# smacke/ffsubsync

Measured on NVIDIA H100. Metric: alignments/sec (2h@100Hz signals), higher is better.
Workload: dtype int64 VAD; f32 FFT nomination + f64 exact re-score

## Files before the change

__graft_entry__.py:

```python
import os
import subprocess
import sys

ROOT = os.path.dirname(os.path.abspath(__file__))
CSRC = os.path.join(ROOT, "ffsubsync_b200", "csrc")
LIB_DIR = os.path.join(ROOT, "ffsubsync_b200", "_lib")
LIB = os.path.join(LIB_DIR, "libffsubsync_b200.so")
EMUL = os.path.join(ROOT, "tests", "host_emul", "corr_emul")
EMUL_BIG = os.path.join(ROOT, "tests", "host_emul", "bigfft_emul")
EMUL_VAD = os.path.join(ROOT, "tests", "host_emul", "vad_emul")
EMUL_RUNS = os.path.join(ROOT, "tests", "host_emul", "runcorr_emul")
EMUL_RASTER = os.path.join(ROOT, "tests", "host_emul", "raster_emul")
EMUL_GSS = os.path.join(ROOT, "tests", "host_emul", "gss_emul")
EMUL_PLAN = os.path.join(ROOT, "tests", "host_emul", "plan_emul")

NVCC_FLAGS = [
    "-gencode", "arch=compute_90a,code=sm_90a", "-lineinfo", "-O3", "-std=c++17",
    "-Xcompiler", "-fPIC", "-Xcompiler", "-ffp-contract=off", "--fmad=true", "--extended-lambda",
    "-Wno-deprecated-gpu-targets",
]


def _sources():
    return sorted(os.path.join(CSRC, f) for f in os.listdir(CSRC) if f.endswith(".cu"))


def _stale(target, deps):
    if not os.path.exists(target):
        return True
    t = os.path.getmtime(target)
    return any(os.path.getmtime(d) > t for d in deps)


def build(force: bool = False, verbose: bool = False) -> None:
    nvcc = os.environ.get("NVCC", "/usr/local/cuda/bin/nvcc")
    os.makedirs(LIB_DIR, exist_ok=True)
    srcs = _sources()
    hdrs = [os.path.join(CSRC, f) for f in os.listdir(CSRC) if f.endswith((".cuh", ".h"))]
    hdrs.append(os.path.join(ROOT, "include", "ffsubsync_b200.h"))
    if force or _stale(LIB, srcs + hdrs):
        objs = []
        for s in srcs:
            o = os.path.join(LIB_DIR, os.path.basename(s)[:-3] + ".o")
            if force or _stale(o, [s] + hdrs):
                cmd = [nvcc] + NVCC_FLAGS + (["-Xptxas", "-v"] if verbose else []) + ["-c", s, "-o", o]
                subprocess.check_call(cmd)
            objs.append(o)
        subprocess.check_call([nvcc, "-shared", "-o", LIB] + objs + ["-Wno-deprecated-gpu-targets"])
    emu_src = EMUL + ".cu"
    if os.path.exists(emu_src) and (force or _stale(EMUL, [emu_src, os.path.join(CSRC, "corr.cuh")])):
        subprocess.check_call([nvcc, "-O2", "-std=c++17", "-Wno-deprecated-gpu-targets", "-o", EMUL, emu_src])
    big_src = EMUL_BIG + ".cu"
    if os.path.exists(big_src) and (force or _stale(EMUL_BIG, [big_src, os.path.join(CSRC, "corr.cuh"),
                                                               os.path.join(CSRC, "bigfft.cuh")])):
        subprocess.check_call([nvcc, "-O2", "-std=c++17", "--extended-lambda", "-Wno-deprecated-gpu-targets",
                               "-o", EMUL_BIG, big_src])
    runs_src = EMUL_RUNS + ".cu"
    if os.path.exists(runs_src) and (force or _stale(EMUL_RUNS, [runs_src, os.path.join(CSRC, "runcorr.cuh")])):
        subprocess.check_call([nvcc, "-O2", "-std=c++17", "-Wno-deprecated-gpu-targets", "-o", EMUL_RUNS, runs_src])
    raster_src = EMUL_RASTER + ".cu"
    if os.path.exists(raster_src) and (force or _stale(EMUL_RASTER, [raster_src, os.path.join(CSRC, "raster_math.cuh")])):
        subprocess.check_call([nvcc, "-O2", "-std=c++17", "-Xcompiler", "-ffp-contract=off",
                               "-Wno-deprecated-gpu-targets", "-o", EMUL_RASTER, raster_src])
    gss_src = EMUL_GSS + ".cu"
    if os.path.exists(gss_src) and (force or _stale(EMUL_GSS, [gss_src, os.path.join(CSRC, "job_plan.cuh"),
                                                               os.path.join(CSRC, "raster_math.cuh")])):
        subprocess.check_call([nvcc, "-O2", "-std=c++17", "-Xcompiler", "-ffp-contract=off",
                               "-Wno-deprecated-gpu-targets", "-o", EMUL_GSS, gss_src])
    plan_src = EMUL_PLAN + ".cu"
    if os.path.exists(plan_src) and (force or _stale(EMUL_PLAN, [plan_src] + hdrs)):
        subprocess.check_call([nvcc, "-O2", "-std=c++17", "-Xcompiler", "-ffp-contract=off",
                               "-Wno-deprecated-gpu-targets", "-o", EMUL_PLAN, plan_src])
    vad_src = EMUL_VAD + ".cu"
    if os.path.exists(vad_src) and (force or _stale(EMUL_VAD, [vad_src, os.path.join(CSRC, "vad_lane.cuh"),
                                                               os.path.join(CSRC, "vad_group.cuh")])):
        subprocess.check_call([nvcc, "-O2", "-std=c++17", "-gencode", "arch=compute_90a,code=sm_90a",
                               "-Wno-deprecated-gpu-targets", "-o", EMUL_VAD, vad_src])
    sys.path.insert(0, ROOT)
    import ffsubsync_b200
    from ffsubsync_b200 import _native

    _native.load()


def smoke() -> None:
    sys.path.insert(0, ROOT)
    import numpy as np

    from ffsubsync_b200.aligners import FFTAligner, MaxScoreAligner
    from ffsubsync_b200.speech_transformers import _make_auditok_detector, _make_energy_zcr_detector
    from oracle import aligner_oracle as ao
    from oracle import auditok_oracle as au
    from oracle import vad_oracle as vo

    rng = np.random.RandomState(0)
    cls = (rng.rand(2000) > 0.5).astype(np.uint8)
    pcm = vo.synth_pcm(cls, 160, seed=1)
    got = _make_energy_zcr_detector(100, 16000, 0.0)(pcm.tobytes())
    want = vo.energy_zcr_detect(pcm.tobytes(), 100, 16000, 0.0)
    assert np.array_equal(got, want), "VAD mismatch"
    got_a = _make_auditok_detector(100, 16000, 0.0)(pcm.tobytes())
    assert np.array_equal(got_a, au.auditok_detect_fast(pcm.tobytes(), 100, 16000, 0.0)), "auditok mismatch"
    ref = want
    sub = np.concatenate([np.zeros(123), ref])[: len(ref)]
    score, off = FFTAligner(max_offset_samples=600).fit_transform(ref, sub, get_score=True)
    wscore, woff = ao.fft_align(ref, sub, 600)
    assert off == woff == -123, (off, woff)
    assert abs(score - wscore) <= 1e-5 * abs(wscore), (score, wscore)
    (s2, o2), _ = MaxScoreAligner(FFTAligner, None, 100, 6).fit_transform(ref, [sub, sub[::-1].copy()])
    assert o2 == -123
    print("smoke ok: vad windows=%d offset=%d score=%.1f" % (len(got), off, score))


if __name__ == "__main__":
    build(force="--force" in sys.argv, verbose="-v" in sys.argv)
    if "--smoke" in sys.argv:
        smoke()
```

ffsubsync_b200/csrc/api.cu:

```cuda
#include <math.h>

#include <chrono>
#include <cmath>
#include <algorithm>
#include <atomic>
#include <thread>

#include "common.cuh"
#include "sync_plan.h"

struct DeviceScope {
  int prev = -1, want;
  bool ok = true;
  explicit DeviceScope(int dev) : want(dev) {
    if (cudaGetDevice(&prev) != cudaSuccess) prev = -1;
    if (prev != want) ok = cudaSetDevice(want) == cudaSuccess;
  }
  ~DeviceScope() {
    if (prev >= 0 && prev != want) cudaSetDevice(prev);
  }
};
extern "C" int b2_version(void) { return 200; }

static uint64_t compute_log2_quirk_mask() {
// ... 625 lines not shown
  if (memspace == B2_HOST) {
    void *da, *db, *dq;
    B2_TRY(stage_in(h, b2_ctx::WS_STAGE_IN0, a, (size_t)n * 4, &da));
    B2_TRY(stage_in(h, b2_ctx::WS_STAGE_IN1, b, (size_t)n * 4, &db));
    B2_TRY(b2i_ws(h, b2_ctx::WS_STAGE_OUT, (size_t)n * 4, &dq));
    d_a = (const float*)da;
    d_b = (const float*)db;
    d_out = (float*)dq;
  }
  B2_TRY(b2i_blend_launch(h, d_a, d_b, n, mode, wa, wb, d_out));
  if (memspace == B2_HOST) {
    B2_TRY(copy_out(h, out, d_out, (size_t)n * 4));
    B2_CUDA(h, cudaStreamSynchronize(h->stream));
  }
  return B2_OK;
}

extern "C" int b2_first_last_nonzero(b2_handle h, const float* sig, const int64_t* sig_off, int n,
                                     int64_t* first, int64_t* last, int memspace) {
  B2_ENTER(h);
  if (n < 0 || !sig_off || !first || !last) B2_FAIL(h, B2_ERR_BAD_ARG, "boundaries: bad arguments");
  if (n == 0) return B2_OK;
  const float* d_sig = sig;
  int64_t *d_first = first, *d_last = last;
  if (memspace == B2_HOST) {
    void *dp, *dq;
    B2_TRY(stage_in(h, b2_ctx::WS_STAGE_IN0, sig, (size_t)sig_off[n] * 4, &dp));
    B2_TRY(b2i_ws(h, b2_ctx::WS_STAGE_OUT, (size_t)n * 16, &dq));
    d_sig = (const float*)dp;
    d_first = (int64_t*)dq;
    d_last = d_first + n;
  }
  B2_TRY(b2i_bounds_launch(h, d_sig, sig_off, n, d_first, d_last));
  if (memspace == B2_HOST) {
    B2_TRY(copy_out(h, first, d_first, (size_t)n * 8));
    B2_TRY(copy_out(h, last, d_last, (size_t)n * 8));
    B2_CUDA(h, cudaStreamSynchronize(h->stream));
  }
  return B2_OK;
}

extern "C" int b2_align_batch(b2_handle h, const float* ref, const int64_t* ref_off,
                              const float* sub, const int64_t* sub_off, int B, int K,
                              int64_t max_offset_samples, double* score, int32_t* offset,
                              int32_t* status, int memspace) {
  B2_ENTER(h);
  if (B < 0 || K < 0 || !ref_off || !sub_off) B2_FAIL(h, B2_ERR_BAD_ARG, "align: bad arguments");
  if (B == 0 || K == 0) return B2_OK;
  if (!score || !offset || !status) B2_FAIL(h, B2_ERR_BAD_ARG, "align: null output");
  size_t J = (size_t)B * K;
  B2_CHECK_DEV(h, memspace, ref, "align: ref");
  B2_CHECK_DEV(h, memspace, sub, "align: sub");
  B2_CHECK_DEV(h, memspace, score, "align: score");
  const float *d_ref = ref, *d_sub = sub;
  double* d_score = score;
  int32_t *d_offset = offset, *d_status = status;
  if (memspace == B2_HOST) {
    void *dr, *ds, *dq;
    B2_TRY(stage_in(h, b2_ctx::WS_STAGE_IN0, ref, (size_t)ref_off[B] * 4, &dr));
    B2_TRY(stage_in(h, b2_ctx::WS_STAGE_IN1, sub, (size_t)sub_off[J] * 4, &ds));
    B2_TRY(b2i_ws(h, b2_ctx::WS_STAGE_OUT, J * 16 + 64, &dq));
    d_ref = (const float*)dr;
    d_sub = (const float*)ds;
    d_score = (double*)dq;
    d_offset = (int32_t*)(d_score + J);
    d_status = d_offset + J;
  }
  B2_TRY(b2i_align_launch(h, d_ref, ref_off, B, nullptr, d_sub, sub_off, B, K, max_offset_samples,
                          d_score, d_offset, d_status, 0, nullptr, 0));
  if (memspace == B2_HOST) {
    B2_TRY(copy_out(h, score, d_score, J * 8));
    B2_TRY(copy_out(h, offset, d_offset, J * 4));
    B2_TRY(copy_out(h, status, d_status, J * 4));
    B2_CUDA(h, cudaStreamSynchronize(h->stream));
  }
  return B2_OK;
}

extern "C" int b2_capture_nominations(b2_handle h, float* scores, int64_t stride, int64_t* win, float* stat,
                                      int32_t* cand) {
  B2_ENTER(h);
  h->capture = B2Capture{};
  if (!scores) return B2_OK;
  if (stride <= 0 || !win || !stat || !cand) B2_FAIL(h, B2_ERR_BAD_ARG, "capture: bad arguments");
  B2_TRY(check_device_ptr(h, scores, "capture: scores"));
  B2_TRY(check_device_ptr(h, win, "capture: win"));
  B2_TRY(check_device_ptr(h, stat, "capture: stat"));
  B2_TRY(check_device_ptr(h, cand, "capture: cand"));
  h->capture = B2Capture{scores, (long long)stride, (long long*)win, stat, cand};
  return B2_OK;
}

extern "C" int b2_reduce_ratios(b2_handle h, const double* score, const int32_t* offset,
                                const int32_t* status, int B, int K, int64_t max_offset_samples,
                                double* best_score, int32_t* best_offset, int32_t* best_k,
                                int memspace) {
  B2_ENTER(h);
  if (B < 0 || K <= 0) B2_FAIL(h, B2_ERR_BAD_ARG, "reduce: bad arguments");
  if (B == 0) return B2_OK;
  if (!score || !offset || !best_score || !best_offset || !best_k)
    B2_FAIL(h, B2_ERR_BAD_ARG, "reduce: null pointer");
  size_t J = (size_t)B * K;
  const double* d_score = score;
  const int32_t *d_offset = offset, *d_status = status;
  double* d_bs = best_score;
  int32_t *d_bo = best_offset, *d_bk = best_k;
  if (memspace == B2_HOST) {
    void *d0, *dq;
    B2_TRY(b2i_ws(h, b2_ctx::WS_STAGE_IN0, J * 16 + 64, &d0));
    B2_CUDA(h, cudaMemcpyAsync(d0, score, J * 8, cudaMemcpyHostToDevice, h->stream));
    int32_t* doff = (int32_t*)((char*)d0 + J * 8);
    B2_CUDA(h, cudaMemcpyAsync(doff, offset, J * 4, cudaMemcpyHostToDevice, h->stream));
    int32_t* dst = doff + J;
    if (status)
      B2_CUDA(h, cudaMemcpyAsync(dst, status, J * 4, cudaMemcpyHostToDevice, h->stream));
    B2_TRY(b2i_ws(h, b2_ctx::WS_STAGE_OUT, (size_t)B * 16 + 64, &dq));
    d_score = (const double*)d0;
    d_offset = doff;
    d_status = status ? dst : nullptr;
    d_bs = (double*)dq;
    d_bo = (int32_t*)(d_bs + B);
    d_bk = d_bo + B;
  }
  B2_TRY(b2i_reduce_launch(h, d_score, d_offset, d_status, B, K, max_offset_samples, d_bs, d_bo,
                           d_bk));
  if (memspace == B2_HOST) {
    B2_TRY(copy_out(h, best_score, d_bs, (size_t)B * 8));
    B2_TRY(copy_out(h, best_offset, d_bo, (size_t)B * 4));
    B2_TRY(copy_out(h, best_k, d_bk, (size_t)B * 4));
    B2_CUDA(h, cudaStreamSynchronize(h->stream));
  }
  return B2_OK;
}


struct SyncBufs {
  const int16_t* pcm;
  float* refsig;
  float* subsig;
  double* score;
  int32_t* offset;
  int32_t* status;
  double* bs;
  int32_t* bo;
  int32_t* bk;
  double* g_all_score;
  int32_t* g_all_offset;
  double* g_ratio;
  double* g_evals;
  bool fused;
  int winner_only;
};

static int enqueue_chain(b2_ctx* h, const SyncRequest& r, const SyncPlan& p, const SyncBufs& b, int v0, int v1) {
  const int K = r.K, t0 = p.trk_off[v0], nt = p.trk_off[v1] - t0;
  const size_t j0 = (size_t)t0 * K;
  std::vector<int> chain_trk(v1 - v0 + 1);
  for (int v = v0; v <= v1; ++v) chain_trk[v - v0] = p.trk_off[v] - t0;
  if (!b.fused)
    B2_TRY(b2i_raster_launch(h, r.cue_start_s, r.cue_end_s, r.cue_keep, r.cue_off + t0, nt, r.ratios, K, 0, nullptr,
                             r.sample_rate, r.start_seconds, b.subsig, p.sub_off.data() + j0));
  const B2CueSource src{r.cue_start_s, r.cue_end_s, r.cue_keep, r.cue_off + t0, r.ratios, r.sample_rate,
                        r.start_seconds, p.ref_label, p.two_level};
  B2_TRY(b2i_align_launch(h, b.refsig, p.ref_off.data() + v0, v1 - v0, chain_trk.data(), b.subsig,
                          p.sub_off.data() + j0, nt, K, r.max_offset_samples, b.score + j0, b.offset + j0,
                          b.status + j0, b.winner_only, b.fused ? &src : nullptr, (long long)j0));
  B2_TRY(b2i_reduce_launch(h, b.score + j0, b.offset + j0, b.status + j0, nt, K, r.max_offset_samples, b.bs + t0,
                           b.bo + t0, b.bk + t0));
  if (!p.gss || nt == 0) return B2_OK;
  const size_t a0 = (size_t)t0 * (K + 1);
  const B2GssOut go{b.bs + t0, b.bo + t0, b.bk + t0, b.score + j0, b.offset + j0,
                    b.g_all_score ? b.g_all_score + a0 : nullptr, b.g_all_offset ? b.g_all_offset + a0 : nullptr,
                    b.g_ratio + t0, b.g_evals ? b.g_evals + (size_t)t0 * kGssEvals : nullptr};
  return b2i_gss_launch(h, b.refsig, p.ref_off.data() + v0, v1 - v0, chain_trk.data(), K, src,
                        p.max_end.data() + t0, r.max_offset_samples, go);
}

static int detect(b2_ctx* h, const SyncRequest& r, const SyncPlan& p, const SyncBufs& b, int v0, int v1) {
  if (!p.auditok) {
    B2_TRY(b2i_vad_launch(h, b.pcm, r.pcm_off + v0, v1 - v0, p.fpw, r.energy.non_speech_label,
                          (int64_t)p.fpw * r.energy.energy_threshold, p.z_lo, p.z_hi, b.refsig, p.ref_off.data() + v0));
  } else {
    const ChunkTable& ch = p.ch;
    const int c0 = ch.first[v0], nc = ch.first[v1] - c0;
    B2_TRY(b2i_vad_launch(h, b.pcm, ch.pcm.data() + c0, nc, p.fpw, 0.0f, p.auditok_e_min, 0, p.fpw, b.refsig,
                          ch.out.data() + c0, ch.tail.data() + c0));
    if (!p.any_subs) return b2i_tokenize_inplace_launch(h, b.refsig, ch.out.data() + c0, nc, p.tok);
    const int k0 = ch.tok_first[v0];
    B2_TRY(b2i_tokenize_inplace_launch(h, b.refsig, ch.tok_off.data() + k0, ch.tok_first[v1] - k0, p.tok,
                                       ch.tok_end.data() + k0));
  }
  if (!p.any_subs) return B2_OK;
  const auto& sv = p.sub_video;
  const int s0 = (int)(std::lower_bound(sv.begin(), sv.end(), v0) - sv.begin());
  const int s1 = (int)(std::lower_bound(sv.begin(), sv.end(), v1) - sv.begin());
  if (s1 == s0) return B2_OK;
  std::vector<int> rel(sv.begin() + s0, sv.begin() + s1);
  for (int& v : rel) v -= v0;
  return b2i_raster_ref_launch(h, r.refs.cue_start_s, r.refs.cue_end_s, r.refs.cue_keep, r.refs.cue_off + v0,
                               p.ref_off.data() + v0, v1 - v0, rel.data(), (int)rel.size(), r.sample_rate,
                               r.start_seconds, b.refsig);
}

static int run_pipeline(b2_ctx* h, const SyncRequest& r, const SyncPlan& p, const SyncBufs& b, bool resident,
                        bool chained, int refsig_slot) {
  const int n_sub = p.n_sub;
  const std::vector<int>& cut = p.cut;
  if (n_sub == 1) {
    B2_TRY(detect(h, r, p, b, 0, r.V));
    return enqueue_chain(h, r, p, b, 0, r.V);
  }
  std::vector<cudaEvent_t> vad_done(n_sub);
  cudaEvent_t inputs_ready = next_event(h);
  B2_CUDA(h, cudaEventRecord(inputs_ready, h->stream));
  const bool trace = getenv("B2_PIPE_TRACE") != nullptr;
  std::vector<cudaEvent_t> tev;
  std::vector<double> host_ms(n_sub + 1, 0.0);
  const auto host_t0 = std::chrono::steady_clock::now();
  auto host_now = [&]() { return std::chrono::duration<double, std::milli>(std::chrono::steady_clock::now() - host_t0).count(); };
  if (trace) {
    tev.resize(1 + 4 * (size_t)n_sub);
    for (auto& e : tev) B2_CUDA(h, cudaEventCreate(&e));
    B2_CUDA(h, cudaEventRecord(tev[0], h->stream));
  }
  bool prev_busy = false;
  if (chained) {
    prev_busy = cudaEventQuery(h->resident_done) == cudaErrorNotReady;
    cudaGetLastError();
  }
  {
    Stream2Scope on2(h);
    B2_CUDA(h, cudaStreamWaitEvent(h->stream, chained ? h->resident_fence : inputs_ready, 0));
    for (int i = 0; i < n_sub; ++i) {
      h->vad_partition_sms = (i > 0 || prev_busy) ? p.vad_sms : 0;
      if (trace) B2_CUDA(h, cudaEventRecord(tev[1 + 4 * i], h->stream));
      const int st = detect(h, r, p, b, cut[i], cut[i + 1]);
      h->vad_partition_sms = 0;
      if (st != B2_OK) return st;
      vad_done[i] = next_event(h);
      B2_CUDA(h, cudaEventRecord(vad_done[i], h->stream));
      if (trace) B2_CUDA(h, cudaEventRecord(tev[2 + 4 * i], h->stream));
    }
  }
  host_ms[0] = host_now();
  for (int i = 0; i < n_sub; ++i) {
    if (resident && i == n_sub - 1) B2_CUDA(h, cudaEventRecord(h->resident_fence, h->stream));
    B2_CUDA(h, cudaStreamWaitEvent(h->stream, vad_done[i], 0));
    if (trace) B2_CUDA(h, cudaEventRecord(tev[3 + 4 * i], h->stream));
    B2_TRY(enqueue_chain(h, r, p, b, cut[i], cut[i + 1]));
    if (trace) B2_CUDA(h, cudaEventRecord(tev[4 + 4 * i], h->stream));
    host_ms[i + 1] = host_now();
  }
  if (resident) {
    B2_CUDA(h, cudaEventRecord(h->resident_done, h->stream));
    h->refsig_parity = refsig_slot == b2_ctx::WS_SIG_REF2 ? 1 : 0;
    h->resident_fence_valid = true;
  }
  if (trace) {
    B2_CUDA(h, cudaStreamSynchronize(h->stream2));
    B2_CUDA(h, cudaStreamSynchronize(h->stream));
    auto at = [&](size_t k) {
      float ms = 0.f;
      cudaEventElapsedTime(&ms, tev[0], tev[k]);
      return ms;
    };
    fprintf(stderr, "[b2 pipe] V=%d T=%d n_sub=%d vad_sms=%d chained=%d prev_busy=%d; host: VADs enqueued at %.3f ms\n",
            r.V, r.T, n_sub, p.vad_sms, (int)chained, (int)prev_busy, host_ms[0]);
    for (int i = 0; i < n_sub; ++i)
      fprintf(stderr, "[b2 pipe]  sub %d videos %4d..%4d  VAD %7.3f -> %7.3f ms   chain %7.3f -> %7.3f ms   host enqueued chain at %.3f ms\n",
              i, cut[i], cut[i + 1], at(1 + 4 * i), at(2 + 4 * i), at(3 + 4 * i), at(4 + 4 * i), host_ms[i + 1]);
    for (auto& e : tev) cudaEventDestroy(e);
  }
  return B2_OK;
}

static int sync_run(b2_ctx* h, bool fence_was_valid, const SyncRequest& r) {
  SyncPlan p;
  const SyncPipeEnv env{h->sm_count, b2_ctx::kEvents - 2, getenv("B2_SUBBATCHES"), getenv("B2_VAD_SMS"),
                        b2i_vad_lane_eligible};
  if (const int st = plan_sync(r, env, &p)) {
    h->err = p.err;
    return st;
  }
  const int T = r.T, K = r.K;
  if (T == 0) return B2_OK;
  const bool resident = r.memspace == B2_DEVICE_RESIDENT;
  const int memspace = resident ? B2_DEVICE : r.memspace;
  const char* prefix = r.track_video ? "sync_tracks" : "sync_batch";
  const std::pair<const void*, const char*> bulk[] = {{r.pcm, "pcm"}, {r.best_score, "best_score"},
                                                      {r.best_offset, "best_offset"}, {r.best_k, "best_k"},
                                                      {r.all_score, "all_score"}, {r.all_offset, "all_offset"}};
  for (const auto& [ptr, name] : bulk) {
    char what[64];
    snprintf(what, sizeof(what), "%s: %s", prefix, name);
    B2_CHECK_DEV(h, memspace, ptr, what);
  }
  if (p.gss) {
    B2_CHECK_DEV(h, memspace, r.gss_ratio, "sync_tracks_gss: gss_ratio");
    B2_CHECK_DEV(h, memspace, r.gss_evals, "sync_tracks_gss: gss_evals");
  }
  SyncBufs b{};
  b.fused = true;
  if (const char* e = getenv("B2_FUSED_RASTER")) b.fused = atoi(e) != 0;
  const size_t J = (size_t)T * K, JG = (size_t)T * (K + 1);
  void *d_refsig, *d_subsig = nullptr, *d_res;
  const bool chained = resident && fence_was_valid;
  const int refsig_slot = chained && h->refsig_parity == 0 ? b2_ctx::WS_SIG_REF2 : b2_ctx::WS_SIG_REF;
  B2_TRY(b2i_ws(h, refsig_slot, (size_t)p.ref_off[r.V] * 4 + 64, &d_refsig));
  if (!b.fused) B2_TRY(b2i_ws(h, b2_ctx::WS_SIG_SUB, (size_t)p.sub_off[J] * 4 + 64, &d_subsig));
  B2_TRY(b2i_ws(h, b2_ctx::WS_MISC, J * 16 + (size_t)T * 16 + 256, &d_res));
  double* d_score = (double*)d_res;
  double* d_bs = d_score + J;
  int32_t* d_offset = (int32_t*)(d_bs + T);
  int32_t* d_status = d_offset + J;
  int32_t* d_bo = d_status + J;
  int32_t* d_bk = d_bo + T;
  b.refsig = (float*)d_refsig;
  b.subsig = (float*)d_subsig;
  b.status = d_status;
  b.g_ratio = r.gss_ratio;
  b.g_evals = r.gss_evals;
  if (p.gss) {
    void* d_go;
    B2_TRY(b2i_ws(h, b2_ctx::WS_GSS_OUT, JG * 12 + (size_t)T * 8 * (1 + kGssEvals) + 256, &d_go));
    double* hs = (double*)d_go;
    double* hr = hs + JG;
    double* he = hr + T;
    int32_t* ho = (int32_t*)(he + (size_t)T * kGssEvals);
    b.g_all_score = r.all_score ? (memspace == B2_DEVICE ? r.all_score : hs) : nullptr;
    b.g_all_offset = r.all_offset ? (memspace == B2_DEVICE ? r.all_offset : ho) : nullptr;
    if (memspace != B2_DEVICE) {
      b.g_ratio = hr;
      b.g_evals = r.gss_evals ? he : nullptr;
    }
  }
  b.pcm = r.pcm;
  if (memspace == B2_HOST) {
    void* dp = nullptr;
    if (p.audio_samples > 0) B2_TRY(stage_in(h, b2_ctx::WS_STAGE_IN0, r.pcm, (size_t)r.pcm_off[r.V] * 2, &dp));
    b.pcm = (const int16_t*)dp;
  }
  const bool dev = memspace == B2_DEVICE;
  b.score = (dev && r.all_score && !p.gss) ? r.all_score : d_score;
  b.offset = (dev && r.all_offset && !p.gss) ? r.all_offset : d_offset;
  b.bs = dev ? r.best_score : d_bs;
  b.bo = dev ? r.best_offset : d_bo;
  b.bk = dev ? r.best_k : d_bk;
  b.winner_only = (!r.all_score && !r.all_offset) ? 1 : 0;
  B2_TRY(run_pipeline(h, r, p, b, resident, chained, refsig_slot));
  if (dev) return B2_OK;
  B2_TRY(copy_out(h, r.best_score, d_bs, (size_t)T * 8));
  B2_TRY(copy_out(h, r.best_offset, d_bo, (size_t)T * 4));
  B2_TRY(copy_out(h, r.best_k, d_bk, (size_t)T * 4));
  if (p.gss) {
    if (r.all_score) B2_TRY(copy_out(h, r.all_score, b.g_all_score, JG * 8));
    if (r.all_offset) B2_TRY(copy_out(h, r.all_offset, b.g_all_offset, JG * 4));
    B2_TRY(copy_out(h, r.gss_ratio, b.g_ratio, (size_t)T * 8));
    if (r.gss_evals) B2_TRY(copy_out(h, r.gss_evals, b.g_evals, (size_t)T * kGssEvals * 8));
  } else {
    if (r.all_score) B2_TRY(copy_out(h, r.all_score, d_score, J * 8));
    if (r.all_offset) B2_TRY(copy_out(h, r.all_offset, d_offset, J * 4));
  }
  B2_CUDA(h, cudaStreamSynchronize(h->stream));
  return B2_OK;
}

extern "C" int b2_sync_batch(b2_handle h, const int16_t* pcm, const int64_t* pcm_off, int B,
                             int frame_rate, int sample_rate, float non_speech_label,
                             int64_t energy_threshold, int z_lo, int z_hi,
                             const double* cue_start_s, const double* cue_end_s,
                             const uint8_t* cue_keep, const int64_t* cue_off, const double* ratios,
                             int K, double start_seconds, int64_t max_offset_samples,
                             double* best_score, int32_t* best_offset, int32_t* best_k,
                             double* all_score, int32_t* all_offset, int memspace) {
  B2_ENTER(h);
  B2Range range("b2_sync_batch");
  const SyncRequest r{"sync_batch", pcm, pcm_off, B, nullptr, B, frame_rate, sample_rate, B2_DETECTOR_ENERGY_ZCR,
                      {non_speech_label, energy_threshold, z_lo, z_hi}, {}, {},
                      cue_start_s, cue_end_s, cue_keep, cue_off, ratios, K, start_seconds, max_offset_samples,
                      best_score, best_offset, best_k, all_score, all_offset, false, nullptr, nullptr, memspace};
  return sync_run(h, _b2_fence_was_valid, r);
}

extern "C" int b2_sync_tracks(b2_handle h, const int16_t* pcm, const int64_t* pcm_off, int V,
                              const int32_t* track_video, int T, int frame_rate, int sample_rate,
                              float non_speech_label, int64_t energy_threshold, int z_lo, int z_hi,
                              const double* cue_start_s, const double* cue_end_s, const uint8_t* cue_keep,
                              const int64_t* cue_off, const double* ratios, int K, double start_seconds,
                              int64_t max_offset_samples, double* best_score, int32_t* best_offset,
                              int32_t* best_k, double* all_score, int32_t* all_offset, int memspace) {
  B2_ENTER(h);
  B2Range range("b2_sync_tracks");
  if (T > 0 && !track_video) B2_FAIL(h, B2_ERR_BAD_ARG, "sync_tracks: null track_video");
  const SyncRequest r{"sync_tracks", pcm, pcm_off, V, track_video, T, frame_rate, sample_rate, B2_DETECTOR_ENERGY_ZCR,
                      {non_speech_label, energy_threshold, z_lo, z_hi}, {}, {},
                      cue_start_s, cue_end_s, cue_keep, cue_off, ratios, K, start_seconds, max_offset_samples,
                      best_score, best_offset, best_k, all_score, all_offset, false, nullptr, nullptr, memspace};
  return sync_run(h, _b2_fence_was_valid, r);
}

extern "C" int b2_sync_tracks_gss(b2_handle h, const int16_t* pcm, const int64_t* pcm_off, int V,
                                  const int32_t* track_video, int T, int frame_rate, int sample_rate,
                                  float non_speech_label, int64_t energy_threshold, int z_lo, int z_hi,
                                  const double* cue_start_s, const double* cue_end_s, const uint8_t* cue_keep,
                                  const int64_t* cue_off, const double* ratios, int K, double start_seconds,
                                  int64_t max_offset_samples, double* best_score, int32_t* best_offset,
                                  int32_t* best_k, double* all_score, int32_t* all_offset, double* gss_ratio,
                                  double* gss_evals, int memspace) {
  B2_ENTER(h);
  B2Range range("b2_sync_tracks_gss");
  if (T > 0 && !track_video) B2_FAIL(h, B2_ERR_BAD_ARG, "sync_tracks_gss: null track_video");
  const SyncRequest r{"sync_tracks_gss", pcm, pcm_off, V, track_video, T, frame_rate, sample_rate,
                      B2_DETECTOR_ENERGY_ZCR, {non_speech_label, energy_threshold, z_lo, z_hi}, {}, {},
                      cue_start_s, cue_end_s, cue_keep, cue_off, ratios, K, start_seconds, max_offset_samples,
                      best_score, best_offset, best_k, all_score, all_offset, true, gss_ratio, gss_evals, memspace};
  return sync_run(h, _b2_fence_was_valid, r);
}

extern "C" int b2_sync_tracks_auditok(b2_handle h, const int16_t* pcm, const int64_t* pcm_off, int V,
                                      const int32_t* track_video, int T, int frame_rate, int sample_rate,
                                      double non_speech_label, double energy_threshold_db, double min_length,
                                      int64_t max_length, double max_continuous_silence, int64_t chunk_samples,
                                      const double* cue_start_s, const double* cue_end_s, const uint8_t* cue_keep,
                                      const int64_t* cue_off, const double* ratios, int K, double start_seconds,
                                      int64_t max_offset_samples, double* best_score, int32_t* best_offset,
                                      int32_t* best_k, double* all_score, int32_t* all_offset, double* gss_ratio,
                                      double* gss_evals, int memspace) {
  B2_ENTER(h);
  B2Range range("b2_sync_tracks_auditok");
  if (T > 0 && !track_video) B2_FAIL(h, B2_ERR_BAD_ARG, "sync_tracks_auditok: null track_video");
  if (!gss_ratio && gss_evals) B2_FAIL(h, B2_ERR_BAD_ARG, "sync_tracks_auditok: gss_evals without gss_ratio");
  const SyncRequest r{gss_ratio ? "sync_tracks_auditok (search)" : "sync_tracks_auditok", pcm, pcm_off, V, track_video,
                      T, frame_rate, sample_rate, B2_DETECTOR_AUDITOK, {},
                      {non_speech_label, energy_threshold_db, min_length, max_continuous_silence, max_length,
                       chunk_samples},
                      {}, cue_start_s, cue_end_s, cue_keep, cue_off, ratios, K, start_seconds, max_offset_samples,
                      best_score, best_offset, best_k, all_score, all_offset, gss_ratio != nullptr, gss_ratio, gss_evals,
                      memspace};
  return sync_run(h, _b2_fence_was_valid, r);
}

extern "C" int b2_sync_tracks_subs(b2_handle h, const int16_t* pcm, const int64_t* pcm_off, int V,
                                   const int32_t* track_video, int T, int frame_rate, int sample_rate, int detector,
                                   double non_speech_label, int64_t energy_threshold, int z_lo, int z_hi,
                                   double energy_threshold_db, double min_length, int64_t max_length,
                                   double max_continuous_silence, int64_t chunk_samples, const uint8_t* ref_is_subs,
                                   const double* ref_cue_start_s, const double* ref_cue_end_s,
                                   const uint8_t* ref_cue_keep, const int64_t* ref_cue_off,
                                   const double* cue_start_s, const double* cue_end_s, const uint8_t* cue_keep,
                                   const int64_t* cue_off, const double* ratios, int K, double start_seconds,
                                   int64_t max_offset_samples, double* best_score, int32_t* best_offset,
                                   int32_t* best_k, double* all_score, int32_t* all_offset, double* gss_ratio,
                                   double* gss_evals, int memspace) {
  B2_ENTER(h);
  B2Range range("b2_sync_tracks_subs");
  if (T > 0 && !track_video) B2_FAIL(h, B2_ERR_BAD_ARG, "sync_tracks_subs: null track_video");
// ... 17 lines not shown
```

ffsubsync_b200/csrc/bigfft.cu:

```cuda
#include <math.h>

#include <algorithm>
#include <map>

#include "common.cuh"
#include "bigfft.cuh"
#include "corr_jobs.cuh"

int bigfft_min_log2n() { return bigfft::kMinQ1 + 11; }
int bigfft_max_log2n() { return bigfft::kMaxQ1 + 11; }

namespace {

using namespace bigfft;

struct BigXform {
  long long src_off;
  long long g_off;
  long long spec_off;
  long long score_off;
  int len, S, m_lo, m_hi;
  int is_bits;
  float hi;
};

struct BigJob {
  int j;
  int x_sub, x_ref;
};

constexpr int kFineCap = (1 << kMaxQ1) + (1 << (kMaxQ1 - 4)) + (1 << (kMaxQ1 - 8)) + 4;
constexpr size_t kBigSmemBytes = kSmemBytes + 1024 * 8 + (size_t)kSkew1024 * 8 + (size_t)kFineCap * 8 + 16 * 8 + 64;

struct Smem {
  float2 *buf, *tw1024, *fine32, *half_pos, *coarse, *fine, *row_tw;
};
__device__ __forceinline__ Smem carve(unsigned char* raw) {
  Smem s;
  s.buf = reinterpret_cast<float2*>(raw);
  s.tw1024 = s.buf + kM;
  s.fine32 = s.tw1024 + 1024;
  s.half_pos = s.fine32 + 32;
  s.coarse = s.half_pos + 1024;
  s.fine = s.coarse + kSkew1024;
  s.row_tw = s.fine + kFineCap;
  return s;
}

__device__ __forceinline__ void l2_prefetch_bulk(const void* p, uint32_t bytes) {
  asm volatile("cp.async.bulk.prefetch.L2.global [%0], %1;" ::"l"(p), "r"(bytes) : "memory");
}
__device__ __forceinline__ void l2_prefetch_line(const void* p) {
  asm volatile("prefetch.global.L2 [%0];" ::"l"(p));
}
__device__ __forceinline__ void prefetch_f2_rows(const float2* base, int q1, int g, int tid) {
  if (tid < 16) l2_prefetch_bulk(base + ((size_t)f2_row_of_slot(q1, g, tid) << 10), kRow * 8);
}
__device__ __forceinline__ void prefetch_cols(const float2* base, int q1, int cg, int tid) {
  const int cl = 14 - q1, c0 = cg << cl, seg = 8 << cl;
  for (int r = tid; r < (1 << q1); r += kThreads) {
    const char* p = reinterpret_cast<const char*>(base + ((size_t)r << 10) + c0);
    for (int b = 0; b < seg; b += 128) l2_prefetch_line(p + b);
  }
}

__device__ __forceinline__ float block_sum(float v, float* red) {
  for (int o = 16; o > 0; o >>= 1) v += __shfl_xor_sync(0xffffffffu, v, o);
  __syncthreads();
  if ((threadIdx.x & 31) == 0) red[threadIdx.x >> 5] = v;
  __syncthreads();
  float r = 0.f;
  for (int w = 0; w < kThreads / 32; ++w) r += red[w];
  return r;
}
__device__ __forceinline__ float block_max(float v, float* red) {
  for (int o = 16; o > 0; o >>= 1) v = fmaxf(v, __shfl_xor_sync(0xffffffffu, v, o));
  __syncthreads();
  if ((threadIdx.x & 31) == 0) red[threadIdx.x >> 5] = v;
  __syncthreads();
  float r = -INFINITY;
  for (int w = 0; w < kThreads / 32; ++w) r = fmaxf(r, red[w]);
  return r;
}

template <int Q1>
__global__ void __launch_bounds__(kThreads, 1)
    big_cols_forward_kernel(const float* __restrict__ sig, const uint32_t* __restrict__ bits,
                            const BigXform* __restrict__ xf, int n_tiles, float2* __restrict__ G,
                            float* __restrict__ tile_energy) {
  extern __shared__ __align__(16) unsigned char smem_raw[];
  __shared__ float red[kThreads / 32];
  const Smem sm = carve(smem_raw);
  const int tid = threadIdx.x;
  init_tables(sm.tw1024, sm.fine32, tid);
  init_big_tables(sm.half_pos, sm.coarse, sm.fine, Q1, tid);
  __syncthreads();
  const Tables t{sm.tw1024, sm.fine32};
  const BigTables bt{sm.tw1024, sm.fine32, sm.half_pos, sm.coarse, sm.fine};
  constexpr int tiles_per = (1 << Q1) / 16;
  for (int tile = blockIdx.x; tile < n_tiles; tile += gridDim.x) {
    const BigXform X = xf[tile / tiles_per];
    const int cg = tile % tiles_per;
    const BigSource src{X.is_bits ? nullptr : sig + X.src_off, X.is_bits ? bits + X.src_off : nullptr, X.len, X.hi};
    const float ss = block_sum(f1_load(sm.buf, src, Q1, cg, tid), red);
    if (tid == 0) tile_energy[tile] = ss;
    col_forward<Q1>(sm.buf, t, tid);
    __syncthreads();
    f1_store(sm.buf, bt, Q1, cg, tid, G + X.g_off);
    __syncthreads();
  }
}

template <int MODE>
__global__ void __launch_bounds__(kThreads, 1)
    big_rows_kernel(const BigXform* __restrict__ xf, int n_tiles, int q1, float2* __restrict__ G) {
  extern __shared__ __align__(16) unsigned char smem_raw[];
  const Smem sm = carve(smem_raw);
  const int tid = threadIdx.x;
  init_tables(sm.tw1024, sm.fine32, tid);
  init_big_tables(sm.half_pos, sm.coarse, sm.fine, q1, tid);
  __syncthreads();
  const Tables t{sm.tw1024, sm.fine32};
  const BigTables bt{sm.tw1024, sm.fine32, sm.half_pos, sm.coarse, sm.fine};
  const int tiles_per = (1 << q1) / 16;
  for (int tile = blockIdx.x; tile < n_tiles; tile += gridDim.x) {
    const BigXform X = xf[tile / tiles_per];
    const int g = tile % tiles_per;
    if (tile + (int)gridDim.x < n_tiles) {
      const int nt = tile + gridDim.x;
      const BigXform Xn = xf[nt / tiles_per];
      prefetch_f2_rows(G + Xn.g_off, q1, nt % tiles_per, tid);
      if (MODE == 1) prefetch_f2_rows(G + Xn.spec_off, q1, nt % tiles_per, tid);
    }
    f2_load(sm.buf, q1, g, tid, G + X.g_off);
    f2_row_twiddles(sm.row_tw, q1, g, tid);
    __syncthreads();
    rows_forward(sm.buf, t, tid);
    __syncthreads();
    if (MODE == 0) {
      f2_untangle_inplace(sm.buf, bt, q1, g, sm.row_tw, tid);
      __syncthreads();
      f2_store(sm.buf, q1, g, tid, G + X.spec_off);
    } else {
      f2_product_inplace(sm.buf, bt, q1, g, sm.row_tw, tid, G + X.spec_off);
      __syncthreads();
      rows_inverse(sm.buf, t, tid);
      __syncthreads();
      f2_store_twiddled(sm.buf, bt, q1, g, tid, G + X.g_off);
    }
    __syncthreads();
  }
}

template <int Q1>
__global__ void __launch_bounds__(kThreads, 1)
    big_cols_inverse_kernel(const BigXform* __restrict__ xf, int n_tiles, const float2* __restrict__ G,
                            float* __restrict__ scores, float* __restrict__ tile_max,
                            float* __restrict__ tile_cn) {
  extern __shared__ __align__(16) unsigned char smem_raw[];
  __shared__ float red[kThreads / 32];
  const Smem sm = carve(smem_raw);
  const int tid = threadIdx.x;
  init_tables(sm.tw1024, sm.fine32, tid);
// ... 268 lines not shown
```

ffsubsync_b200/csrc/common.cuh:

```cuda
#pragma once

#include <cuda_runtime.h>
#include <stdint.h>
#include <stdio.h>
#include <string.h>

#include <string>
#include <vector>

#include <nvtx3/nvToolsExt.h>

#include "../../include/ffsubsync_b200.h"

struct B2Range {
  explicit B2Range(const char* name) { nvtxRangePushA(name); }
  ~B2Range() { nvtxRangePop(); }
};

struct DeviceBuf {
  void* p = nullptr;
  size_t cap = 0;
};

struct HostBuf {
  void* p = nullptr;
  size_t cap = 0;
};

struct B2Capture {
  float* scores = nullptr;
  long long stride = 0;
  long long* win = nullptr;
  float* stat = nullptr;
  int* cand = nullptr;
};

struct b2_ctx {
  int device = 0;
  int sm_count = 132;
  cudaStream_t stream = nullptr;
  bool own_stream = true;
  std::string err;
  int64_t launches = 0;
  uint64_t log2_quirk_mask = 0;
  int vad_partition_sms = 0;
  B2Capture capture;
  bool resident_fence_valid = false;
  cudaEvent_t resident_fence = nullptr, resident_done = nullptr;
  int refsig_parity = 0;
  enum { WS_STAGE_IN0, WS_STAGE_IN1, WS_STAGE_OUT, WS_META, WS_SPEC, WS_SCORES, WS_CAND,
         WS_SIG_REF, WS_SIG_REF2, WS_SIG_SUB, WS_MISC, WS_COUNTERS, WS_RUNS, WS_GSS, WS_GSS_OUT, WS_COUNT };
  DeviceBuf ws[WS_COUNT];
  HostBuf pinned[4];
  cudaEvent_t pinned_ev[4] = {};
  static const int kMetaSlots = 8;
  struct MetaSlot {
    void* d = nullptr;
    void* p = nullptr;
    size_t cap = 0;
    cudaEvent_t ev = nullptr;
  };
  MetaSlot meta[2][kMetaSlots];
  uint64_t meta_seq[2] = {0, 0};
  int ring = 0;
  struct VadStream {
    static const int kSlots = 3;
    struct Slot {
      void* hp = nullptr;
      void* dp = nullptr;
      float* hout = nullptr;
      float* dout = nullptr;
      size_t cap = 0, out_cap = 0;
      cudaEvent_t ev = nullptr;
      int64_t n_out = 0;
      bool busy = false;
    } slot[kSlots];
    bool active = false;
    int frame_rate = 0, sample_rate = 0, fpw = 0, z_lo = 0, z_hi = 0;
    float label = 0.f;
    int64_t thr = 0, windows = 0;
    uint64_t seq = 0;
    std::vector<float> results;
  } vs;
  struct Bounce {
    void* p = nullptr;
    cudaEvent_t ev = nullptr;
  } bounce[2];
  cudaStream_t stream2 = nullptr;
  static const int kEvents = 64;
  cudaEvent_t ev_pool[kEvents] = {};
  int ev_next = 0;
};

#define B2_FAIL(h, code, ...)                          \
  do {                                                 \
    char _b[512];                                      \
    snprintf(_b, sizeof(_b), __VA_ARGS__);             \
    (h)->err = _b;                                     \
    return (code);                                     \
  } while (0)

#define B2_CUDA(h, expr)                                                              \
  do {                                                                                \
    cudaError_t _e = (expr);                                                          \
    if (_e != cudaSuccess)                                                            \
      B2_FAIL(h, B2_ERR_CUDA, "%s failed: %s (%s:%d)", #expr, cudaGetErrorString(_e), \
              __FILE__, __LINE__);                                                    \
  } while (0)

#define B2_CHECK_LAUNCH(h, name)                                                         \
  do {                                                                                   \
    (h)->launches++;                                                                     \
    cudaError_t _e = cudaGetLastError();                                                 \
    if (_e != cudaSuccess)                                                               \
      B2_FAIL(h, B2_ERR_CUDA, "launch of %s failed: %s", name, cudaGetErrorString(_e));  \
  } while (0)

#define B2_TRY(expr)            \
  do {                          \
    int _s = (expr);            \
    if (_s != B2_OK) return _s; \
  } while (0)

int b2i_ws(b2_ctx* h, int which, size_t bytes, void** out);
int b2i_pinned(b2_ctx* h, int which, size_t bytes, void** out);
struct MetaArena {
  b2_ctx* h;
  char* dbase = nullptr;
  char* hbase = nullptr;
  size_t cap = 0, used = 0;
  int slot = 0, ring = 0;
};
int b2i_meta_begin(b2_ctx* h, MetaArena* a, size_t bytes);
void* b2i_meta_put(MetaArena* a, const void* src, size_t bytes);
void* b2i_meta_reserve(MetaArena* a, size_t bytes, void** host_view);
int b2i_meta_commit(MetaArena* a);

static inline int64_t ceil_div64(int64_t a, int64_t b) { return (a + b - 1) / b; }

bool b2i_vad_lane_eligible(const int64_t* pcm_off_host, int B, int fpw);
int b2i_vad_launch(b2_ctx* h, const int16_t* d_pcm, const int64_t* pcm_off_host, int B, int fpw,
                   float non_speech_label, int64_t e_min_full, int z_lo, int z_hi,
                   float* d_out, const int64_t* out_off_host, const int64_t* tail_emin_host = nullptr);
struct B2TokenizerParams {
  double min_length, max_continuous_silence, non_speech_label;
  long long max_length;
};
int b2i_tokenize_launch(b2_ctx* h, const float* d_flags, const int64_t* off_host, int n_chunks,
                        const B2TokenizerParams& tp, double* d_out);
int b2i_tokenize_inplace_launch(b2_ctx* h, float* d_flags_sig, const int64_t* off_host, int n_chunks,
                                const B2TokenizerParams& tp, const int64_t* end_host = nullptr);
int b2i_synth_launch(b2_ctx* h, const uint8_t* d_cls, int64_t n_windows, int fpw, uint32_t seed,
                     int16_t* d_out);
int b2i_raster_launch(b2_ctx* h, const double* cue_start, const double* cue_end,
                      const uint8_t* cue_keep, const int64_t* cue_off, int B, const double* ratios,
                      int K, int per_pair_ratios, const double* levels, int sample_rate,
                      double start_seconds, float* d_out, const int64_t* out_off_host);
int b2i_raster_ref_launch(b2_ctx* h, const double* cue_start, const double* cue_end, const uint8_t* cue_keep,
                          const int64_t* cue_off, const int64_t* out_off, int n_videos, const int* videos, int n_subs,
                          int sample_rate, double start_seconds, float* d_out);
int b2i_bounds_launch(b2_ctx* h, const float* d_sig, const int64_t* off_host, int n,
                      int64_t* d_first, int64_t* d_last);
int b2i_blend_launch(b2_ctx* h, const float* d_a, const float* d_b, int64_t n, int mode, double wa,
                     double wb, float* d_out);
struct B2CueSource {
  const double* cue_start;
  const double* cue_end;
  const uint8_t* cue_keep;
  const int64_t* cue_off;
  const double* ratios;
  int sample_rate;
  double start_seconds;
  float ref_label;
  bool ref_two_level;
};
int b2i_raster_bits_launch(b2_ctx* h, const B2CueSource* src, int B, int K, const int64_t* sig_off,
                           const long long* bits_off, uint32_t* d_bits);
struct B2CueDev {
  const double* start;
  const double* end;
  const uint8_t* keep;
  const long long* cue_off;
  int sample_rate;
  double start_seconds;
};
int b2i_raster_bits_dev_launch(b2_ctx* h, const B2CueDev& cues, int n_sig, int64_t max_cues, const double* d_ratio,
                               const long long* d_len, long long sig_words, uint32_t* d_bits);
int b2i_align_launch(b2_ctx* h, const float* d_ref, const int64_t* ref_off_host, int V, const int* trk_off,
                     const float* d_sub, const int64_t* sub_off_host, int B, int K,
                     int64_t max_offset_samples, double* d_score, int32_t* d_offset,
                     int32_t* d_status, int winner_only, const B2CueSource* cue_src,
                     long long capture_j0);
int b2i_reduce_launch(b2_ctx* h, const double* d_score, const int32_t* d_offset,
                      const int32_t* d_status, int B, int K, int64_t max_offset_samples,
                      double* d_best_score, int32_t* d_best_offset, int32_t* d_best_k);
struct B2GssOut {
  double* bs;
  int32_t* bo;
  int32_t* bk;
  const double* g_score;
  const int32_t* g_offset;
  double* a_score;
  int32_t* a_offset;
  double* gss_ratio;
  double* evals;
};
int b2i_gss_launch(b2_ctx* h, const float* d_ref, const int64_t* ref_off_host, int V, const int* trk_off, int K,
                   const B2CueSource& src, const double* max_end, int64_t max_offset_samples, const B2GssOut& out);
```

ffsubsync_b200/csrc/corr.cu:

```cuda
#include <math.h>

#include <algorithm>
#include <cmath>

#include "common.cuh"
#include "corr.cuh"
#include "corr_jobs.cuh"
#include "job_plan.cuh"

namespace {

using namespace corr;

struct SpecItem {
  long long ref_off;
  int R;
  int i0;
};

struct SubJob {
  long long sub_off;
  long long score_off;
  long long spec_base;
  int S, blk_lo, blk_hi, n_out, energy_slot;
  long long bits_off;
  float hi;
};

constexpr size_t kSmemBytesBits = kSmemBytes + 2 * (size_t)(kP / 32) * 4;

__device__ __forceinline__ void l2_prefetch(const void* p, uint32_t bytes) {
  asm volatile("cp.async.bulk.prefetch.L2.global [%0], %1;" ::"l"(p), "r"(bytes) : "memory");
}

__device__ __forceinline__ void l2_prefetch_floats(const float* p, int n) {
  if (n <= 0) return;
  const uintptr_t a0 = (reinterpret_cast<uintptr_t>(p) + 15) & ~uintptr_t(15);
  const uintptr_t a1 = reinterpret_cast<uintptr_t>(p + n) & ~uintptr_t(15);
  if (a1 > a0) l2_prefetch(reinterpret_cast<const void*>(a0), (uint32_t)(a1 - a0));
}

__global__ void __maxnreg__(96)
    ref_spectra_kernel(const float* __restrict__ ref, const SpecItem* __restrict__ items, int n_items,
                       float4* __restrict__ spec, float* __restrict__ spec_energy) {
  extern __shared__ __align__(16) unsigned char smem_raw[];
  float2* buf = reinterpret_cast<float2*>(smem_raw);
  float2* tw1024 = buf + kM;
  float2* fine32 = tw1024 + 1024;
  __shared__ float red[kThreads / 32];
  const int tid = threadIdx.x;
  init_tables(tw1024, fine32, tid);
  __syncthreads();
  const Tables t{tw1024, fine32};
  const PairCtx pc = pair_ctx(t, tid);
  for (int item = blockIdx.x; item < n_items; item += gridDim.x) {
    const SpecItem it = items[item];
    if (tid == 0 && item + (int)gridDim.x < n_items) {
      const SpecItem nx = items[item + gridDim.x];
      const int lo = nx.i0 < 0 ? -nx.i0 : 0, hi = min(nx.R - nx.i0, kP);
      l2_prefetch_floats(ref + nx.ref_off + nx.i0 + lo, hi - lo);
    }
    float ss = float_pass1(buf, t, tid, ref + it.ref_off + it.i0, it.i0 < 0 ? -it.i0 : 0,
                           min(it.R - it.i0, kP));
    forward_rest(buf, t, tid);
    spec_store(buf, t, pc, tid, spec + (size_t)item * kPairs);
    for (int o = 16; o > 0; o >>= 1) ss += __shfl_xor_sync(0xffffffffu, ss, o);
    if ((tid & 31) == 0) red[tid >> 5] = ss;
    __syncthreads();
    if (tid == 0) {
      float e = 0.f;
      for (int w = 0; w < kThreads / 32; ++w) e += red[w];
      spec_energy[item] = e;
    }
  }
}

template <bool BITS>
__device__ __forceinline__ void sub_correlate_body(
    const float* __restrict__ sub, const SubJob* __restrict__ jobs, const float4* __restrict__ spec,
    const float* __restrict__ spec_energy, int L, float* __restrict__ scores,
    float4* __restrict__ job_energy, const uint32_t* __restrict__ sub_bits) {
  extern __shared__ __align__(16) unsigned char smem_raw[];
  float2* buf = reinterpret_cast<float2*>(smem_raw);
  float2* tw1024 = buf + kM;
  float2* fine32 = tw1024 + 1024;
  uint32_t* bit_words = reinterpret_cast<uint32_t*>(smem_raw + kSmemBytes);
  __shared__ float red[kThreads / 32];
  const int tid = threadIdx.x;
  const SubJob job = jobs[blockIdx.x];
  float* out = scores + job.score_off;
  if (job.blk_lo >= job.blk_hi) {
    for (int m = tid; m < job.n_out; m += kThreads) out[m] = 0.f;
    if (tid == 0) job_energy[job.energy_slot] = make_float4(0.f, 0.f, 0.f, 0.f);
    return;
  }
  init_tables(tw1024, fine32, tid);
  const int wpb = L >> 5;
  const uint32_t* bits = BITS ? sub_bits + job.bits_off : nullptr;
  if (BITS) {
    const uint32_t* src = bits + (long long)job.blk_lo * wpb;
    uint32_t* dst = bit_words + (job.blk_lo & 1) * (kP / 32);
    for (int w = tid; w < wpb; w += kThreads) dst[w] = __ldg(src + w);
  }
  __syncthreads();
  const Tables t{tw1024, fine32};
  const PairCtx pc = pair_ctx(t, tid);
  SubState st;
  sub_state_clear(st);
  float er = 0.f;
  for (int blk = job.blk_lo; blk < job.blk_hi; ++blk) {
    const int j0 = blk * L;
    const bool more = blk + 1 < job.blk_hi;
    if (tid == 0 && more) {
      const int jn = j0 + L;
      if (!BITS) l2_prefetch_floats(sub + job.sub_off + jn, min(job.S - jn, L));
      l2_prefetch(spec + (size_t)(job.spec_base + (blk + 1 - job.blk_lo)) * kPairs, kPairs * 16);
    }
    uint32_t nw0 = 0, nw1 = 0;
    if (BITS) {
      const uint32_t* src = bits + (long long)(blk + 1) * wpb;
      if (more && tid < wpb) nw0 = __ldg(src + tid);
      if (more && tid + kThreads < wpb) nw1 = __ldg(src + tid + kThreads);
      st.ss += bits_pass1(buf, t, tid, bit_words + (blk & 1) * (kP / 32), min(job.S - j0, L), L, job.hi);
      forward_rest(buf, t, tid);
    } else {
      BlockSource s;
      s.src = sub + job.sub_off + j0;
      s.t_lo = 0;
      s.t_hi = min(job.S - j0, L);
      st.ss += forward_block(buf, t, tid, s);
    }
    const size_t item = (size_t)(job.spec_base + (blk - job.blk_lo));
    sub_accumulate(st, buf, t, pc, tid, spec + item * kPairs);
    er += spec_energy[item];
    if (BITS) {
      uint32_t* dst = bit_words + ((blk + 1) & 1) * (kP / 32);
      dst[tid] = nw0;
      dst[tid + kThreads] = nw1;
    }
    __syncthreads();
  }
  sub_retangle_store(st, buf, t, pc, tid);
  __syncthreads();
  inverse_passes_1(buf, tid);
  __syncthreads();
  inverse_passes_2(buf, t, tid);
  __syncthreads();
  inverse_passes_3(buf, t, tid);
  __syncthreads();
  inverse_passes_4(buf, t, tid);
  __syncthreads();
  for (int m = tid; m < job.n_out; m += kThreads) out[m] = window_value(buf, m);
  float cn = 0.f;
  for (int i = tid; i < kM; i += kThreads) {
    const float2 z = buf[i];
    cn = fmaf(z.x, z.x, fmaf(z.y, z.y, cn));
  }
  cn *= kOutScale * kOutScale;
  float ss = st.ss;
  for (int o = 16; o > 0; o >>= 1) {
    ss += __shfl_xor_sync(0xffffffffu, ss, o);
    cn += __shfl_xor_sync(0xffffffffu, cn, o);
  }
  __shared__ float red2[kThreads / 32];
  if ((tid & 31) == 0) {
// ... 64 lines not shown
        ex += e.x;
        ey += e.y;
        cn += sqrtf(e.z);
        blocks = fmaxf(blocks, e.w);
      }
      const float fwd = kTauFwd + fmaxf(0.f, blocks - (float)kTauBlocks);
      tau = fmaxf(tau, tau_bound(fwd, sqrtf(ex * ey), kTauInv + (float)(job.n_split - 1), cn));
    }
    job_stat[blockIdx.x] = make_float2(smax[0], nomination_tau(tau));
  }
}


__device__ __forceinline__ float nomination_cut(const SelJob& job, const float2* __restrict__ job_stat, int j,
                                                int K, int winner_only, bool& approx_only) {
  const float2 stat = job_stat[j];
  approx_only = false;
  if (winner_only && !job.no_prune) {
    const int b0 = (j / K) * K;
    float best_floor = -INFINITY;
    for (int k = 0; k < K; ++k) {
      const float2 s = job_stat[b0 + k];
      best_floor = fmaxf(best_floor, s.x - s.y);
    }
    if (stat.x + stat.y < best_floor) {
      approx_only = true;
      return stat.x;
    }
  }
  return stat.x - stat.y;
}

__global__ void __launch_bounds__(256) nominate_count_kernel(const SelJob* __restrict__ sel,
                                                              const int* __restrict__ jlist,
                                                              const float* __restrict__ scores,
                                                              const float2* __restrict__ job_stat, int K,
                                                              int winner_only, int n_chunks,
                                                              int* __restrict__ chunk_cnt) {
  const int j = jlist ? jlist[blockIdx.x] : (int)blockIdx.x;
  const SelJob job = sel[j];
  if (job.kind != 0 || job.m_lo > job.m_hi) return;
  __shared__ int s_cnt[8];
  bool approx;
  const float cut = nomination_cut(job, job_stat, j, K, winner_only, approx);
  const float* c = scores + job.score_off;
  for (int ch = blockIdx.y; ch < n_chunks; ch += gridDim.y) {
    const int lo = max(job.m_lo, ch * kChunk), hi = min(job.m_hi, ch * kChunk + (kChunk - 1));
    int cnt = 0;
    for (int m = lo + threadIdx.x; m <= hi; m += 256) cnt += c[m] >= cut;
    for (int o = 16; o > 0; o >>= 1) cnt += __shfl_xor_sync(0xffffffffu, cnt, o);
    if ((threadIdx.x & 31) == 0) s_cnt[threadIdx.x >> 5] = cnt;
    __syncthreads();
    if (threadIdx.x == 0) {
      int tot = 0;
      for (int w = 0; w < 8; ++w) tot += s_cnt[w];
      chunk_cnt[(size_t)blockIdx.x * n_chunks + ch] = tot;
    }
    __syncthreads();
  }
}

__global__ void __launch_bounds__(256) nominate_select_kernel(const SelJob* __restrict__ sel,
                                                               const int* __restrict__ jlist,
                                                               const float* __restrict__ scores,
                                                               const float2* __restrict__ job_stat, int K,
                                                               int winner_only, int n_chunks,
                                                               const int* __restrict__ chunk_cnt,
                                                               int* __restrict__ cand_off,
                                                               int* __restrict__ cand_cnt,
                                                               int* __restrict__ work_list,
                                                               int* __restrict__ work_count) {
  const int j = jlist ? jlist[blockIdx.x] : (int)blockIdx.x;
  const SelJob job = sel[j];
  const int tid = threadIdx.x;
  __shared__ int scount;
  __shared__ int swarp[8];
  if (job.kind != 0 || job.m_lo > job.m_hi) {
    if (tid == 0) cand_cnt[j] = 0;
    return;
  }
  bool approx_only;
  const float cut = nomination_cut(job, job_stat, j, K, winner_only, approx_only);
  const float* c = scores + job.score_off;
  __shared__ int hit_chunk[kCandMax];
  __shared__ int n_hit, s_total;
  if (tid == 0) {
    scount = 0;
    n_hit = 0;
    s_total = 0;
  }
  __syncthreads();
  const int* cnt = chunk_cnt + (size_t)blockIdx.x * n_chunks;
  for (int top = n_chunks - 1; top >= 0; top -= 256) {
    const int ch = top - tid;
    const int here = ch >= 0 ? cnt[ch] : 0;
    const unsigned ball = __ballot_sync(0xffffffffu, here > 0);
    int wsum = here;
    for (int o = 16; o > 0; o >>= 1) wsum += __shfl_xor_sync(0xffffffffu, wsum, o);
    if ((tid & 31) == 0) {
      swarp[tid >> 5] = __popc(ball);
      atomicAdd(&s_total, wsum);
    }
    __syncthreads();
    int before = n_hit;
    for (int w = 0; w < (tid >> 5); ++w) before += swarp[w];
    before += __popc(ball & ((1u << (tid & 31)) - 1u));
    if (here > 0 && before < kCandMax) hit_chunk[before] = ch;
    __syncthreads();
    if (tid == 0) {
      int tot = 0;
      for (int w = 0; w < 8; ++w) tot += swarp[w];
      n_hit += tot;
    }
    __syncthreads();
  }
  const int total = s_total;
  const int n_walk = min(n_hit, kCandMax);
  for (int h = 0; h < n_walk; ++h) {
    if (scount >= kCandMax) break;
    const int ch = hit_chunk[h];
    const int lo = max(job.m_lo, ch * kChunk), hi = min(job.m_hi, ch * kChunk + (kChunk - 1));
    for (int top = hi; top >= lo; top -= 256) {
      const int m = top - tid;
      const bool hit = (m >= lo) && (c[m] >= cut);
      const unsigned ball = __ballot_sync(0xffffffffu, hit);
      if ((tid & 31) == 0) swarp[tid >> 5] = __popc(ball);
      __syncthreads();
      int before = scount;
      for (int w = 0; w < (tid >> 5); ++w) before += swarp[w];
      before += __popc(ball & ((1u << (tid & 31)) - 1u));
      if (hit && before < kCandMax) cand_off[(size_t)j * kCandMax + before] = job.o_first + m;
      __syncthreads();
      if (tid == 0) {
        int tot = 0;
        for (int w = 0; w < 8; ++w) tot += swarp[w];
        scount += tot;
      }
      __syncthreads();
    }
  }
  if (approx_only) {
    if (tid == 0) cand_cnt[j] = -1;
    return;
  }
  if (tid == 0) {
    cand_cnt[j] = total;
    scount = min(total, kCandMax);
    swarp[0] = atomicAdd(work_count, scount);
  }
  __syncthreads();
  if (tid < scount) work_list[swarp[0] + tid] = (j << 5) | tid;
}

__global__ void __launch_bounds__(256) rescore_kernel(const SelJob* __restrict__ jobs,
                                                       const float* __restrict__ ref,
                                                       const float* __restrict__ sub,
                                                       const int* __restrict__ cand_off,
                                                       const int* __restrict__ work_list,
                                                       const int* __restrict__ work_count,
                                                       const uint32_t* __restrict__ sub_bits,
                                                       double* __restrict__ cand_partial) {
  __shared__ double sh[256];
  const int total = *work_count * kRescoreSeg;
  for (int w = blockIdx.x; w < total; w += gridDim.x) {
    const int item = work_list[w / kRescoreSeg], seg = w % kRescoreSeg;
    const int j = item >> 5, ci = item & 31;
    const SelJob job = jobs[j];
    const int o = cand_off[(size_t)j * kCandMax + ci];
    const float* r = ref + job.ref_off;
    const float* s = sub + job.sub_off;
    const int j_lo = max(0, -o), j_hi = min(job.S, job.R - o);
    const int len = max(0, j_hi - j_lo);
    const int per = (len + kRescoreSeg - 1) / kRescoreSeg;
    const int a0 = j_lo + seg * per, a1 = min(j_hi, a0 + per);
    double acc = 0.0;
    int i = a0 + threadIdx.x;
    if (job.bits_off >= 0) {
      const uint32_t* bits = sub_bits + job.bits_off;
      const double hi = 2.0 * (double)job.sub_level - 1.0;
      for (; i + 7 * 256 < a1; i += 8 * 256) {
        uint32_t bw[8];
        float rv[8];
#pragma unroll
        for (int u = 0; u < 8; ++u) {
          bw[u] = __ldg(bits + ((i + u * 256) >> 5));
          rv[u] = __ldg(r + i + u * 256 + o);
        }
#pragma unroll
        for (int u = 0; u < 8; ++u)
          acc = fma(((bw[u] >> (i & 31)) & 1u) ? hi : -1.0, 2.0 * (double)rv[u] - 1.0, acc);
      }
      for (; i < a1; i += 256) {
        const double a = ((__ldg(bits + (i >> 5)) >> (i & 31)) & 1u) ? hi : -1.0;
        const double b = 2.0 * (double)__ldg(r + i + o) - 1.0;
        acc = fma(a, b, acc);
      }
    }
    for (; i + 3 * 256 < a1; i += 4 * 256) {
      float sv[4], rv[4];
#pragma unroll
      for (int u = 0; u < 4; ++u) {
        sv[u] = __ldg(s + i + u * 256);
        rv[u] = __ldg(r + i + u * 256 + o);
      }
#pragma unroll
      for (int u = 0; u < 4; ++u)
        acc = fma(2.0 * (double)sv[u] - 1.0, 2.0 * (double)rv[u] - 1.0, acc);
    }
    for (; i < a1; i += 256) {
      const double a = 2.0 * (double)__ldg(s + i) - 1.0;
      const double b = 2.0 * (double)__ldg(r + i + o) - 1.0;
      acc = fma(a, b, acc);
    }
    sh[threadIdx.x] = acc;
    __syncthreads();
    for (int h = 128; h > 0; h >>= 1) {
      if (threadIdx.x < h) sh[threadIdx.x] += sh[threadIdx.x + h];
      __syncthreads();
    }
    if (threadIdx.x == 0) cand_partial[((size_t)j * kCandMax + ci) * kRescoreSeg + seg] = sh[0];
    __syncthreads();
  }
}

__global__ void __launch_bounds__(128) pick_kernel(const SelJob* __restrict__ jobs, int n_jobs,
                                                    const int* __restrict__ cand_off,
                                                    const int* __restrict__ cand_cnt,
                                                    const double* __restrict__ cand_partial,
                                                    const float2* __restrict__ job_stat,
                                                    double* __restrict__ score,
                                                    int32_t* __restrict__ offset,
                                                    int32_t* __restrict__ status) {
  const int j = blockIdx.x * blockDim.x + threadIdx.x;
  if (j >= n_jobs) return;
  const SelJob job = jobs[j];
  if (job.kind == 1) {
    score[job.out_index] = 0.0;
    offset[job.out_index] = 0;
    status[job.out_index] = B2_ALIGN_EMPTY;
    return;
  }
  if (job.kind == 2 || job.m_lo > job.m_hi) {
    score[job.out_index] = -INFINITY;
    offset[job.out_index] = job.masked_offset;
    status[job.out_index] = B2_ALIGN_ALL_MASKED;
    return;
  }
  const int cnt = cand_cnt[j];
  if (cnt < 0) {
    score[job.out_index] = (double)job_stat[j].x;
    offset[job.out_index] = cand_off[(size_t)j * kCandMax];
    status[job.out_index] = B2_ALIGN_APPROX;
    return;
  }
  const int n = min(cnt, kCandMax);
  double bs = -INFINITY;
  int bo = 0;
  for (int c = 0; c < n; ++c) {
    double s = 0.0;
    for (int g = 0; g < kRescoreSeg; ++g) s += cand_partial[((size_t)j * kCandMax + c) * kRescoreSeg + g];
    const int o = cand_off[(size_t)j * kCandMax + c];
    if (c == 0 || s > bs || (s == bs && o > bo)) {
      bs = s;
      bo = o;
    }
  }
  score[job.out_index] = bs;
  offset[job.out_index] = bo;
  status[job.out_index] = cnt > kCandMax ? B2_ALIGN_CAND_OVERFLOW : B2_ALIGN_OK;
}

__global__ void __launch_bounds__(256) capture_nominations_kernel(const SelJob* __restrict__ jobs,
                                                                   const int* __restrict__ jlist,
                                                                   const float* __restrict__ scores,
                                                                   const float2* __restrict__ job_stat,
                                                                   const int* __restrict__ cand_cnt,
                                                                   B2Capture cap, long long j0, int scores_written) {
  const int j = jlist ? jlist[blockIdx.x] : (int)blockIdx.x;
  const SelJob job = jobs[j];
  const bool live = job.kind == 0 && job.m_lo <= job.m_hi;
  if (live && !scores && !scores_written) return;
  const long long g = j0 + j;
  const int n = live ? job.m_hi - job.m_lo + 1 : 0;
  if (threadIdx.x == 0) {
    const float2 s = job_stat[j];
    cap.win[2 * g] = live ? (long long)job.o_first + job.m_lo : 0;
    cap.win[2 * g + 1] = n;
    cap.stat[2 * g] = s.x;
    cap.stat[2 * g + 1] = s.y;
    cap.cand[g] = cand_cnt[j];
  }
  if (n == 0 || scores_written) return;
  const float* c = scores + job.score_off + job.m_lo;
  float* out = cap.scores + g * cap.stride;
  for (int i = threadIdx.x; i < n; i += 256) out[i] = c[i];
}

long long floor_div(long long a, long long b) {
  long long q = a / b;
  if ((a % b != 0) && ((a < 0) != (b < 0))) --q;
  return q;
}

}

int b2i_select_launch(b2_ctx* h, const SelJob* d_sel, const int* d_jlist, int n, const float* scores,
                      int n_chunks, int K, int winner_only, int* chunk_cnt, const B2CandBuffers& cb) {
  if (n <= 0) return B2_OK;
  const dim3 grid((unsigned)n, (unsigned)std::min(n_chunks, 65535));
  nominate_count_kernel<<<grid, 256, 0, h->stream>>>(d_sel, d_jlist, scores, cb.job_stat, K, winner_only,
                                                     n_chunks, chunk_cnt);
  B2_CHECK_LAUNCH(h, "nominate_count_kernel");
  nominate_select_kernel<<<(unsigned)n, 256, 0, h->stream>>>(d_sel, d_jlist, scores, cb.job_stat, K, winner_only,
                                                             n_chunks, chunk_cnt, cb.cand_off, cb.cand_cnt,
                                                             cb.work_list, cb.work_count);
  B2_CHECK_LAUNCH(h, "nominate_select_kernel");
  return B2_OK;
}

int b2i_capture_launch(b2_ctx* h, const SelJob* d_sel, const int* d_jlist, int n, const float* scores,
                       const B2CandBuffers& cb, long long j0, bool scores_written) {
  if (n <= 0) return B2_OK;
  capture_nominations_kernel<<<(unsigned)n, 256, 0, h->stream>>>(d_sel, d_jlist, scores, cb.job_stat, cb.cand_cnt,
                                                                  h->capture, j0, scores_written ? 1 : 0);
  B2_CHECK_LAUNCH(h, "capture_nominations_kernel");
  return B2_OK;
}

int b2i_align_launch(b2_ctx* h, const float* d_ref, const int64_t* ref_off, int V, const int* trk_off,
                     const float* d_sub, const int64_t* sub_off, int B, int K, int64_t max_offset_samples,
                     double* d_score, int32_t* d_offset, int32_t* d_status, int winner_only,
                     const B2CueSource* cue_src, long long capture_j0) {
  B2Range range("b2:align (ref_spectra, sub_correlate, select, rescore, pick)");
  const size_t J = (size_t)B * K;
  std::vector<int> ident;
  if (!trk_off) {
    ident.resize(B + 1);
    for (int b = 0; b <= B; ++b) ident[b] = b;
    trk_off = ident.data();
    V = B;
  }
  const bool cue_mode = cue_src != nullptr;
  std::vector<long long> bits_off(cue_mode ? J + 1 : 1, 0);
  if (cue_mode)
    for (size_t j = 0; j < J; ++j)
      bits_off[j + 1] = bits_off[j] + ((sub_off[j + 1] - sub_off[j]) + kP) / 32 + 1;
  std::vector<SelJob> sel(J);
  std::vector<long long> idx_lo(J, 0), idx_hi(J, 0), n_pad(J, 0);
  struct PairPlan { long long o_min, o_max; int n_tiles; bool any; };
  std::vector<PairPlan> pp(V);
  long long max_w = 1;
  bool big_ok = true;
  const long long mo_clamped =
      std::max<long long>(-(1LL << 40), std::min<long long>(1LL << 40, max_offset_samples));
  for (int v = 0; v < V; ++v) {
    const long long R = ref_off[v + 1] - ref_off[v];
    if (R < 0 || R > 0x3fffffff) B2_FAIL(h, B2_ERR_BAD_ARG, "align: bad reference length at %d", v);
    PairPlan& p = pp[v];
    p.any = false;
    p.o_min = 0;
    p.o_max = -1;
    for (int b = trk_off[v]; b < trk_off[v + 1]; ++b) {
      long long t_min = 0, t_max = -1;
      bool t_any = false;
      for (int k = 0; k < K; ++k) {
        const size_t j = (size_t)b * K + k;
        const long long S = sub_off[j + 1] - sub_off[j];
        if (S < 0 || S > 0x3fffffff) B2_FAIL(h, B2_ERR_BAD_ARG, "align: bad subtitle length at %zu", j);
        SelJob& s = sel[j];
        memset(&s, 0, sizeof(s));
        s.ref_off = ref_off[v];
        s.sub_off = sub_off[j];
        s.R = (int)R;
        s.S = (int)S;
        s.out_index = (int)j;
        s.bits_off = cue_mode ? bits_off[j] : -1;
        s.sub_level = cue_mode ? (float)std::min(1.0 / cue_src->ratios[k], 1.0) : 0.f;
        const B2JobPlan jp = b2_plan_job(R, S, max_offset_samples, h->log2_quirk_mask);
        if (jp.kind != 0) {
          s.kind = jp.kind;
          s.masked_offset = jp.masked_offset;
          continue;
        }
        const long long N = jp.N, o_lo = jp.o_lo, o_hi = jp.o_hi;
        idx_lo[j] = jp.lo;
        idx_hi[j] = jp.hi;
        n_pad[j] = N;
        if (N < (1LL << (bigfft_min_log2n())) || N > (1LL << bigfft_max_log2n())) big_ok = false;
        s.kind = 0;
        s.m_lo = (int)o_lo;
        s.m_hi = (int)o_hi;
        t_min = t_any ? std::min(t_min, o_lo) : o_lo;
        t_max = t_any ? std::max(t_max, o_hi) : o_hi;
        t_any = true;
      }
      if (!t_any) continue;
      p.o_min = p.any ? std::min(p.o_min, t_min) : t_min;
      p.o_max = p.any ? std::max(p.o_max, t_max) : t_max;
      p.any = true;
      if (max_offset_samples != B2_MAX_OFFSET_NONE && std::max(llabs(t_min), llabs(t_max)) > mo_clamped)
        for (int k = 0; k < K; ++k) sel[(size_t)b * K + k].no_prune = 1;
    }
    if (p.any) max_w = std::max(max_w, p.o_max - p.o_min + 1);
  }
  const bool capture = h->capture.scores != nullptr;
  if (capture)
    for (size_t j = 0; j < J; ++j)
      if (sel[j].kind == 0 && (long long)sel[j].m_hi - sel[j].m_lo + 1 > h->capture.stride)
        B2_FAIL(h, B2_ERR_BAD_ARG, "capture: job %lld has %lld surviving offsets, stride %lld",
                capture_j0 + (long long)j, (long long)sel[j].m_hi - sel[j].m_lo + 1, h->capture.stride);
  const int Wt = (int)(max_w <= kP / 2 + 1 ? 32 * ((max_w + 30) / 32) + 1 : (kP / 2 + 1));
  const int L = kP - Wt + 1;
  uint32_t* d_bits = nullptr;
  if (cue_mode) {
    void* db;
    B2_TRY(b2i_ws(h, b2_ctx::WS_SIG_SUB, (size_t)bits_off[J] * 4 + 64, &db));
    d_bits = (uint32_t*)db;
    B2_TRY(b2i_raster_bits_launch(h, cue_src, B, K, sub_off, bits_off.data(), d_bits));
    B2_CUDA(h, cudaFuncSetAttribute(sub_correlate_bits_kernel,
                                    cudaFuncAttributeMaxDynamicSharedMemorySize, (int)kSmemBytesBits));
  }
  void* d_cand;
  B2_TRY(b2i_ws(h, b2_ctx::WS_CAND, J * kCandMax * (8 * kRescoreSeg + 8) + J * 12 + 64, &d_cand));
  B2CandBuffers cb;
  cb.cand_partial = (double*)d_cand;
  cb.job_stat = (float2*)(cb.cand_partial + J * kCandMax * kRescoreSeg);
  cb.cand_off = (int*)(cb.job_stat + J);
  cb.cand_cnt = cb.cand_off + J * kCandMax;
  cb.work_list = cb.cand_cnt + J;
  cb.work_count = cb.work_list + J * kCandMax;
  if (J >= (1u << 26)) B2_FAIL(h, B2_ERR_UNSUPPORTED, "align: B*K too large for one call");

  bool use_big = big_ok && max_w > (long long)kBigMinTiles * (kP / 2 + 1);
  const char* path_env = getenv("B2_ALIGN_PATH");
  const bool force_runs = path_env && !strcmp(path_env, "runs");
  if (path_env) {
    if (!strcmp(path_env, "tiled") || force_runs) use_big = false;
    if (!strcmp(path_env, "big") && big_ok) use_big = true;
  }
  if (cue_mode && (!capture || force_runs) && !use_big && cue_src->ref_two_level && std::isfinite(cue_src->ref_label) &&
      !(path_env && !strcmp(path_env, "tiled"))) {
    bool fits = true, pays = true;
    int max_runs = 1;
    for (int v = 0; v < V && fits; ++v) {
      const long long n_tiles_v = pp[v].any ? ceil_div64(pp[v].o_max - pp[v].o_min + 1, Wt) : 0;
      for (int b = trk_off[v]; b < trk_off[v + 1]; ++b) {
        const long long cues = cue_src->cue_off[b + 1] - cue_src->cue_off[b];
        for (int k = 0; k < K; ++k) {
          const SelJob& s = sel[(size_t)b * K + k];
          if (s.kind != 0) continue;
          const long long w = (long long)s.m_hi - s.m_lo + 1;
          if (w > kRunMaxWindow || cues > kRunMaxCues || llabs((long long)s.m_lo) > (1LL << 30) ||
              llabs((long long)s.m_hi) > (1LL << 30))
            fits = false;
          if ((double)cues * (double)w > kRunCostPerBlock * (double)(n_tiles_v * (ceil_div64(s.S, L) + 1)))
            pays = false;
          max_runs = std::max<int>(max_runs, (int)std::min<long long>(cues, kRunMaxCues));
        }
      }
    }
    if (fits && (pays || force_runs)) {
      const SelJob* d_sel_runs = nullptr;
      B2_TRY(b2i_align_runs(h, d_ref, ref_off, V, trk_off, K, sel, d_bits, max_runs, cue_src->ref_label, winner_only,
                            cb, &d_sel_runs, capture_j0));
      return b2i_rescore_pick(h, d_sel_runs, J, d_ref, d_sub, d_bits, cb, d_score, d_offset, d_status);
    }
  }
  if (use_big) {
    const SelJob* d_sel_big = nullptr;
    B2_TRY(b2i_align_big(h, d_ref, d_sub, d_bits, V, trk_off, K, sel, idx_lo, idx_hi, n_pad, winner_only, cb,
                         &d_sel_big, capture_j0));
    return b2i_rescore_pick(h, d_sel_big, J, d_ref, d_sub, d_bits, cb, d_score, d_offset, d_status);
  }

  long long n_jobs_total = 0, max_blocks = 1;
  for (int v = 0; v < V; ++v) {
    PairPlan& p = pp[v];
    p.n_tiles = p.any ? (int)ceil_div64(p.o_max - p.o_min + 1, Wt) : 0;
    for (size_t j = (size_t)trk_off[v] * K; j < (size_t)trk_off[v + 1] * K; ++j) {
      const SelJob& s = sel[j];
      if (s.kind != 0) continue;
      n_jobs_total += p.n_tiles;
      max_blocks = std::max<long long>(max_blocks, ceil_div64(s.S, L));
    }
  }
  int n_split = 1;
  if (n_jobs_total > 0 && n_jobs_total < 2LL * h->sm_count)
    n_split = (int)std::max<long long>(1, std::min<long long>(ceil_div64(2LL * h->sm_count, n_jobs_total),
                                                               max_blocks / 4));
  if (const char* e = getenv("B2_ALIGN_SPLIT")) n_split = std::max(1, atoi(e));
  long long score_total = 0, energy_total = 0, max_score_len = 0;
  for (int v = 0; v < V; ++v) {
    PairPlan& p = pp[v];
    for (size_t j = (size_t)trk_off[v] * K; j < (size_t)trk_off[v + 1] * K; ++j) {
      SelJob& s = sel[j];
      if (s.kind != 0) continue;
      max_score_len = std::max(max_score_len, (long long)p.n_tiles * Wt);
      s.o_first = (int)p.o_min;
      s.m_lo -= (int)p.o_min;
      s.m_hi -= (int)p.o_min;
      s.score_off = score_total;
      s.energy_slot = (int)energy_total;
      s.n_tiles = p.n_tiles;
      s.n_split = n_split;
      score_total += (long long)p.n_tiles * Wt * n_split;
      energy_total += (long long)p.n_tiles * n_split;
    }
  }

  const int n_chunks = (int)std::max<long long>(1, ceil_div64(max_score_len, kChunk));
  void* d_scores;
  B2_TRY(b2i_ws(h, b2_ctx::WS_SCORES,
                (size_t)(score_total + 16) * 4 + (size_t)(energy_total + 2) * 16 + J * n_chunks * 4, &d_scores));
  float* scores = (float*)d_scores;
  float4* job_energy = (float4*)((char*)d_scores + (((size_t)(score_total + 16) * 4 + 15) & ~size_t(15)));
  int* chunk_cnt = (int*)(job_energy + energy_total);

  B2_CUDA(h, cudaFuncSetAttribute(ref_spectra_kernel, cudaFuncAttributeMaxDynamicSharedMemorySize,
                                  (int)kSmemBytes));
  B2_CUDA(h, cudaFuncSetAttribute(sub_correlate_kernel, cudaFuncAttributeMaxDynamicSharedMemorySize,
                                  (int)kSmemBytes));

  const size_t kSpecBytes = (size_t)kPairs * 16;
  const size_t cap_items = std::max<size_t>(64, ((size_t)6 << 30) / kSpecBytes);
  std::vector<SpecItem> items;
  std::vector<SubJob> jobs;
  auto flush = [&]() -> int {
    if (jobs.empty()) {
      items.clear();
      return B2_OK;
    }
    void* d_spec;
    B2_TRY(b2i_ws(h, b2_ctx::WS_SPEC, items.size() * kSpecBytes + items.size() * 4 + 256, &d_spec));
    float4* spec = (float4*)d_spec;
    float* spec_energy = (float*)((char*)d_spec + items.size() * kSpecBytes);
    MetaArena a;
    B2_TRY(b2i_meta_begin(h, &a, items.size() * sizeof(SpecItem) + jobs.size() * sizeof(SubJob) + 256));
    const SpecItem* d_items = (const SpecItem*)b2i_meta_put(&a, items.data(), items.size() * sizeof(SpecItem));
    const SubJob* d_jobs = (const SubJob*)b2i_meta_put(&a, jobs.data(), jobs.size() * sizeof(SubJob));
    B2_TRY(b2i_meta_commit(&a));
    if (!items.empty()) {
      const unsigned grid = (unsigned)std::min<size_t>(items.size(), (size_t)h->sm_count);
      ref_spectra_kernel<<<grid, kThreads, kSmemBytes, h->stream>>>(d_ref, d_items, (int)items.size(),
                                                                    spec, spec_energy);
      B2_CHECK_LAUNCH(h, "ref_spectra_kernel");
    }
    if (cue_mode)
      sub_correlate_bits_kernel<<<(unsigned)jobs.size(), kThreads, kSmemBytesBits, h->stream>>>(
          d_jobs, spec, spec_energy, L, scores, job_energy, d_bits);
    else
      sub_correlate_kernel<<<(unsigned)jobs.size(), kThreads, kSmemBytes, h->stream>>>(
          d_sub, d_jobs, spec, spec_energy, L, scores, job_energy);
    B2_CHECK_LAUNCH(h, "sub_correlate_kernel");
    items.clear();
    jobs.clear();
    return B2_OK;
  };

  for (int v = 0; v < V; ++v) {
    const PairPlan& p = pp[v];
    if (!p.any) continue;
    const long long R = ref_off[v + 1] - ref_off[v];
    const size_t j_lo = (size_t)trk_off[v] * K, j_hi = (size_t)trk_off[v + 1] * K;
    long long nblk_max = 0;
    for (size_t j = j_lo; j < j_hi; ++j) {
      const SelJob& s = sel[j];
      if (s.kind == 0) nblk_max = std::max<long long>(nblk_max, ceil_div64(s.S, L));
    }
    for (int tile = 0; tile < p.n_tiles; ++tile) {
      const long long o_t = p.o_min + (long long)tile * Wt;
      const long long blk_lo = std::max(0LL, floor_div(-o_t - kP, L) + 1);
      const long long blk_hi = std::min<long long>(nblk_max, R - o_t > 0 ? ceil_div64(R - o_t, L) : 0LL);
      const long long n_items = std::max(0LL, blk_hi - blk_lo);
      if (items.size() + (size_t)n_items > cap_items) B2_TRY(flush());
      const long long spec_base = (long long)items.size();
      for (long long blk = blk_lo; blk < blk_hi; ++blk) {
        SpecItem it;
        it.ref_off = ref_off[v];
        it.R = (int)R;
        it.i0 = (int)(blk * L + o_t);
        items.push_back(it);
      }
      for (size_t j = j_lo; j < j_hi; ++j) {
        const SelJob& s = sel[j];
        if (s.kind != 0) continue;
        const long long job_hi = std::min<long long>(blk_hi, ceil_div64(s.S, L));
        const long long n_blk = std::max(0LL, job_hi - blk_lo);
        for (int sp = 0; sp < n_split; ++sp) {
          const long long c_lo = blk_lo + n_blk * sp / n_split, c_hi = blk_lo + n_blk * (sp + 1) / n_split;
          SubJob jb;
          jb.sub_off = s.sub_off;
          jb.S = s.S;
          jb.score_off = s.score_off + ((long long)sp * p.n_tiles + tile) * Wt;
          jb.spec_base = spec_base + (c_lo - blk_lo);
          jb.blk_lo = (int)c_lo;
          jb.blk_hi = (int)c_hi;
          jb.n_out = Wt;
          jb.energy_slot = s.energy_slot + tile * n_split + sp;
          jb.bits_off = 0;
          jb.hi = 0.f;
          if (cue_mode) {
            jb.bits_off = s.bits_off;
            jb.hi = 2.f * s.sub_level - 1.f;
          }
          jobs.push_back(jb);
        }
      }
    }
  }
  B2_TRY(flush());

  B2Range range_sel("b2:select+rescore+pick");

  MetaArena a;
  B2_TRY(b2i_meta_begin(h, &a, J * sizeof(SelJob) + 256));
  const SelJob* d_sel = (const SelJob*)b2i_meta_put(&a, sel.data(), J * sizeof(SelJob));
  B2_TRY(b2i_meta_commit(&a));
  B2_CUDA(h, cudaMemsetAsync(cb.work_count, 0, sizeof(int), h->stream));
  window_max_kernel<<<(unsigned)J, 256, 0, h->stream>>>(d_sel, scores, job_energy, cb.job_stat, Wt);
  B2_CHECK_LAUNCH(h, "window_max_kernel");
  B2_TRY(b2i_select_launch(h, d_sel, nullptr, (int)J, scores, n_chunks, K, winner_only, chunk_cnt, cb));
  if (capture) B2_TRY(b2i_capture_launch(h, d_sel, nullptr, (int)J, scores, cb, capture_j0));
  return b2i_rescore_pick(h, d_sel, J, d_ref, d_sub, d_bits, cb, d_score, d_offset, d_status);
}

int b2i_rescore_pick(b2_ctx* h, const SelJob* d_sel, size_t J, const float* d_ref, const float* d_sub,
                     const uint32_t* d_bits, const B2CandBuffers& cb, double* d_score, int32_t* d_offset,
                     int32_t* d_status) {
  rescore_kernel<<<(unsigned)(h->sm_count * 8), 256, 0, h->stream>>>(
      d_sel, d_ref, d_sub, cb.cand_off, cb.work_list, cb.work_count, d_bits, cb.cand_partial);
  B2_CHECK_LAUNCH(h, "rescore_kernel");
  pick_kernel<<<(unsigned)((J + 127) / 128), 128, 0, h->stream>>>(d_sel, (int)J, cb.cand_off, cb.cand_cnt,
                                                                   cb.cand_partial, cb.job_stat, d_score,
                                                                   d_offset, d_status);
  B2_CHECK_LAUNCH(h, "pick_kernel");
  return B2_OK;
}
```

ffsubsync_b200/csrc/corr_jobs.cuh:

```cuda
#pragma once
#include <stdint.h>

constexpr int kCandMax = 32;
constexpr int kRescoreSeg = 16;
constexpr float kU = 5.9604645e-8f;
constexpr float kTauFwd = 512.0f;
constexpr float kTauInv = 192.0f;
constexpr int kTauBlocks = 64;

__device__ __forceinline__ float tau_bound(float fwd, float sqrt_e, float inv, float cn) {
  return kU * (fwd * sqrt_e + inv * cn);
}
__device__ __forceinline__ float nomination_tau(float tau) { return tau * 1.0001f + 1e-30f; }

constexpr int kChunk = 4096;

struct SelJob {
  long long ref_off, sub_off, score_off;
  int R, S, o_first;
  int m_lo, m_hi;
  int energy_slot, n_tiles;
  int n_split;
  int out_index;
  int kind;
  int masked_offset;
  int no_prune;
  long long bits_off;
  float sub_level;
};


constexpr int kBigMinTiles = 4;
int bigfft_min_log2n();
int bigfft_max_log2n();

struct B2CandBuffers {
  double* cand_partial;
  float2* job_stat;
  int* cand_off;
  int* cand_cnt;
  int* work_list;
  int* work_count;
};
int b2i_select_launch(b2_ctx* h, const SelJob* d_sel, const int* d_jlist, int n, const float* scores,
                      int n_chunks, int K, int winner_only, int* chunk_cnt, const B2CandBuffers& cb);
int b2i_rescore_pick(b2_ctx* h, const SelJob* d_sel, size_t J, const float* d_ref, const float* d_sub,
                     const uint32_t* d_bits, const B2CandBuffers& cb, double* d_score, int32_t* d_offset,
                     int32_t* d_status);
int b2i_capture_launch(b2_ctx* h, const SelJob* d_sel, const int* d_jlist, int n, const float* scores,
                       const B2CandBuffers& cb, long long j0, bool scores_written = false);
int b2i_align_runs(b2_ctx* h, const float* d_ref, const int64_t* ref_off, int V, const int* trk_off, int K,
                   std::vector<SelJob>& sel, const uint32_t* d_bits, int max_runs, float ref_label, int winner_only,
                   const B2CandBuffers& cb, const SelJob** d_sel_out, long long capture_j0);
constexpr double kRunCostPerBlock = 5.6e5;
constexpr int kRunMaxCues = 16384;
constexpr int kRunMaxWindow = 32 * 1024;
struct GssTrack {
  long long ref_off;
  long long bits_off;
  double max_end;
  int R;
};
struct B2GssLane;
int b2i_gss_step_launch(b2_ctx* h, int r, int T, const GssTrack* d_trk, B2GssLane* d_lane, const double* prev_score,
                        SelJob* d_sel, double* d_x, long long* d_len, double* evals, long long max_offset_samples,
                        int sample_rate);
int b2i_gss_combine_launch(b2_ctx* h, int T, int K, const GssTrack* d_trk, const double* d_x, const double* r_score,
                           const int32_t* r_offset, long long max_offset_samples, const B2GssOut& out);
int b2i_align_big(b2_ctx* h, const float* d_ref, const float* d_sub, const uint32_t* d_bits, int V,
                  const int* trk_off, int K, std::vector<SelJob>& sel, const std::vector<long long>& idx_lo,
                  const std::vector<long long>& idx_hi, const std::vector<long long>& n_pad, int winner_only,
                  const B2CandBuffers& cb, const SelJob** d_sel_out, long long capture_j0);
```

ffsubsync_b200/csrc/runcorr.cu:

```cuda
#include <limits.h>
#include <math.h>

#include <algorithm>

#include "common.cuh"
#include "corr_jobs.cuh"
#include "job_plan.cuh"
#include "runcorr.cuh"

namespace {

using namespace runcorr;
static_assert(kMaxWindow == kRunMaxWindow, "run path window bound");

struct RunRef {
  long long ref_off;
  long long q_off;
  int R;
};

struct RunStat {
  double mx;
  double eps;
  int total;
  int arg;
};

__device__ __forceinline__ int block_excl_scan(int v, int* sh, int* total) {
  const int lane = threadIdx.x & 31, warp = threadIdx.x >> 5, nw = blockDim.x >> 5;
  int x = v;
#pragma unroll
  for (int d = 1; d < 32; d <<= 1) {
    const int y = __shfl_up_sync(0xffffffffu, x, d);
    if (lane >= d) x += y;
  }
  if (lane == 31) sh[warp] = x;
  __syncthreads();
  if (warp == 0) {
    int s = lane < nw ? sh[lane] : 0;
    const int own = s;
#pragma unroll
    for (int d = 1; d < 32; d <<= 1) {
      const int y = __shfl_up_sync(0xffffffffu, s, d);
      if (lane >= d) s += y;
    }
    sh[lane] = s - own;
    if (lane == 31) sh[32] = s;
  }
  __syncthreads();
  const int r = sh[warp] + x - v;
  *total = sh[32];
  __syncthreads();
  return r;
}

__global__ void __launch_bounds__(1024) ref_bits_kernel(const float* __restrict__ ref, const RunRef* __restrict__ vids,
                                                        uint2* __restrict__ q_all) {
  __shared__ int sh[33];
  const RunRef v = vids[blockIdx.x];
  const float* r = ref + v.ref_off;
  uint2* q = q_all + v.q_off;
  const int lane = threadIdx.x & 31, warp = threadIdx.x >> 5;
  const int n_words = (v.R >> 5) + 2;
  if (threadIdx.x == 0) q[0] = make_uint2(0u, 0u);
  int carry = 0;
  for (int w0 = 0; w0 < n_words; w0 += blockDim.x) {
    const int wb = w0 + 32 * warp;
    float x[32];
#pragma unroll
    for (int u = 0; u < 32; ++u) {
      const long long i = 32LL * (wb + u) + lane;
      x[u] = i < v.R ? __ldg(r + i) : 0.f;
    }
    uint32_t mine = 0;
#pragma unroll
    for (int u = 0; u < 32; ++u) {
      const long long i = 32LL * (wb + u) + lane;
      const uint32_t bal = __ballot_sync(0xffffffffu, i < v.R && x[u] == 1.0f);
      if (lane == u) mine = bal;
    }
    const int w = wb + lane;
    int tot;
    const int ex = block_excl_scan(__popc(mine), sh, &tot);
    if (w < n_words) q[w + 1] = make_uint2(mine, (uint32_t)(carry + ex));
    carry += tot;
  }
}

template <bool CAPTURE>
__global__ void __launch_bounds__(kMaxThreads) run_corr_kernel(const SelJob* __restrict__ sel,
                                                                const long long* __restrict__ job_q,
                                                                const uint2* __restrict__ q_all,
                                                                const uint32_t* __restrict__ sub_bits,
                                                                float ref_label, int max_runs,
                                                                RunStat* __restrict__ stat,
                                                                int* __restrict__ cand_off,
                                                                B2Capture cap, long long cap_j0) {
  extern __shared__ int rsm[];
  int* ra = rsm;
  int* rb = ra + max_runs;
  int* rl = rb + max_runs;
  __shared__ int sh[33];
  __shared__ double smx[32];
  __shared__ int sarg[32];
  const int j = blockIdx.x, tid = threadIdx.x, nthr = blockDim.x;
  const SelJob job = sel[j];
  if (job.kind != 0 || job.m_lo > job.m_hi) {
    if (tid == 0) stat[j] = RunStat{-INFINITY, 0.0, 0, 0};
    return;
  }
  const int R = job.R, S = job.S;
  const uint32_t* bits = sub_bits + job.bits_off;
  const int nws = S >> 5;
  int n_end = 0;
  for (int w0 = 0; w0 <= nws; w0 += nthr) {
    const int w = w0 + tid;
    uint32_t t = 0;
    if (w <= nws) {
      const int nb = S - 32 * w;
      const uint32_t x = nb >= 32 ? __ldg(bits + w) : (nb > 0 ? __ldg(bits + w) & ((1u << nb) - 1u) : 0u);
      const uint32_t prev = w > 0 ? __ldg(bits + w - 1) : 0u;
      t = x ^ ((x << 1) | (prev >> 31));
    }
    int tot;
    int idx = n_end + block_excl_scan(__popc(t), sh, &tot);
    while (t) {
      const int e = 32 * w + __ffs(t) - 1;
      t &= t - 1;
      if (idx < 2 * max_runs) (idx & 1 ? rb : ra)[idx >> 1] = e;
      ++idx;
    }
    n_end += tot;
  }
  const int nr = min(n_end >> 1, max_runs);
  __syncthreads();
  for (int r0 = 0, carry = 0; r0 < nr; r0 += nthr) {
    const int r = r0 + tid;
    const int len = r < nr ? rb[r] - ra[r] : 0;
    int tot;
    const int ex = block_excl_scan(len, sh, &tot);
    if (r < nr) rl[r] = carry + ex;
    carry += tot;
  }
  __syncthreads();
  const uint2* q = q_all + job_q[j];
  const int o_lo = job.o_first + job.m_lo, o_hi = job.o_first + job.m_hi;
  const int o0 = o_lo + kOffsetsPerThread * tid;
  const int n_mine = o0 <= o_hi ? min(kOffsetsPerThread, o_hi - o0 + 1) : 0;
  const RcLevels lv = rc_levels(job.sub_level, ref_label);
  int cnt[32], base = 0;
  if (n_mine > 0) {
    rc_thread_counts(q, R, ra, rb, nr, o0, cnt, base);
  } else {
#pragma unroll
    for (int t = 0; t < 32; ++t) cnt[t] = 0;
  }
  double best = -INFINITY;
  int barg = INT_MIN;
  {
    int um = base;
#pragma unroll
    for (int i = 0; i < 32; ++i) {
      if (i < n_mine) {
        const double g = rc_score(q, R, S, ra, rb, rl, nr, o0 + i, um, lv);
        if (CAPTURE) cap.scores[(cap_j0 + j) * cap.stride + kOffsetsPerThread * tid + i] = (float)g;
        if (g >= best) {
          best = g;
          barg = o0 + i;
        }
      }
      um += cnt[i] - nr;
    }
  }
  for (int d = 16; d > 0; d >>= 1) {
    const double ob = __shfl_xor_sync(0xffffffffu, best, d);
    const int oa = __shfl_xor_sync(0xffffffffu, barg, d);
    if (ob > best || (ob == best && oa > barg)) {
      best = ob;
      barg = oa;
    }
  }
  if ((tid & 31) == 0) {
    smx[tid >> 5] = best;
    sarg[tid >> 5] = barg;
  }
  __syncthreads();
  double mx = smx[0];
  int arg = sarg[0];
  for (int w = 1; w < (nthr >> 5); ++w)
    if (smx[w] > mx || (smx[w] == mx && sarg[w] > arg)) {
      mx = smx[w];
      arg = sarg[w];
    }
  const double eps = rc_eps((double)min(R, S), lv);
  const double cut = mx - eps;
  uint32_t hit = 0;
  {
    int um = base;
#pragma unroll
    for (int i = 0; i < 32; ++i) {
      if (i < n_mine && rc_score(q, R, S, ra, rb, rl, nr, o0 + i, um, lv) >= cut) hit |= 1u << i;
      um += cnt[i] - nr;
    }
  }
  int total;
  const int h = __popc(hit);
  int rank = block_excl_scan(h, sh, &total);
  rank = total - rank - h;
  while (hit && rank < kCandMax) {
    const int i = 31 - __clz(hit);
    hit &= ~(1u << i);
    cand_off[(size_t)j * kCandMax + rank] = o0 + i;
    ++rank;
  }
  if (tid == 0) stat[j] = RunStat{mx, eps, total, arg};
}

__global__ void __launch_bounds__(128) run_finalize_kernel(const SelJob* __restrict__ sel, int n_jobs, int K,
                                                            int winner_only, const RunStat* __restrict__ stat,
                                                            B2CandBuffers cb) {
  const int j = blockIdx.x * blockDim.x + threadIdx.x;
  if (j >= n_jobs) return;
  const SelJob job = sel[j];
  if (job.kind != 0 || job.m_lo > job.m_hi) {
    cb.cand_cnt[j] = 0;
    cb.job_stat[j] = make_float2(-INFINITY, 0.f);
    return;
  }
  const RunStat st = stat[j];
  cb.job_stat[j] = make_float2((float)st.mx, (float)st.eps);
  if (winner_only && !job.no_prune) {
    const int b0 = (j / K) * K;
    double best_floor = -INFINITY;
    for (int k = 0; k < K; ++k) {
      const RunStat s = stat[b0 + k];
      best_floor = fmax(best_floor, s.mx - s.eps);
    }
    if (fmax(st.mx, (double)(float)st.mx) + st.eps < best_floor) {
      cb.cand_off[(size_t)j * kCandMax] = st.arg;
      cb.cand_cnt[j] = -1;
      return;
    }
  }
  cb.cand_cnt[j] = st.total;
  const int n = min(st.total, kCandMax);
  const int slot = atomicAdd(cb.work_count, n);
  for (int i = 0; i < n; ++i) cb.work_list[slot + i] = (j << 5) | i;
}

}

int b2i_align_runs(b2_ctx* h, const float* d_ref, const int64_t* ref_off, int V, const int* trk_off, int K,
                   std::vector<SelJob>& sel, const uint32_t* d_bits, int max_runs, float ref_label, int winner_only,
                   const B2CandBuffers& cb, const SelJob** d_sel_out, long long capture_j0) {
  B2Range range("b2:align runs (ref_bits, run_corr, finalize)");
  const size_t J = sel.size();
  std::vector<RunRef> vids;
  std::vector<long long> job_q(J, 0);
  long long q_total = 0;
  int max_thr = 32;
  for (int v = 0; v < V; ++v) {
    const int R = (int)(ref_off[v + 1] - ref_off[v]);
    bool any = false;
    for (size_t j = (size_t)trk_off[v] * K; j < (size_t)trk_off[v + 1] * K; ++j) {
      SelJob& s = sel[j];
      if (s.kind != 0) continue;
      const long long w = (long long)s.m_hi - s.m_lo + 1;
      s.o_first = s.m_lo;
      s.m_lo = 0;
      s.m_hi = (int)(w - 1);
      max_thr = std::max<int>(max_thr, (int)(32 * ceil_div64(ceil_div64(w, kOffsetsPerThread), 32)));
      job_q[j] = q_total;
      any = true;
    }
    if (!any) continue;
    vids.push_back(RunRef{(long long)ref_off[v], q_total, R});
    q_total += rc_ref_entries(R);
  }
  if (max_thr > kMaxThreads) B2_FAIL(h, B2_ERR_UNSUPPORTED, "align runs: window wider than %d offsets", kMaxWindow);
  void* d_ws;
  const size_t q_bytes = ((size_t)q_total * 8 + 15) & ~size_t(15);
  B2_TRY(b2i_ws(h, b2_ctx::WS_RUNS, q_bytes + J * sizeof(RunStat) + 64, &d_ws));
  uint2* q = (uint2*)d_ws;
  RunStat* stat = (RunStat*)((char*)d_ws + q_bytes);
  MetaArena a;
  B2_TRY(b2i_meta_begin(h, &a, J * sizeof(SelJob) + J * 8 + vids.size() * sizeof(RunRef) + 256));
  const SelJob* d_sel = (const SelJob*)b2i_meta_put(&a, sel.data(), J * sizeof(SelJob));
  const long long* d_job_q = (const long long*)b2i_meta_put(&a, job_q.data(), J * 8);
  const RunRef* d_vids = vids.empty() ? nullptr : (const RunRef*)b2i_meta_put(&a, vids.data(), vids.size() * sizeof(RunRef));
  B2_TRY(b2i_meta_commit(&a));
  *d_sel_out = d_sel;
  if (!vids.empty()) {
    ref_bits_kernel<<<(unsigned)vids.size(), 1024, 0, h->stream>>>(d_ref, d_vids, q);
    B2_CHECK_LAUNCH(h, "ref_bits_kernel");
  }
  max_runs = std::max(1, max_runs);
  const size_t smem = (size_t)3 * max_runs * sizeof(int);
  const bool capture = h->capture.scores != nullptr;
  auto kernel = capture ? run_corr_kernel<true> : run_corr_kernel<false>;
  B2_CUDA(h, cudaFuncSetAttribute(kernel, cudaFuncAttributeMaxDynamicSharedMemorySize, (int)smem));
  kernel<<<(unsigned)J, (unsigned)max_thr, smem, h->stream>>>(d_sel, d_job_q, q, d_bits, ref_label, max_runs, stat,
                                                             cb.cand_off, h->capture, capture_j0);
  B2_CHECK_LAUNCH(h, "run_corr_kernel");
  B2_CUDA(h, cudaMemsetAsync(cb.work_count, 0, sizeof(int), h->stream));
  run_finalize_kernel<<<(unsigned)((J + 127) / 128), 128, 0, h->stream>>>(d_sel, (int)J, K, winner_only, stat, cb);
  B2_CHECK_LAUNCH(h, "run_finalize_kernel");
  if (capture) B2_TRY(b2i_capture_launch(h, d_sel, nullptr, (int)J, nullptr, cb, capture_j0, true));
  return B2_OK;
}

int b2i_gss_launch(b2_ctx* h, const float* d_ref, const int64_t* ref_off, int V, const int* trk_off, int K,
                   const B2CueSource& src, const double* max_end, int64_t max_offset_samples, const B2GssOut& out) {
  B2Range range("b2:gss rounds (step, raster_bits, run_corr, finalize, rescore, pick) x 17");
  const int T = trk_off[V] - trk_off[0];
  if (T <= 0) return B2_OK;
  if (max_offset_samples < 0 || max_offset_samples > kMaxWindow / 2)
    B2_FAIL(h, B2_ERR_UNSUPPORTED, "gss: max_offset_samples %lld is outside [0, %d]", (long long)max_offset_samples,
            kMaxWindow / 2);
  const long long w_bound = std::max<long long>(1, 2 * (long long)max_offset_samples);
  const int max_thr = (int)(32 * ceil_div64(ceil_div64(w_bound, kOffsetsPerThread), 32));
  std::vector<GssTrack> trk(T);
  std::vector<RunRef> vids;
  std::vector<long long> job_q(T, 0);
  long long q_total = 0, sig_words = 1;
  int max_runs = 1;
  const long long c0 = src.cue_off[0], nc = src.cue_off[T] - c0;
  for (int v = 0; v < V; ++v) {
    const long long R = ref_off[v + 1] - ref_off[v];
    if (R < 0 || R > 0x3fffffff) B2_FAIL(h, B2_ERR_BAD_ARG, "gss: bad reference length at %d", v);
    if (trk_off[v + 1] == trk_off[v]) continue;
    vids.push_back(RunRef{(long long)ref_off[v], q_total, (int)R});
    for (int t = trk_off[v]; t < trk_off[v + 1]; ++t) {
      const long long s_max = b2_signal_length(max_end[t], B2_GSS_HI, src.sample_rate);
      if (s_max > 0x3fffffff) B2_FAIL(h, B2_ERR_BAD_ARG, "gss: subtitle signal of track %d too long", t);
      sig_words = std::max(sig_words, (s_max >> 5) + 2);
      trk[t] = GssTrack{(long long)ref_off[v], 0, max_end[t], (int)R};
      job_q[t] = q_total;
      max_runs = std::max<int>(max_runs, (int)std::min<long long>(src.cue_off[t + 1] - src.cue_off[t], kRunMaxCues));
    }
    q_total += rc_ref_entries((int)R);
  }
  long long max_cues = 0;
  for (int t = 0; t < T; ++t) {
    trk[t].bits_off = (long long)t * sig_words;
    max_cues = std::max<long long>(max_cues, src.cue_off[t + 1] - src.cue_off[t]);
  }
  std::vector<long long> cue_rel(T + 1);
  for (int t = 0; t <= T; ++t) cue_rel[t] = src.cue_off[t] - c0;

  size_t at = 0;
  auto take = [&](size_t bytes) { const size_t o = at; at = (at + bytes + 255) & ~size_t(255); return o; };
  const size_t o_q = take((size_t)q_total * 8), o_stat = take((size_t)T * sizeof(RunStat)),
               o_lane = take((size_t)T * sizeof(B2GssLane)), o_sel = take((size_t)T * sizeof(SelJob)),
               o_x = take((size_t)T * 8), o_len = take((size_t)T * 8), o_rs = take((size_t)T * 8),
               o_ro = take((size_t)T * 4), o_rst = take((size_t)T * 4), o_bits = take((size_t)T * sig_words * 4),
               o_cp = take((size_t)T * kCandMax * kRescoreSeg * 8), o_js = take((size_t)T * 8),
               o_co = take((size_t)T * kCandMax * 4), o_cc = take((size_t)T * 4),
               o_wl = take((size_t)T * kCandMax * 4), o_wc = take(16);
  void* d_ws;
  B2_TRY(b2i_ws(h, b2_ctx::WS_GSS, at + 256, &d_ws));
  char* base = (char*)d_ws;
  uint2* q = (uint2*)(base + o_q);
  RunStat* stat = (RunStat*)(base + o_stat);
  B2GssLane* lane = (B2GssLane*)(base + o_lane);
  SelJob* d_sel = (SelJob*)(base + o_sel);
  double* d_x = (double*)(base + o_x);
  long long* d_len = (long long*)(base + o_len);
  double* r_score = (double*)(base + o_rs);
  int32_t* r_offset = (int32_t*)(base + o_ro);
  int32_t* r_status = (int32_t*)(base + o_rst);
  uint32_t* d_bits = (uint32_t*)(base + o_bits);
  B2CandBuffers cb;
  cb.cand_partial = (double*)(base + o_cp);
  cb.job_stat = (float2*)(base + o_js);
  cb.cand_off = (int*)(base + o_co);
  cb.cand_cnt = (int*)(base + o_cc);
  cb.work_list = (int*)(base + o_wl);
  cb.work_count = (int*)(base + o_wc);

  MetaArena a;
  B2_TRY(b2i_meta_begin(h, &a, (size_t)nc * 17 + (size_t)(T + 1) * 8 + (size_t)T * (sizeof(GssTrack) + 8) +
                                   vids.size() * sizeof(RunRef) + 1024));
  B2CueDev cues;
  cues.start = (const double*)b2i_meta_put(&a, src.cue_start + c0, (size_t)nc * 8);
  cues.end = (const double*)b2i_meta_put(&a, src.cue_end + c0, (size_t)nc * 8);
  cues.keep = src.cue_keep ? (const uint8_t*)b2i_meta_put(&a, src.cue_keep + c0, (size_t)nc) : nullptr;
  cues.cue_off = (const long long*)b2i_meta_put(&a, cue_rel.data(), (size_t)(T + 1) * 8);
  cues.sample_rate = src.sample_rate;
  cues.start_seconds = src.start_seconds;
  const GssTrack* d_trk = (const GssTrack*)b2i_meta_put(&a, trk.data(), (size_t)T * sizeof(GssTrack));
  const long long* d_job_q = (const long long*)b2i_meta_put(&a, job_q.data(), (size_t)T * 8);
  const RunRef* d_vids = (const RunRef*)b2i_meta_put(&a, vids.data(), vids.size() * sizeof(RunRef));
  B2_TRY(b2i_meta_commit(&a));

  ref_bits_kernel<<<(unsigned)vids.size(), 1024, 0, h->stream>>>(d_ref, d_vids, q);
  B2_CHECK_LAUNCH(h, "ref_bits_kernel");
  const size_t smem = (size_t)3 * max_runs * sizeof(int);
  B2_CUDA(h, cudaFuncSetAttribute(run_corr_kernel<false>, cudaFuncAttributeMaxDynamicSharedMemorySize, (int)smem));
  for (int r = 0; r < kGssEvals; ++r) {
    B2_TRY(b2i_gss_step_launch(h, r, T, d_trk, lane, r_score, d_sel, d_x, d_len,
                               out.evals, max_offset_samples, src.sample_rate));
    B2_TRY(b2i_raster_bits_dev_launch(h, cues, T, max_cues, d_x, d_len, sig_words, d_bits));
    run_corr_kernel<false><<<(unsigned)T, (unsigned)max_thr, smem, h->stream>>>(
        d_sel, d_job_q, q, d_bits, src.ref_label, max_runs, stat, cb.cand_off, B2Capture{}, 0);
    B2_CHECK_LAUNCH(h, "run_corr_kernel");
    B2_CUDA(h, cudaMemsetAsync(cb.work_count, 0, sizeof(int), h->stream));
    run_finalize_kernel<<<(unsigned)((T + 127) / 128), 128, 0, h->stream>>>(d_sel, T, 1, 0, stat, cb);
    B2_CHECK_LAUNCH(h, "run_finalize_kernel");
    B2_TRY(b2i_rescore_pick(h, d_sel, (size_t)T, d_ref, nullptr, d_bits, cb, r_score, r_offset, r_status));
  }
  return b2i_gss_combine_launch(h, T, K, d_trk, d_x, r_score, r_offset, max_offset_samples, out);
}
```

ffsubsync_b200/csrc/sync_plan.h:

```cpp
#pragma once

#include <math.h>
#include <stdlib.h>

#include <algorithm>
#include <cmath>
#include <string>
#include <vector>

#include "common.cuh"
#include "corr_jobs.cuh"
#include "job_plan.cuh"

static inline uint64_t magnitude_bits(double x) {
  uint64_t u;
  memcpy(&u, &x, 8);
  return u & 0x7fffffffffffffffull;
}

static inline double from_bits(uint64_t u) {
  double x;
  memcpy(&x, &u, 8);
  return x;
}

static inline bool cue_magnitude_ok(uint64_t max_bits, double r_max) {
  return from_bits(max_bits) * r_max < B2_MAX_CUE_SECONDS;
}

static inline bool ratio_ok(double r) { return r > 0.0 && r < INFINITY; }

static const char* bad_cue_input(const double* cue_start_s, const double* cue_end_s, const int64_t* cue_off,
                                 int B, const double* ratios, int K, int per_pair_ratios, double start_seconds,
                                 int64_t* at, double* val) {
  *at = -1;
  *val = start_seconds;
  if (!(fabs(start_seconds) < B2_MAX_CUE_SECONDS)) return "start_seconds is not finite or too large";
  for (int b = 0; b < B; ++b) {
    double r_max = 0.0;
    for (int k = 0; k < K; ++k) {
      const size_t i = per_pair_ratios ? (size_t)b * K + k : (size_t)k;
      *at = (int64_t)i;
      *val = ratios[i];
      if (!ratio_ok(ratios[i])) return "ratio is not a finite positive number";
      r_max = std::max(r_max, ratios[i]);
    }
    const int64_t c0 = cue_off[b], c1 = cue_off[b + 1];
    for (const double* t : {cue_start_s, cue_end_s}) {
      if (!t) continue;
      uint64_t m4[4] = {0, 0, 0, 0};
      int64_t c = c0;
      for (; c + 4 <= c1; c += 4)
        for (int i = 0; i < 4; ++i) m4[i] = std::max(m4[i], magnitude_bits(t[c + i]));
      for (; c < c1; ++c) m4[0] = std::max(m4[0], magnitude_bits(t[c]));
      if (cue_magnitude_ok(std::max(std::max(m4[0], m4[1]), std::max(m4[2], m4[3])), r_max)) continue;
      for (int64_t c = c0; c < c1; ++c)
        if (!cue_magnitude_ok(magnitude_bits(t[c]), r_max)) {
          *at = c;
          *val = t[c];
          return t == cue_start_s ? "cue start time times ratio is not finite or too large"
                                  : "cue end time times ratio is not finite or too large";
        }
    }
  }
  return nullptr;
}

static int rasterize_lengths(const double* cue_start_s, const double* cue_end_s, const int64_t* cue_off, int B,
                             const double* ratios, int K, int per_pair_ratios, int sample_rate, int64_t* lengths) {
  if (B < 0 || K < 0 || !cue_off || (!ratios && K) || !lengths || sample_rate <= 0)
    return B2_ERR_BAD_ARG;
  for (int b = 0; b < B; ++b) {
    const int64_t c0 = cue_off[b], c1 = cue_off[b + 1];
    const bool any = c1 > c0;
    double e4[4];
    uint64_t m4[4] = {0, 0, 0, 0};
    for (int i = 0; i < 4; ++i) e4[i] = any ? cue_end_s[c0] : 0.0;
    int64_t c = c0;
    for (; c + 4 <= c1; c += 4)
      for (int i = 0; i < 4; ++i) {
        e4[i] = std::max(e4[i], cue_end_s[c + i]);
        m4[i] = std::max(m4[i], magnitude_bits(cue_end_s[c + i]));
        if (cue_start_s) m4[i] = std::max(m4[i], magnitude_bits(cue_start_s[c + i]));
      }
    for (; c < c1; ++c) {
      e4[0] = std::max(e4[0], cue_end_s[c]);
      m4[0] = std::max(m4[0], magnitude_bits(cue_end_s[c]));
      if (cue_start_s) m4[0] = std::max(m4[0], magnitude_bits(cue_start_s[c]));
    }
    const double max_end = std::max(std::max(e4[0], e4[1]), std::max(e4[2], e4[3]));
    const uint64_t m = std::max(std::max(m4[0], m4[1]), std::max(m4[2], m4[3]));
    for (int k = 0; k < K; ++k) {
      double r = per_pair_ratios ? ratios[(size_t)b * K + k] : ratios[k];
      if (!ratio_ok(r) || !cue_magnitude_ok(m, r)) return B2_ERR_BAD_ARG;
      lengths[(size_t)b * K + k] = b2_signal_length(any ? max_end : 0.0, r, sample_rate);
    }
  }
  return B2_OK;
}

static int cue_lengths(std::string* err, const char* who, const char* what, const char* fallback,
                       const double* cue_start_s, const double* cue_end_s, const int64_t* cue_off, int B,
                       const double* ratios, int K, double start_seconds, int sample_rate, int64_t* lengths) {
  if (fabs(start_seconds) < B2_MAX_CUE_SECONDS &&
      rasterize_lengths(cue_start_s, cue_end_s, cue_off, B, ratios, K, 0, sample_rate, lengths) == B2_OK)
    return B2_OK;
  int64_t at;
  double val;
  const char* why = bad_cue_input(cue_start_s, cue_end_s, cue_off, B, ratios, K, 0, start_seconds, &at, &val);
  char b[512];
  if (why || !fallback)
    snprintf(b, sizeof(b), "%s: %s%s (index %lld: %g)", who, what, why ? why : "bad cue list", (long long)at, val);
  else
    snprintf(b, sizeof(b), "%s: %s", who, fallback);
  *err = b;
  return B2_ERR_BAD_ARG;
}

static inline int vad_frames_per_window(int frame_rate, int sample_rate) {
  if (frame_rate <= 0 || sample_rate <= 0) return 0;
  return (int)((1.0 / (double)sample_rate) * (double)frame_rate + 0.5);
}

static inline int auditok_block_size(int frame_rate, int sample_rate) {
  if (frame_rate <= 0 || sample_rate <= 0) return 0;
  volatile double dur = 1.0 / (double)sample_rate;
  volatile double prod = (double)frame_rate * dur;
  const int block = (int)prod;
  return block == frame_rate / sample_rate ? block : 0;
}

static inline int64_t auditok_energy_floor(int n_samples, double energy_threshold_db) {
  if (n_samples <= 0) return INT64_MAX;
  if (-200.0 >= energy_threshold_db) return 0;
  auto valid = [&](int64_t e) {
    volatile double energy = (double)e / (double)n_samples;
    volatile double le = 10.0 * log10(energy);
    return le >= energy_threshold_db;
  };
  const double guess = (double)n_samples * pow(10.0, energy_threshold_db / 10.0);
  const double e_max = (double)n_samples * 32768.0 * 32768.0;
  if (!(guess <= 2.0 * e_max)) return INT64_MAX;
  int64_t lo = 0, hi = (int64_t)guess + 1;
  while (!valid(hi)) {
    if ((double)hi > 4.0 * e_max) return INT64_MAX;
    hi *= 2;
  }
  while (hi - lo > 1) {
    const int64_t mid = lo + (hi - lo) / 2;
    if (valid(mid)) hi = mid;
    else lo = mid;
  }
  return hi;
}

static inline bool tokenizer_params_ok(double min_length, int64_t max_length, double max_continuous_silence,
                                       int64_t chunk_samples) {
  return max_length > 0 && min_length > 0 && min_length <= (double)max_length &&
         max_continuous_silence < (double)max_length && chunk_samples >= 0;
}

struct ChunkTable {
  std::vector<int64_t> pcm, out, tail, tok_off, tok_end;
  std::vector<int> first, tok_first;
};

static void build_chunk_table(const int64_t* pcm_off, int V, int64_t base, int fpw, int64_t chunk_samples,
                              double energy_threshold_db, const int64_t* subs_len, ChunkTable* ct) {
  ct->first.assign(V + 1, 0);
  ct->pcm.assign(1, V ? pcm_off[0] - base : 0);
  ct->out.assign(1, 0);
  if (subs_len) ct->tok_first.assign(V + 1, 0);
  int tail_rem = -1;
  int64_t tail_floor = 0;
  for (int v = 0; v < V; ++v) {
    const int64_t n = pcm_off[v + 1] - pcm_off[v];
    if (subs_len && subs_len[v] >= 0) {
      ct->pcm.push_back(pcm_off[v + 1] - base);
      ct->out.push_back(ct->out.back() + subs_len[v]);
      ct->tail.push_back(0);
    } else {
      const int64_t step = chunk_samples > 0 ? chunk_samples : (n > 0 ? n : 1);
      for (int64_t s = 0; s < n; s += step) {
        const int64_t len = std::min(step, n - s);
        ct->pcm.push_back(pcm_off[v] - base + s + len);
        ct->out.push_back(ct->out.back() + (len + fpw - 1) / fpw);
        const int rem = (int)(len % fpw);
        if (rem && rem != tail_rem) {
          tail_rem = rem;
          tail_floor = auditok_energy_floor(rem, energy_threshold_db);
        }
        ct->tail.push_back(rem ? tail_floor : 0);
        if (subs_len) {
          ct->tok_off.push_back(ct->out[ct->out.size() - 2]);
          ct->tok_end.push_back(ct->out.back());
        }
      }
    }
    ct->first[v + 1] = (int)ct->tail.size();
    if (subs_len) ct->tok_first[v + 1] = (int)ct->tok_off.size();
  }
}

struct SyncRequest {
  const char* who;
  const int16_t* pcm;
  const int64_t* pcm_off;
  int V;
  const int32_t* track_video;
  int T;
  int frame_rate, sample_rate;
  int detector;
  struct {
    float non_speech_label;
    int64_t energy_threshold;
    int z_lo, z_hi;
  } energy;
  struct {
    double non_speech_label, energy_threshold_db, min_length, max_continuous_silence;
    int64_t max_length, chunk_samples;
  } auditok;
  struct {
    const uint8_t* is_subs;
    const double* cue_start_s;
    const double* cue_end_s;
    const uint8_t* cue_keep;
    const int64_t* cue_off;
  } refs;
  const double* cue_start_s;
  const double* cue_end_s;
  const uint8_t* cue_keep;
  const int64_t* cue_off;
  const double* ratios;
  int K;
  double start_seconds;
  int64_t max_offset_samples;
  double* best_score;
  int32_t* best_offset;
  int32_t* best_k;
  double* all_score;
  int32_t* all_offset;
  bool search;
  double* gss_ratio;
  double* gss_evals;
  int memspace;
};

struct SyncPipeEnv {
  int sm_count, max_sub;
  const char* subbatches;
  const char* vad_sms;
  bool (*lane_eligible)(const int64_t* pcm_off, int n, int fpw);
};

struct SyncPlan {
  std::string err;
  bool gss = false, auditok = false, any_subs = false;
  int fpw = 0, z_lo = 0, z_hi = 0;
  float label = 0.0f, ref_label = 0.0f;
  bool two_level = false;
  int64_t audio_samples = 0;
  std::vector<int> trk_off;
  std::vector<int64_t> ref_off;
  std::vector<int64_t> sub_off;
  std::vector<int> sub_video;
  ChunkTable ch;
  int64_t auditok_e_min = 0;
  B2TokenizerParams tok{0.0, 0.0, 0.0, 0};
  std::vector<double> max_end;
  int n_sub = 1, vad_sms = 0;
  std::vector<int> cut;
};

static void plan_cuts(const SyncRequest& r, const SyncPipeEnv& env, SyncPlan* p) {
  const int V = r.V, T = r.T;
  const bool lane_ok = p->auditok ? env.lane_eligible(p->ch.pcm.data(), (int)p->ch.tail.size(), p->fpw)
                                  : env.lane_eligible(r.pcm_off, V, p->fpw);
  p->n_sub = 1;
  p->vad_sms = 0;
  if (T >= 96 && lane_ok) {
    p->n_sub = 3;
    p->vad_sms = (env.sm_count * 54 + 50) / 100;
  }
  if (env.subbatches) p->n_sub = std::max(1, std::min(T, atoi(env.subbatches)));
  if (env.vad_sms) p->vad_sms = std::max(0, std::min(env.sm_count, atoi(env.vad_sms)));
  p->n_sub = std::min(p->n_sub, env.max_sub);
  const std::vector<int>& trk_off = p->trk_off;
  p->cut.assign(1, 0);
  for (int i = 1; i < p->n_sub; ++i) {
    const int target = (int)((int64_t)T * i / p->n_sub);
    const int v = (int)(std::lower_bound(trk_off.begin(), trk_off.end(), target) - trk_off.begin());
    if (trk_off[v] > trk_off[p->cut.back()] && trk_off[v] < T) p->cut.push_back(v);
  }
  p->cut.push_back(V);
  p->n_sub = (int)p->cut.size() - 1;
}

static int plan_refs_check(const SyncRequest& r, SyncPlan* p, bool* any_audio) {
  const char* who = r.who;
  const auto& s = r.refs;
  for (int v = 0; v < r.V; ++v) {
    const bool is_subs = s.is_subs && s.is_subs[v];
    if (s.cue_off[v + 1] < s.cue_off[v]) B2_FAIL(p, B2_ERR_BAD_ARG, "%s: ref_cue_off not monotone at %d", who, v);
    if (!is_subs && s.cue_off[v + 1] != s.cue_off[v])
      B2_FAIL(p, B2_ERR_BAD_ARG, "%s: video %d has reference cues but no subtitle reference (ref_is_subs[%d] = 0)",
              who, v, v);
    if (is_subs && r.pcm_off[v + 1] != r.pcm_off[v])
      B2_FAIL(p, B2_ERR_BAD_ARG, "%s: video %d has a subtitle reference and a non-empty PCM range (%lld samples); "
              "its audio is never read", who, v, (long long)(r.pcm_off[v + 1] - r.pcm_off[v]));
    p->any_subs = p->any_subs || is_subs;
    *any_audio = *any_audio || !is_subs;
  }
  if (r.V > 0 && s.cue_off[r.V] > s.cue_off[0] && (!s.cue_start_s || !s.cue_end_s))
    B2_FAIL(p, B2_ERR_BAD_ARG, "%s: null reference cue arrays", who);
  if (p->audio_samples > 0 && !r.pcm)
    B2_FAIL(p, B2_ERR_BAD_ARG, "%s: null pcm with %lld samples of audio", who, (long long)p->audio_samples);
  return B2_OK;
}

static int plan_gss_check(const SyncRequest& r, SyncPlan* p, bool auditok_two_level) {
  const char* who = r.who;
  if (r.max_offset_samples == B2_MAX_OFFSET_NONE || r.max_offset_samples < 0 ||
      r.max_offset_samples > (int64_t)(kRunMaxWindow / 2))
    B2_FAIL(p, B2_ERR_UNSUPPORTED, "sync_tracks_gss: max_offset_samples must lie in [0, %d] (a window of at most "
            "2 max_offset_samples <= %d offsets, one CTA of the run path)", kRunMaxWindow / 2, kRunMaxWindow);
  if (!std::isfinite(p->ref_label))
    B2_FAIL(p, B2_ERR_UNSUPPORTED, "sync_tracks_gss: non_speech_label must be finite (the run path's two-level reference)");
  if (!p->two_level && !auditok_two_level)
    B2_FAIL(p, B2_ERR_UNSUPPORTED, "%s: non_speech_label = %g gives the auditok signal more than two levels; the "
            "search runs on the run path, which needs label 0", who, r.auditok.non_speech_label);
  if (!p->two_level)
    B2_FAIL(p, B2_ERR_UNSUPPORTED, "%s: subtitle references (levels 1 and 0) and audio references (levels 1 and "
            "non_speech_label = %g) in one call give three levels; the search runs on the run path, which needs "
            "label 0 or references of one kind", who, (double)p->label);
  for (int t = 0; t < r.T; ++t)
    if (r.cue_off[t + 1] - r.cue_off[t] > kRunMaxCues)
      B2_FAIL(p, B2_ERR_UNSUPPORTED, "sync_tracks_gss: track %d has %lld cues, more than %d", t,
              (long long)(r.cue_off[t + 1] - r.cue_off[t]), kRunMaxCues);
  return B2_OK;
}

static int plan_references(const SyncRequest& r, SyncPlan* p) {
  const char* who = r.who;
  const int V = r.V;
  if (p->auditok) {
    p->fpw = auditok_block_size(r.frame_rate, r.sample_rate);
    if (p->fpw <= 0)
      B2_FAIL(p, B2_ERR_UNSUPPORTED, "%s: int(frame_rate/sample_rate) block size and frame_rate//sample_rate window "
              "size differ (or are 0) for %d / %d", who, r.frame_rate, r.sample_rate);
    const auto& a = r.auditok;
    if (!tokenizer_params_ok(a.min_length, a.max_length, a.max_continuous_silence, a.chunk_samples))
      B2_FAIL(p, B2_ERR_BAD_ARG, "%s: bad tokenizer parameters", who);
    p->auditok_e_min = auditok_energy_floor(p->fpw, a.energy_threshold_db);
    p->tok = B2TokenizerParams{a.min_length, a.max_continuous_silence, a.non_speech_label, (long long)a.max_length};
  } else {
    p->fpw = vad_frames_per_window(r.frame_rate, r.sample_rate);
  }
  const int fpw = p->fpw;
  if (fpw <= 0) B2_FAIL(p, B2_ERR_BAD_ARG, "%s: bad frame_rate/sample_rate", who);
  p->z_lo = r.energy.z_lo < 0 ? 0 : r.energy.z_lo;
  p->z_hi = r.energy.z_hi < 0 ? (3 * fpw) / 8 : r.energy.z_hi;
  std::vector<int64_t> subs_len;
  if (p->any_subs) {
    const double one = 1.0;
    subs_len.resize(V);
    B2_TRY(cue_lengths(&p->err, who, "reference ", "bad reference cue list", r.refs.cue_start_s, r.refs.cue_end_s,
                       r.refs.cue_off, V, &one, 1, r.start_seconds, r.sample_rate, subs_len.data()));
    for (int v = 0; v < V; ++v) {
      if (r.refs.is_subs[v]) p->sub_video.push_back(v);
      else subs_len[v] = -1;
    }
  }
  p->ref_off.assign(V + 1, 0);
  for (int v = 0; v < V; ++v) {
    const int64_t n = r.pcm_off[v + 1] - r.pcm_off[v];
    if (n < 0) B2_FAIL(p, B2_ERR_BAD_ARG, "%s: pcm_off not monotone", who);
    if (p->any_subs && subs_len[v] >= 0) p->ref_off[v + 1] = p->ref_off[v] + subs_len[v];
    else if (!p->auditok) p->ref_off[v + 1] = p->ref_off[v] + (n + fpw - 1) / fpw;
  }
  if (p->auditok) {
    build_chunk_table(r.pcm_off, V, 0, fpw, r.auditok.chunk_samples, r.auditok.energy_threshold_db,
                      p->any_subs ? subs_len.data() : nullptr, &p->ch);
    for (int v = 0; v < V; ++v) p->ref_off[v + 1] = p->ch.out[p->ch.first[v + 1]];
  }
  return B2_OK;
}

static int plan_sync(const SyncRequest& r, const SyncPipeEnv& env, SyncPlan* p) {
  const char* who = r.who;
  const int V = r.V, T = r.T, K = r.K;
  p->gss = r.search;
  p->auditok = r.detector == B2_DETECTOR_AUDITOK;
  if (V < 0 || T < 0 || K <= 0 || !r.pcm_off || !r.cue_off || !r.ratios)
    B2_FAIL(p, B2_ERR_BAD_ARG, "%s: bad arguments", who);
  bool any_audio = !r.refs.cue_off;
  for (int v = 0; v < V; ++v)
    if (r.pcm_off[v + 1] > r.pcm_off[v]) p->audio_samples += r.pcm_off[v + 1] - r.pcm_off[v];
  if (r.refs.cue_off) B2_TRY(plan_refs_check(r, p, &any_audio));
  p->label = p->auditok ? (float)r.auditok.non_speech_label : r.energy.non_speech_label;
  p->ref_label = any_audio ? p->label : 0.0f;
  const bool auditok_two_level = !p->auditok || r.auditok.non_speech_label == 0.0;
  const bool mix_two_level = !p->any_subs || p->label == 0.0f;
  p->two_level = !any_audio || (auditok_two_level && mix_two_level);
  if (r.track_video) {
    for (int t = 0; t < T; ++t)
      if (r.track_video[t] < 0 || r.track_video[t] >= V || (t > 0 && r.track_video[t] < r.track_video[t - 1]))
        B2_FAIL(p, B2_ERR_BAD_ARG, "sync_tracks: track_video[%d] = %d is out of [0, %d) or decreases", t,
                (int)r.track_video[t], V);
    for (int t = 0; t < T; ++t)
      if (r.cue_off[t + 1] < r.cue_off[t]) B2_FAIL(p, B2_ERR_BAD_ARG, "sync_tracks: cue_off not monotone at %d", t);
  }
  if (p->gss) B2_TRY(plan_gss_check(r, p, auditok_two_level));
  if (T == 0) return B2_OK;
  if (!r.best_score || !r.best_offset || !r.best_k) B2_FAIL(p, B2_ERR_BAD_ARG, "%s: null output", who);
  if (p->gss && !r.gss_ratio) B2_FAIL(p, B2_ERR_BAD_ARG, "%s: null gss_ratio", who);
  B2_TRY(plan_references(r, p));
  p->trk_off.resize(V + 1);
  for (int v = 0, t = 0; v <= V; ++v) {
    if (r.track_video)
      while (t < T && r.track_video[t] < v) ++t;
    else
      t = v;
    p->trk_off[v] = t;
  }
  const size_t J = (size_t)T * K;
  std::vector<int64_t> lengths(J);
  B2_TRY(cue_lengths(&p->err, who, "", "bad cue list / ratios", r.cue_start_s, r.cue_end_s, r.cue_off, T, r.ratios,
                     K, r.start_seconds, r.sample_rate, lengths.data()));
  p->sub_off.assign(J + 1, 0);
  for (size_t j = 0; j < J; ++j) p->sub_off[j + 1] = p->sub_off[j] + lengths[j];
  if (p->gss) {
    const double r_hi = B2_GSS_HI;
    char what[32];
    snprintf(what, sizeof(what), "at ratio %g: ", r_hi);
    std::vector<int64_t> len_hi(T);
    B2_TRY(cue_lengths(&p->err, who, what, nullptr, r.cue_start_s, r.cue_end_s, r.cue_off, T,
                       &r_hi, 1, r.start_seconds, r.sample_rate, len_hi.data()));
    p->max_end.assign(T, 0.0);
    for (int t = 0; t < T; ++t)
      for (int64_t c = r.cue_off[t]; c < r.cue_off[t + 1]; ++c)
        p->max_end[t] = c == r.cue_off[t] ? r.cue_end_s[c] : std::max(p->max_end[t], r.cue_end_s[c]);
  }
  plan_cuts(r, env, p);
  return B2_OK;
}
```

ffsubsync_b200/csrc/vad.cu:

```cuda
#include "common.cuh"
#include "vad_group.cuh"
#include "vad_lane.cuh"

namespace {

constexpr int kConsumerThreads = 256;
constexpr int kMaxStages = 10;
constexpr int kLaneMaxStages = 24;
constexpr int kLaneBatch = 5;
constexpr int kLaneConsumers = 256;
constexpr int kLanePipes = 2;

struct TileDesc {
  long long out_base;
  long long n_left;
  long long span_gbyte;
  int n_windows;
  int sig;
  int head_bytes;
  int tail_src_off;
  int tail_end;
  int seq;
};

struct VadParams {
  const unsigned char* pcm_bytes;
  float* out;
  const long long* pcm_off;
  const long long* out_off;
  const long long* tile_off;
  unsigned long long* tile_counter;
  long long total_tiles;
  long long pcm_total_bytes;
  long long e_min;
  const long long* tail_emin;
  int B, fpw, G, tw, z_lo, z_hi, fast, stage_bytes, cpl, stages, consumers, batch, evict_first;
  float label;
};

__device__ __forceinline__ uint32_t smem_u32(const void* p) {
  return (uint32_t)__cvta_generic_to_shared(p);
}
__device__ __forceinline__ void mbar_init(uint64_t* bar, int count) {
  asm volatile("mbarrier.init.shared::cta.b64 [%0], %1;" ::"r"(smem_u32(bar)), "r"(count));
}
__device__ __forceinline__ void mbar_arrive_expect_tx(uint64_t* bar, uint32_t bytes) {
  asm volatile("mbarrier.arrive.expect_tx.shared::cta.b64 _, [%0], %1;" ::"r"(smem_u32(bar)),
               "r"(bytes)
               : "memory");
}
__device__ __forceinline__ void mbar_arrive(uint64_t* bar) {
  asm volatile("mbarrier.arrive.shared::cta.b64 _, [%0];" ::"r"(smem_u32(bar)) : "memory");
}
__device__ __forceinline__ void mbar_wait(uint64_t* bar, uint32_t parity) {
  asm volatile(
      "{\n\t"
      ".reg .pred p;\n\t"
      "WAIT_%=:\n\t"
      "mbarrier.try_wait.parity.shared::cta.b64 p, [%0], %1;\n\t"
      "@p bra DONE_%=;\n\t"
      "bra WAIT_%=;\n\t"
      "DONE_%=:\n\t"
      "}" ::"r"(smem_u32(bar)),
      "r"(parity)
      : "memory");
}
__device__ __forceinline__ void tma_bulk_g2s(void* dst, const void* src, uint32_t bytes,
                                             uint64_t* bar) {
  asm volatile(
      "cp.async.bulk.shared::cluster.global.mbarrier::complete_tx::bytes [%0], [%1], %2, [%3];" ::
          "r"(smem_u32(dst)),
      "l"(src), "r"(bytes), "r"(smem_u32(bar))
      : "memory");
}

template <int GT>
__device__ __forceinline__ void lane_group_sum(int G, long long& e, int& z) {
  if (GT > 0) {
#pragma unroll
    for (int off = GT >> 1; off > 0; off >>= 1) {
      e += __shfl_xor_sync(0xffffffffu, e, off);
      z += __shfl_xor_sync(0xffffffffu, z, off);
    }
  } else {
    for (int off = G >> 1; off > 0; off >>= 1) {
      e += __shfl_xor_sync(0xffffffffu, e, off);
      z += __shfl_xor_sync(0xffffffffu, z, off);
    }
  }
}

template <int CPL, int GT>
__device__ __forceinline__ void consume_tile_fast(const VadParams& p, const TileDesc& d,
                                                  const unsigned char* span, int g, int wl0,
                                                  int wstep) {
  const int fpw = p.fpw;
#pragma unroll 1
  for (int wl = wl0; wl < p.tw; wl += wstep) {
    long long e = 0;
    int z = 0;
    const bool active = wl < d.n_windows;
    const long long avail = d.n_left - (long long)wl * fpw;
    const bool full = active && avail >= fpw;
    const bool tail = active && !full && avail > 0 && p.tail_emin != nullptr;
    if (full) {
      vadgroup::window_part_fast<CPL>(span + (size_t)wl * fpw * 2, g, p.cpl, e, z);
    } else if (tail) {
      const short* xs = reinterpret_cast<const short*>(span + (size_t)wl * fpw * 2);
      for (int i = g; i < (int)avail; i += p.G) e += (long long)xs[i] * xs[i];
    }
    lane_group_sum<GT>(p.G, e, z);
    if (active && g == 0) {
      const bool speech = full ? (e >= p.e_min && z >= p.z_lo && z <= p.z_hi)
                               : (tail && e >= p.tail_emin[d.sig]);
      p.out[d.out_base + wl] = speech ? 1.0f : p.label;
    }
  }
}

__device__ __forceinline__ TileDesc make_tile(const VadParams& p, long long t, int& cur_b, uint32_t& bulk) {
  TileDesc d;
  while (t >= p.tile_off[cur_b + 1]) ++cur_b;
  const long long w0 = (t - p.tile_off[cur_b]) * p.tw;
  const long long sig0 = p.pcm_off[cur_b], sig1 = p.pcm_off[cur_b + 1];
  const long long nwin = p.out_off[cur_b + 1] - p.out_off[cur_b];
  const int nw = (int)min((long long)p.tw, nwin - w0);
  const long long s0 = sig0 + w0 * p.fpw;
  const long long s1 = min(s0 + (long long)nw * p.fpw, sig1);
  const long long b0 = 2 * s0, b1 = 2 * s1;
  const long long a0 = b0 & ~15LL;
  const long long a1 = (b1 + 15) & ~15LL;
  const long long limit = p.pcm_total_bytes & ~15LL;
  const long long bulk_end = min(a1, limit);
  bulk = bulk_end > a0 ? (uint32_t)(bulk_end - a0) : 0u;
  d.n_windows = nw;
  d.sig = cur_b;
  d.out_base = p.out_off[cur_b] + w0;
  d.n_left = sig1 - s0;
  d.head_bytes = (int)(b0 - a0);
  d.span_gbyte = a0;
  if (bulk_end < b1) {
    d.tail_src_off = (int)(max(bulk_end, a0) - a0);
    d.tail_end = (int)(b1 - a0);
  } else {
    d.tail_src_off = -1;
    d.tail_end = 0;
  }
  return d;
}
__device__ __forceinline__ TileDesc end_tile() {
  TileDesc d;
  d.n_windows = 0;
  d.sig = 0;
  d.out_base = d.n_left = d.span_gbyte = 0;
  d.head_bytes = 0;
  d.tail_src_off = -1;
  d.tail_end = 0;
  return d;
}

__global__ void __launch_bounds__(kConsumerThreads + 32) vad_energy_zcr_kernel(VadParams p) {
  extern __shared__ __align__(128) unsigned char smem[];
  unsigned char* data = smem;
  uint64_t* full_bar = reinterpret_cast<uint64_t*>(smem + (size_t)p.stages * p.stage_bytes);
  uint64_t* empty_bar = full_bar + kMaxStages;
  TileDesc* descs = reinterpret_cast<TileDesc*>(empty_bar + kMaxStages);

  const int nst = p.stages;
  const int tid = threadIdx.x;
  if (tid == 0) {
    for (int s = 0; s < kMaxStages; ++s) {
      mbar_init(&full_bar[s], 1);
      mbar_init(&empty_bar[s], kConsumerThreads / 32);
    }
    asm volatile("fence.mbarrier_init.release.cluster;" ::: "memory");
  }
  __syncthreads();

  if (tid >= kConsumerThreads) {
    if (tid != kConsumerThreads) return;
    int cur_b = 0, stage = 0;
    uint32_t round = 0;
    for (;; ++stage) {
      if (stage == nst) {
        stage = 0;
        ++round;
      }
      if (round > 0) mbar_wait(&empty_bar[stage], (round - 1) & 1u);
      const long long t = (long long)atomicAdd(p.tile_counter, 1ULL);
      TileDesc d;
      if (t >= p.total_tiles) {
        descs[stage] = end_tile();
        mbar_arrive(&full_bar[stage]);
        return;
      }
      uint32_t bulk;
      d = make_tile(p, t, cur_b, bulk);
      descs[stage] = d;
      if (bulk) {
        mbar_arrive_expect_tx(&full_bar[stage], bulk);
        tma_bulk_g2s(data + (size_t)stage * p.stage_bytes, p.pcm_bytes + d.span_gbyte, bulk, &full_bar[stage]);
      } else {
        mbar_arrive(&full_bar[stage]);
      }
    }
  }

  const int G = p.G;
  const int g = tid % G;
  const int wl0 = tid / G;
  const int wstep = kConsumerThreads / G;
  const int fpw = p.fpw;
  int stage = 0;
  uint32_t phase = 0;
  for (;;) {
    mbar_wait(&full_bar[stage], phase);
    const TileDesc d = descs[stage];
    if (d.n_windows == 0) break;
    unsigned char* span = data + (size_t)stage * p.stage_bytes;
    if (d.tail_src_off >= 0) {
      const int nb = d.tail_end - d.tail_src_off;
      if (tid < nb) span[d.tail_src_off + tid] = p.pcm_bytes[d.span_gbyte + d.tail_src_off + tid];
      asm volatile("bar.sync 1, %0;" ::"n"(kConsumerThreads) : "memory");
    }
    if (p.fast && d.head_bytes == 0) {
      if (p.cpl == 5 && G == 4) consume_tile_fast<5, 4>(p, d, span, g, wl0, wstep);
      else if (p.cpl == 15 && G == 4) consume_tile_fast<15, 4>(p, d, span, g, wl0, wstep);
      else consume_tile_fast<0, 0>(p, d, span, g, wl0, wstep);
    } else {
      for (int wl = wl0; wl < p.tw; wl += wstep) {
        long long e = 0;
        int z = 0;
        const bool active = wl < d.n_windows;
        const long long avail = d.n_left - (long long)wl * fpw;
        const bool full = active && avail >= fpw;
        const bool tail = active && !full && avail > 0 && p.tail_emin != nullptr;
        if (full || tail) {
          const short* xs = reinterpret_cast<const short*>(span + d.head_bytes + (size_t)wl * fpw * 2);
          const int n_use = full ? fpw : (int)avail;
          for (int i = g; i < n_use; i += G) {
            const int x = xs[i];
            const int px = i > 0 ? (int)xs[i - 1] : x;
            e += (long long)x * x;
            z += ((x < 0) != (px < 0));
          }
        }
        lane_group_sum<0>(G, e, z);
        if (active && g == 0) {
          const bool speech = full ? (e >= p.e_min && z >= p.z_lo && z <= p.z_hi)
                                   : (tail && e >= p.tail_emin[d.sig]);
          p.out[d.out_base + wl] = speech ? 1.0f : p.label;
        }
      }
    }
    __syncwarp();
    if ((tid & 31) == 0) mbar_arrive(&empty_bar[stage]);
    if (++stage == nst) {
      stage = 0;
      phase ^= 1u;
    }
  }
}

__device__ __forceinline__ void tma_bulk_g2s_stream(void* dst, const void* src, uint32_t bytes, uint64_t* bar,
                                                    uint64_t policy) {
  asm volatile(
      "cp.async.bulk.shared::cluster.global.mbarrier::complete_tx::bytes.L2::cache_hint [%0], [%1], %2, [%3], %4;" ::
          "r"(smem_u32(dst)),
      "l"(src), "r"(bytes), "r"(smem_u32(bar)), "l"(policy)
      : "memory");
}
__device__ __forceinline__ uint64_t l2_evict_first_policy() {
  uint64_t pol;
  asm volatile("createpolicy.fractional.L2::evict_first.b64 %0, 1.0;" : "=l"(pol));
  return pol;
}

struct SigCache {
  int b;
  long long tile_lo, tile_hi, sig0, sig1, nwin, out0;
};
__device__ __forceinline__ TileDesc make_tile_cached(const VadParams& p, long long t, SigCache& c, uint32_t& bulk) {
  if (c.b < 0 || t >= c.tile_hi) {
    int b = c.b < 0 ? 0 : c.b;
    while (t >= p.tile_off[b + 1]) ++b;
    c.b = b;
    c.tile_lo = p.tile_off[b];
    c.tile_hi = p.tile_off[b + 1];
    c.sig0 = p.pcm_off[b];
    c.sig1 = p.pcm_off[b + 1];
    c.out0 = p.out_off[b];
    c.nwin = p.out_off[b + 1] - c.out0;
  }
  TileDesc d;
  const long long w0 = (t - c.tile_lo) * p.tw;
  const long long s0 = c.sig0 + w0 * p.fpw;
  d.sig = c.b;
  d.out_base = c.out0 + w0;
  d.n_left = c.sig1 - s0;
  d.seq = 0;
  if (t + 1 < c.tile_hi) {
    d.n_windows = p.tw;
    d.head_bytes = 0;
    d.span_gbyte = 2 * s0;
    d.tail_src_off = -1;
    d.tail_end = 0;
    bulk = (uint32_t)(p.tw * p.fpw * 2);
    return d;
  }
  const int nw = (int)min((long long)p.tw, c.nwin - w0);
  const long long s1 = min(s0 + (long long)nw * p.fpw, c.sig1);
  const long long b0 = 2 * s0, b1 = 2 * s1;
  const long long a0 = b0 & ~15LL;
  const long long a1 = (b1 + 15) & ~15LL;
  const long long limit = p.pcm_total_bytes & ~15LL;
  const long long bulk_end = min(a1, limit);
  bulk = bulk_end > a0 ? (uint32_t)(bulk_end - a0) : 0u;
  d.n_windows = nw;
  d.head_bytes = (int)(b0 - a0);
  d.span_gbyte = a0;
  if (bulk_end < b1) {
    d.tail_src_off = (int)(max(bulk_end, a0) - a0);
    d.tail_end = (int)(b1 - a0);
  } else {
    d.tail_src_off = -1;
    d.tail_end = 0;
  }
  return d;
}

__device__ __forceinline__ long long claim_tiles(unsigned long long* counter, int n, int skew) {
  unsigned long long r;
  asm volatile("atom.global.add.u64 %0, [%1], %2;" : "=l"(r) : "l"(counter + skew), "l"((unsigned long long)n) : "memory");
  return (long long)r;
}

template <int C, int WPL>
__global__ void __launch_bounds__(kLaneConsumers + 32 * kLanePipes) vad_lane_kernel(VadParams p) {
  constexpr int RMAX = vadlane::rotation_max(C);
  constexpr int kWarps = kLaneConsumers / 32 / kLanePipes;
  extern __shared__ __align__(128) unsigned char smem[];
  const int nst = p.stages;
  const int tid = threadIdx.x;
  const int warp = tid >> 5;
  const bool is_producer = tid >= kLaneConsumers;
  const int pipe = is_producer ? warp - kLaneConsumers / 32 : warp / kWarps;
  uint64_t* bar0 = reinterpret_cast<uint64_t*>(smem + (size_t)kLanePipes * nst * p.stage_bytes);
  TileDesc* desc0 = reinterpret_cast<TileDesc*>(bar0 + 2 * kLaneMaxStages);
  unsigned char* data = smem + (size_t)pipe * nst * p.stage_bytes;
  uint64_t* full_bar = bar0 + pipe * nst;
  uint64_t* empty_bar = bar0 + kLaneMaxStages + pipe * nst;
  TileDesc* descs = desc0 + pipe * nst;
  volatile int* zeros = reinterpret_cast<volatile int*>(desc0 + kLaneMaxStages);
  if (tid == 0) {
    for (int s = 0; s < kLaneMaxStages; ++s) {
      mbar_init(&bar0[s], 1);
      mbar_init(&bar0[kLaneMaxStages + s], 1);
      desc0[s].seq = -1;
    }
    for (int i = 0; i < 8; ++i) zeros[i] = 0;
    asm volatile("fence.mbarrier_init.release.cluster;" ::: "memory");
  }
  __syncthreads();

  if (is_producer) {
    const int lane = tid & 31;
    SigCache sc;
    sc.b = -1;
    int q0 = 0;
    int stage0 = 0;
    uint32_t round = 0;
    int ends_left = kWarps;
    long long pending = 0;
    const int skew = zeros[lane & 7];
    const uint64_t l2_policy = l2_evict_first_policy();
    if (lane == 0) pending = claim_tiles(p.tile_counter, p.batch, skew);
    for (;;) {
      const long long t0 = __shfl_sync(0xffffffffu, pending, 0);
      const int n = (int)max(0LL, min((long long)p.batch, p.total_tiles - t0));
      if (n > 0 && lane == 0) pending = claim_tiles(p.tile_counter, p.batch, skew);
      const int count = n > 0 ? n : min(ends_left, p.batch);
      if (lane < count) {
        TileDesc d = end_tile();
        uint32_t bulk = 0;
        if (n > 0) d = make_tile_cached(p, t0 + lane, sc, bulk);
        d.seq = q0 + lane;
        int stage = stage0 + lane;
        uint32_t rnd = round;
        if (stage >= nst) {
          stage -= nst;
          ++rnd;
        }
        if (rnd > 0) mbar_wait(&empty_bar[stage], (rnd - 1) & 1u);
        descs[stage] = d;
        if (bulk) {
          mbar_arrive_expect_tx(&full_bar[stage], bulk);
          if (p.evict_first)
            tma_bulk_g2s_stream(data + (size_t)stage * p.stage_bytes, p.pcm_bytes + d.span_gbyte, bulk,
                                &full_bar[stage], l2_policy);
          else
            tma_bulk_g2s(data + (size_t)stage * p.stage_bytes, p.pcm_bytes + d.span_gbyte, bulk, &full_bar[stage]);
        } else {
          mbar_arrive(&full_bar[stage]);
        }
      }
      __syncwarp();
      q0 += count;
      stage0 += count;
      if (stage0 >= nst) {
        stage0 -= nst;
        ++round;
      }
      if (n == 0) {
        ends_left -= count;
        if (ends_left == 0) return;
      }
    }
  }

  const int lane = tid & 31;
  const int rot = vadlane::lane_rotation(C, lane);
  constexpr int fpw = 8 * C;
  int q = warp - pipe * kWarps;
  int stage = q;
  uint32_t phase = 0;
  for (;;) {
    while (*reinterpret_cast<volatile int*>(&descs[stage].seq) != q) {
    }
    mbar_wait(&full_bar[stage], phase);
    const TileDesc d = descs[stage];
    if (d.n_windows == 0) break;
    unsigned char* span = data + (size_t)stage * p.stage_bytes;
    if (d.tail_src_off >= 0) {
      const int nb = d.tail_end - d.tail_src_off;
      if (lane < nb) span[d.tail_src_off + lane] = p.pcm_bytes[d.span_gbyte + d.tail_src_off + lane];
      __syncwarp();
    }
#pragma unroll 1
    for (int k = 0; k < WPL; ++k) {
      const int wl = lane + 32 * k;
      const bool active = wl < d.n_windows;
      const long long avail = d.n_left - (long long)wl * fpw;
      const bool full = active && avail >= fpw;
      long long e = 0;
      int z = 0;
      bool speech = false;
      if (full) {
        vadlane::lane_window<C, RMAX>(span + (size_t)wl * (fpw * 2), rot, e, z);
        speech = e >= p.e_min && z >= p.z_lo && z <= p.z_hi;
      } else if (active && avail > 0 && p.tail_emin != nullptr) {
        const short* xs = reinterpret_cast<const short*>(span + (size_t)wl * (fpw * 2));
        for (int i = 0; i < (int)avail; ++i) e += (long long)xs[i] * xs[i];
        speech = e >= p.tail_emin[d.sig];
      }
      if (active) p.out[d.out_base + wl] = speech ? 1.0f : p.label;
    }
    __syncwarp();
    if (lane == 0) mbar_arrive(&empty_bar[stage]);
    q += kWarps;
    stage += kWarps;
    if (stage >= nst) {
      stage -= nst;
      phase ^= 1u;
    }
  }
}

__device__ __forceinline__ uint32_t lowbias32(uint32_t x) {
  x ^= x >> 16;
  x *= 0x7feb352du;
  x ^= x >> 15;
  x *= 0x846ca68bu;
  x ^= x >> 16;
  return x;
}

__global__ void __launch_bounds__(256) synth_pcm_kernel(const uint8_t* __restrict__ cls,
                                                         long long n_windows, int fpw,
                                                         uint32_t seed, short* __restrict__ out) {
  const long long n = n_windows * (long long)fpw;
  for (long long i = (long long)blockIdx.x * blockDim.x + threadIdx.x; i < n;
       i += (long long)gridDim.x * blockDim.x) {
    const long long w = i / fpw;
    const int pos = (int)(i - w * fpw);
    const uint32_t hsh = lowbias32(((uint32_t)i) ^ seed);
    const int c = cls[w];
    int v;
    if (c == 0)
      v = (int)((hsh >> 26) & 0x3fu) - 32;
    else if (c == 1)
      v = ((((pos / 40) & 1) == 0) ? 6000 : -6000) + (int)((hsh >> 14) & 0xfffu) - 2048;
    else
      v = (int)(hsh & 0x3fffu) - 8192;
    out[i] = (short)v;
  }
}

}

int b2i_synth_launch(b2_ctx* h, const uint8_t* d_cls, int64_t n_windows, int fpw, uint32_t seed,
                     int16_t* d_out) {
  long long n = n_windows * (long long)fpw;
  int blocks = (int)std::min<long long>((n + 255) / 256, (long long)h->sm_count * 16);
  synth_pcm_kernel<<<blocks, 256, 0, h->stream>>>(d_cls, n_windows, fpw, seed, (short*)d_out);
  B2_CHECK_LAUNCH(h, "synth_pcm_kernel");
  return B2_OK;
}

bool b2i_vad_lane_eligible(const int64_t* pcm_off, int B, int fpw) {
  if (fpw != 80 && fpw != 160) return false;
  if (const char* e = getenv("B2_VAD_LAYOUT"))
    if (strcmp(e, "group") == 0) return false;
  for (int b = 0; b < B; ++b)
    if (pcm_off[b + 1] > pcm_off[b] && pcm_off[b] % 8 != 0) return false;
  return true;
}

int b2i_vad_launch(b2_ctx* h, const int16_t* d_pcm, const int64_t* pcm_off, int B, int fpw,
                   float non_speech_label, int64_t e_min_full, int z_lo, int z_hi,
                   float* d_out, const int64_t* out_off, const int64_t* tail_emin) {
  B2Range range("b2:vad_energy_zcr");
  if (((uintptr_t)d_pcm & 15) != 0)
    B2_FAIL(h, B2_ERR_BAD_ARG, "vad: device PCM pointer must be 16-byte aligned");
  VadParams p;
  p.consumers = kConsumerThreads;
  const int C = fpw / 8;
  p.fast = (fpw % 8 == 0) ? 1 : 0;
  int G = 0, best_score = -1;
  for (int g = 32; g >= 2 && p.fast; g >>= 1) {
    if (C % g != 0) continue;
    const int cpl = C / g;
    const long long tile = (long long)(kConsumerThreads / g) * fpw * 2;
    const int score = ((cpl & 1) ? 4 : 0) + (tile <= 65536 ? 2 : 0) + (cpl >= 3 ? 1 : 0);
    if (score > best_score) { best_score = score; G = g; }
  }
  if (G == 0) {
    p.fast = 0;
    G = 4;
    if (C > 32) G = 8;
    if (C > 64) G = 16;
    if (C > 128) G = 32;
  }
  p.G = G;
  p.cpl = p.fast ? C / G : 0;
  int wpt = 1;
  if (const char* e = getenv("B2_VAD_WPT")) wpt = std::max(1, std::min(8, atoi(e)));
  p.fpw = fpw;
  int stages = 4;
  if (const char* e = getenv("B2_VAD_STAGES")) stages = std::max(2, std::min(kMaxStages, atoi(e)));
  for (;;) {
    p.tw = wpt * (kConsumerThreads / G);
    p.stage_bytes = ((p.tw * fpw * 2 + 32) + 127) & ~127;
    if ((size_t)stages * p.stage_bytes <= 200 * 1024) break;
    if (wpt > 1) --wpt;
    else if (stages > 2) --stages;
    else break;
  }
  p.stages = stages;
  size_t smem = (size_t)stages * p.stage_bytes + 2 * kMaxStages * sizeof(uint64_t) +
                kMaxStages * sizeof(TileDesc) + 64;
  if (smem > 227 * 1024) B2_FAIL(h, B2_ERR_UNSUPPORTED, "vad: window of %d samples too large", fpw);

  std::vector<long long> tile_off(B + 1);
  tile_off[0] = 0;
  bool aligned = true;
  for (int b = 0; b < B; ++b) {
    long long n = pcm_off[b + 1] - pcm_off[b];
    long long nwin = (n + fpw - 1) / fpw;
    tile_off[b + 1] = tile_off[b] + (nwin + p.tw - 1) / p.tw;
    if (n > 0 && pcm_off[b] % 8 != 0) aligned = false;
  }
  if (!aligned) p.fast = 0;
  bool lane_layout = p.fast && (C == 10 || C == 20);
  if (const char* e = getenv("B2_VAD_LAYOUT")) lane_layout = lane_layout && strcmp(e, "group") != 0;
  int wpl = C == 10 ? 2 : 1;
  if (const char* e = getenv("B2_VAD_WPL")) wpl = (C == 10 ? 2 : 1) * (atoi(e) >= 2 ? 2 : 1);
  if (lane_layout) {
    p.tw = 32 * wpl;
    p.stage_bytes = ((p.tw * fpw * 2 + 32) + 127) & ~127;
    stages = std::min<int>(kLaneMaxStages, (int)((208 * 1024) / p.stage_bytes)) / kLanePipes;
    if (const char* e = getenv("B2_VAD_STAGES"))
      stages = std::max(kLaneConsumers / 32 / kLanePipes, std::min(stages, atoi(e)));
    p.consumers = kLaneConsumers;
    p.stages = stages;
    p.evict_first = 1;
    if (const char* e = getenv("B2_VAD_EVICT_FIRST")) p.evict_first = atoi(e) != 0;
    p.batch = kLaneBatch;
    if (const char* e = getenv("B2_VAD_BATCH")) p.batch = std::max(1, std::min(16, atoi(e)));
    p.batch = std::min(p.batch, stages);
    smem = (size_t)kLanePipes * stages * p.stage_bytes + 2 * kLaneMaxStages * sizeof(uint64_t) +
           kLaneMaxStages * sizeof(TileDesc) + 64;
    for (int b = 0; b < B; ++b) {
      const long long n = pcm_off[b + 1] - pcm_off[b];
      tile_off[b + 1] = tile_off[b] + ((n + fpw - 1) / fpw + p.tw - 1) / p.tw;
    }
  }
  p.total_tiles = tile_off[B];
  if (p.total_tiles == 0) return B2_OK;

  MetaArena a;
  size_t tbl = (size_t)(B + 1) * 8;
  B2_TRY(b2i_meta_begin(h, &a, 4 * tbl + 256));
  p.pcm_off = (const long long*)b2i_meta_put(&a, pcm_off, tbl);
  p.out_off = (const long long*)b2i_meta_put(&a, out_off, tbl);
  p.tile_off = (const long long*)b2i_meta_put(&a, tile_off.data(), tbl);
  p.tail_emin = tail_emin ? (const long long*)b2i_meta_put(&a, tail_emin, (size_t)B * 8) : nullptr;
  B2_TRY(b2i_meta_commit(&a));

  p.pcm_bytes = (const unsigned char*)d_pcm;
  p.out = d_out;
  p.B = B;
  p.pcm_total_bytes = 2 * (long long)pcm_off[B];
  p.e_min = (long long)e_min_full;
  p.z_lo = z_lo;
  p.z_hi = z_hi;
  p.label = non_speech_label;

  void* d_counter;
  B2_TRY(b2i_ws(h, b2_ctx::WS_COUNTERS, 64, &d_counter));
  p.tile_counter = (unsigned long long*)d_counter;
  B2_CUDA(h, cudaMemsetAsync(d_counter, 0, 8, h->stream));
  if (lane_layout) {
    void (*lk)(VadParams) = C == 10 ? (wpl == 2 ? vad_lane_kernel<10, 2> : vad_lane_kernel<10, 4>)
                                    : (wpl == 1 ? vad_lane_kernel<20, 1> : vad_lane_kernel<20, 2>);
    if (smem < 116 * 1024) smem = 116 * 1024;
    B2_CUDA(h, cudaFuncSetAttribute(lk, cudaFuncAttributeMaxDynamicSharedMemorySize, (int)smem));
    long long grid = std::min<long long>((p.total_tiles + kLanePipes * p.batch - 1) / (kLanePipes * p.batch), (long long)h->sm_count);
    if (h->vad_partition_sms > 0) grid = std::min<long long>(grid, h->vad_partition_sms);
    lk<<<(unsigned)grid, kLaneConsumers + 32 * kLanePipes, smem, h->stream>>>(p);
    B2_CHECK_LAUNCH(h, "vad_lane_kernel");
    return B2_OK;
  }
  B2_CUDA(h, cudaFuncSetAttribute(vad_energy_zcr_kernel, cudaFuncAttributeMaxDynamicSharedMemorySize, (int)smem));
  int per_sm = (int)std::max<size_t>(1, std::min<size_t>(4, (220 * 1024) / smem));
  if (const char* f = getenv("B2_VAD_CTAS_FORCE")) per_sm = std::max(1, atoi(f));
  const long long grid = std::min<long long>(p.total_tiles, (long long)h->sm_count * per_sm);
  vad_energy_zcr_kernel<<<(unsigned)grid, kConsumerThreads + 32, smem, h->stream>>>(p);
  B2_CHECK_LAUNCH(h, "vad_energy_zcr_kernel");
  return B2_OK;
}
```

Measured before the change: 12460.

## Emit bit-packed VAD reference when the run-length alignment path is selected

When planning selects the runs alignment path, the VAD kernel writes the reference speech mask as warp-ballot 32-bit words instead of one float per window. The ref-table build then scans packed words directly, and the rescore kernel reads reference bits from that packed array. The aim is to cut reference write and read traffic by roughly 32x. In exchange, the alignment-path planning is hoisted into a shared header so it can run at sync-plan time, and each kernel involved gets a second code path.

```diff
diff --git a/__graft_entry__.py b/__graft_entry__.py
--- a/__graft_entry__.py
+++ b/__graft_entry__.py
@@ -13,6 +13,7 @@
 EMUL_RASTER = os.path.join(ROOT, "tests", "host_emul", "raster_emul")
 EMUL_GSS = os.path.join(ROOT, "tests", "host_emul", "gss_emul")
 EMUL_PLAN = os.path.join(ROOT, "tests", "host_emul", "plan_emul")
+EMUL_REF_FORMAT = os.path.join(ROOT, "tests", "host_emul", "ref_format_emul")
 
 NVCC_FLAGS = [
     "-gencode", "arch=compute_90a,code=sm_90a", "-lineinfo", "-O3", "-std=c++17",
@@ -67,10 +68,11 @@
                                                                os.path.join(CSRC, "raster_math.cuh")])):
         subprocess.check_call([nvcc, "-O2", "-std=c++17", "-Xcompiler", "-ffp-contract=off",
                                "-Wno-deprecated-gpu-targets", "-o", EMUL_GSS, gss_src])
-    plan_src = EMUL_PLAN + ".cu"
-    if os.path.exists(plan_src) and (force or _stale(EMUL_PLAN, [plan_src] + hdrs)):
-        subprocess.check_call([nvcc, "-O2", "-std=c++17", "-Xcompiler", "-ffp-contract=off",
-                               "-Wno-deprecated-gpu-targets", "-o", EMUL_PLAN, plan_src])
+    for emul in (EMUL_PLAN, EMUL_REF_FORMAT):
+        emul_src = emul + ".cu"
+        if os.path.exists(emul_src) and (force or _stale(emul, [emul_src] + hdrs)):
+            subprocess.check_call([nvcc, "-O2", "-std=c++17", "-Xcompiler", "-ffp-contract=off",
+                                   "-Wno-deprecated-gpu-targets", "-o", emul, emul_src])
     vad_src = EMUL_VAD + ".cu"
     if os.path.exists(vad_src) and (force or _stale(EMUL_VAD, [vad_src, os.path.join(CSRC, "vad_lane.cuh"),
                                                                os.path.join(CSRC, "vad_group.cuh")])):
diff --git a/ffsubsync_b200/csrc/align_path.h b/ffsubsync_b200/csrc/align_path.h
--- /dev/null
+++ b/ffsubsync_b200/csrc/align_path.h
@@ -0,0 +1,146 @@
+#pragma once
+
+#include <stdlib.h>
+#include <string.h>
+
+#include <algorithm>
+#include <cmath>
+#include <string>
+#include <vector>
+
+#include "common.cuh"
+#include "corr_jobs.cuh"
+#include "job_plan.cuh"
+
+constexpr int kAlignBlock = 32768;
+
+enum B2AlignPath { B2_PATH_TILED = 0, B2_PATH_BIG = 1, B2_PATH_RUNS = 2 };
+
+struct B2AlignPairPlan {
+  long long o_min, o_max;
+  int n_tiles;
+  bool any;
+};
+
+struct B2AlignJobs {
+  std::string err;
+  std::vector<SelJob> sel;
+  std::vector<long long> idx_lo, idx_hi, n_pad;
+  std::vector<long long> bits_off;
+  std::vector<B2AlignPairPlan> pp;
+  long long max_w = 1;
+  bool big_ok = true;
+  int Wt = 0, L = 0;
+};
+
+static int b2_plan_align_jobs(const int64_t* ref_off, int V, const int* trk_off, const int64_t* sub_off, int B, int K,
+                              int64_t max_offset_samples, uint64_t quirk_mask, const double* cue_ratios,
+                              B2AlignJobs* a) {
+  const size_t J = (size_t)B * K;
+  const bool cue_mode = cue_ratios != nullptr;
+  a->bits_off.assign(cue_mode ? J + 1 : 1, 0);
+  if (cue_mode)
+    for (size_t j = 0; j < J; ++j)
+      a->bits_off[j + 1] = a->bits_off[j] + ((sub_off[j + 1] - sub_off[j]) + kAlignBlock) / 32 + 1;
+  a->sel.assign(J, SelJob{});
+  a->idx_lo.assign(J, 0);
+  a->idx_hi.assign(J, 0);
+  a->n_pad.assign(J, 0);
+  a->pp.assign(V, B2AlignPairPlan{});
+  a->max_w = 1;
+  a->big_ok = true;
+  const long long mo_clamped =
+      std::max<long long>(-(1LL << 40), std::min<long long>(1LL << 40, max_offset_samples));
+  for (int v = 0; v < V; ++v) {
+    const long long R = ref_off[v + 1] - ref_off[v];
+    if (R < 0 || R > 0x3fffffff) B2_FAIL(a, B2_ERR_BAD_ARG, "align: bad reference length at %d", v);
+    B2AlignPairPlan& p = a->pp[v];
+    p.any = false;
+    p.o_min = 0;
+    p.o_max = -1;
+    for (int b = trk_off[v]; b < trk_off[v + 1]; ++b) {
+      long long t_min = 0, t_max = -1;
+      bool t_any = false;
+      for (int k = 0; k < K; ++k) {
+        const size_t j = (size_t)b * K + k;
+        const long long S = sub_off[j + 1] - sub_off[j];
+        if (S < 0 || S > 0x3fffffff) B2_FAIL(a, B2_ERR_BAD_ARG, "align: bad subtitle length at %zu", j);
+        SelJob& s = a->sel[j];
+        memset(&s, 0, sizeof(s));
+        s.ref_off = ref_off[v];
+        s.sub_off = sub_off[j];
+        s.R = (int)R;
+        s.S = (int)S;
+        s.out_index = (int)j;
+        s.bits_off = cue_mode ? a->bits_off[j] : -1;
+        s.sub_level = cue_mode ? (float)std::min(1.0 / cue_ratios[k], 1.0) : 0.f;
+        const B2JobPlan jp = b2_plan_job(R, S, max_offset_samples, quirk_mask);
+        if (jp.kind != 0) {
+          s.kind = jp.kind;
+          s.masked_offset = jp.masked_offset;
+          continue;
+        }
+        const long long N = jp.N, o_lo = jp.o_lo, o_hi = jp.o_hi;
+        a->idx_lo[j] = jp.lo;
+        a->idx_hi[j] = jp.hi;
+        a->n_pad[j] = N;
+        if (N < (1LL << kBigMinLog2n) || N > (1LL << kBigMaxLog2n)) a->big_ok = false;
+        s.kind = 0;
+        s.m_lo = (int)o_lo;
+        s.m_hi = (int)o_hi;
+        t_min = t_any ? std::min(t_min, o_lo) : o_lo;
+        t_max = t_any ? std::max(t_max, o_hi) : o_hi;
+        t_any = true;
+      }
+      if (!t_any) continue;
+      p.o_min = p.any ? std::min(p.o_min, t_min) : t_min;
+      p.o_max = p.any ? std::max(p.o_max, t_max) : t_max;
+      p.any = true;
+      if (max_offset_samples != B2_MAX_OFFSET_NONE && std::max(llabs(t_min), llabs(t_max)) > mo_clamped)
+        for (int k = 0; k < K; ++k) a->sel[(size_t)b * K + k].no_prune = 1;
+    }
+    if (p.any) a->max_w = std::max(a->max_w, p.o_max - p.o_min + 1);
+  }
+  a->Wt = (int)(a->max_w <= kAlignBlock / 2 + 1 ? 32 * ((a->max_w + 30) / 32) + 1 : (kAlignBlock / 2 + 1));
+  a->L = kAlignBlock - a->Wt + 1;
+  return B2_OK;
+}
+
+struct B2AlignPathChoice {
+  int path;
+  int max_runs;
+};
+
+static B2AlignPathChoice b2_align_path(const B2AlignJobs& a, const int* trk_off, int V, int K, const int64_t* cue_off,
+                                       bool ref_two_level, float ref_label, const char* align_path, bool capture) {
+  bool use_big = a.big_ok && a.max_w > (long long)kBigMinTiles * (kAlignBlock / 2 + 1);
+  const bool force_runs = align_path && !strcmp(align_path, "runs");
+  const bool force_tiled = align_path && !strcmp(align_path, "tiled");
+  if (force_tiled || force_runs) use_big = false;
+  if (align_path && !strcmp(align_path, "big") && a.big_ok) use_big = true;
+  B2AlignPathChoice c{use_big ? B2_PATH_BIG : B2_PATH_TILED, 1};
+  if (!cue_off || (capture && !force_runs) || use_big || !ref_two_level || !std::isfinite(ref_label) || force_tiled)
+    return c;
+  bool fits = true, pays = true;
+  int max_runs = 1;
+  for (int v = 0; v < V && fits; ++v) {
+    const B2AlignPairPlan& p = a.pp[v];
+    const long long n_tiles_v = p.any ? ceil_div64(p.o_max - p.o_min + 1, a.Wt) : 0;
+    for (int b = trk_off[v]; b < trk_off[v + 1]; ++b) {
+      const long long cues = cue_off[b + 1] - cue_off[b];
+      for (int k = 0; k < K; ++k) {
+        const SelJob& s = a.sel[(size_t)b * K + k];
+        if (s.kind != 0) continue;
+        const long long w = (long long)s.m_hi - s.m_lo + 1;
+        if (w > kRunMaxWindow || cues > kRunMaxCues || llabs((long long)s.m_lo) > (1LL << 30) ||
+            llabs((long long)s.m_hi) > (1LL << 30))
+          fits = false;
+        if ((double)cues * (double)w > kRunCostPerBlock * (double)(n_tiles_v * (ceil_div64(s.S, a.L) + 1)))
+          pays = false;
+        max_runs = std::max<int>(max_runs, (int)std::min<long long>(cues, kRunMaxCues));
+      }
+    }
+  }
+  if (fits && (pays || force_runs)) c = B2AlignPathChoice{B2_PATH_RUNS, max_runs};
+  return c;
+}
diff --git a/ffsubsync_b200/csrc/api.cu b/ffsubsync_b200/csrc/api.cu
--- a/ffsubsync_b200/csrc/api.cu
+++ b/ffsubsync_b200/csrc/api.cu
@@ -801,7 +801,8 @@
   int winner_only;
 };
 
-static int enqueue_chain(b2_ctx* h, const SyncRequest& r, const SyncPlan& p, const SyncBufs& b, int v0, int v1) {
+static int enqueue_chain(b2_ctx* h, const SyncRequest& r, const SyncPlan& p, const SyncBufs& b, int v0, int v1,
+                         bool ref_packed) {
   const int K = r.K, t0 = p.trk_off[v0], nt = p.trk_off[v1] - t0;
   const size_t j0 = (size_t)t0 * K;
   std::vector<int> chain_trk(v1 - v0 + 1);
@@ -810,7 +811,7 @@
     B2_TRY(b2i_raster_launch(h, r.cue_start_s, r.cue_end_s, r.cue_keep, r.cue_off + t0, nt, r.ratios, K, 0, nullptr,
                              r.sample_rate, r.start_seconds, b.subsig, p.sub_off.data() + j0));
   const B2CueSource src{r.cue_start_s, r.cue_end_s, r.cue_keep, r.cue_off + t0, r.ratios, r.sample_rate,
-                        r.start_seconds, p.ref_label, p.two_level};
+                        r.start_seconds, p.ref_label, p.two_level, ref_packed};
   B2_TRY(b2i_align_launch(h, b.refsig, p.ref_off.data() + v0, v1 - v0, chain_trk.data(), b.subsig,
                           p.sub_off.data() + j0, nt, K, r.max_offset_samples, b.score + j0, b.offset + j0,
                           b.status + j0, b.winner_only, b.fused ? &src : nullptr, (long long)j0));
@@ -825,10 +826,12 @@
                         p.max_end.data() + t0, r.max_offset_samples, go);
 }
 
-static int detect(b2_ctx* h, const SyncRequest& r, const SyncPlan& p, const SyncBufs& b, int v0, int v1) {
+static int detect(b2_ctx* h, const SyncRequest& r, const SyncPlan& p, const SyncBufs& b, int v0, int v1,
+                  bool ref_packed) {
   if (!p.auditok) {
     B2_TRY(b2i_vad_launch(h, b.pcm, r.pcm_off + v0, v1 - v0, p.fpw, r.energy.non_speech_label,
-                          (int64_t)p.fpw * r.energy.energy_threshold, p.z_lo, p.z_hi, b.refsig, p.ref_off.data() + v0));
+                          (int64_t)p.fpw * r.energy.energy_threshold, p.z_lo, p.z_hi, b.refsig, p.ref_off.data() + v0,
+                          nullptr, ref_packed));
   } else {
     const ChunkTable& ch = p.ch;
     const int c0 = ch.first[v0], nc = ch.first[v1] - c0;
@@ -856,8 +859,8 @@
   const int n_sub = p.n_sub;
   const std::vector<int>& cut = p.cut;
   if (n_sub == 1) {
-    B2_TRY(detect(h, r, p, b, 0, r.V));
-    return enqueue_chain(h, r, p, b, 0, r.V);
+    B2_TRY(detect(h, r, p, b, 0, r.V, p.ref_packed[0]));
+    return enqueue_chain(h, r, p, b, 0, r.V, p.ref_packed[0]);
   }
   std::vector<cudaEvent_t> vad_done(n_sub);
   cudaEvent_t inputs_ready = next_event(h);
@@ -883,7 +886,7 @@
     for (int i = 0; i < n_sub; ++i) {
       h->vad_partition_sms = (i > 0 || prev_busy) ? p.vad_sms : 0;
       if (trace) B2_CUDA(h, cudaEventRecord(tev[1 + 4 * i], h->stream));
-      const int st = detect(h, r, p, b, cut[i], cut[i + 1]);
+      const int st = detect(h, r, p, b, cut[i], cut[i + 1], p.ref_packed[i]);
       h->vad_partition_sms = 0;
       if (st != B2_OK) return st;
       vad_done[i] = next_event(h);
@@ -896,7 +899,7 @@
     if (resident && i == n_sub - 1) B2_CUDA(h, cudaEventRecord(h->resident_fence, h->stream));
     B2_CUDA(h, cudaStreamWaitEvent(h->stream, vad_done[i], 0));
     if (trace) B2_CUDA(h, cudaEventRecord(tev[3 + 4 * i], h->stream));
-    B2_TRY(enqueue_chain(h, r, p, b, cut[i], cut[i + 1]));
+    B2_TRY(enqueue_chain(h, r, p, b, cut[i], cut[i + 1], p.ref_packed[i]));
     if (trace) B2_CUDA(h, cudaEventRecord(tev[4 + 4 * i], h->stream));
     host_ms[i + 1] = host_now();
   }
@@ -925,8 +928,14 @@
 
 static int sync_run(b2_ctx* h, bool fence_was_valid, const SyncRequest& r) {
   SyncPlan p;
-  const SyncPipeEnv env{h->sm_count, b2_ctx::kEvents - 2, getenv("B2_SUBBATCHES"), getenv("B2_VAD_SMS"),
-                        b2i_vad_lane_eligible};
+  SyncPipeEnv env{h->sm_count, b2_ctx::kEvents - 2, getenv("B2_SUBBATCHES"), getenv("B2_VAD_SMS"),
+                  b2i_vad_lane_eligible};
+  env.quirk_mask = h->log2_quirk_mask;
+  env.capture = h->capture.scores != nullptr;
+  env.align_path = getenv("B2_ALIGN_PATH");
+  env.fused = true;
+  if (const char* e = getenv("B2_FUSED_RASTER")) env.fused = atoi(e) != 0;
+  env.ref_packed = getenv("B2_REF_PACKED");
   if (const int st = plan_sync(r, env, &p)) {
     h->err = p.err;
     return st;
@@ -949,8 +958,7 @@
     B2_CHECK_DEV(h, memspace, r.gss_evals, "sync_tracks_gss: gss_evals");
   }
   SyncBufs b{};
-  b.fused = true;
-  if (const char* e = getenv("B2_FUSED_RASTER")) b.fused = atoi(e) != 0;
+  b.fused = env.fused;
   const size_t J = (size_t)T * K, JG = (size_t)T * (K + 1);
   void *d_refsig, *d_subsig = nullptr, *d_res;
   const bool chained = resident && fence_was_valid;
diff --git a/ffsubsync_b200/csrc/bigfft.cu b/ffsubsync_b200/csrc/bigfft.cu
--- a/ffsubsync_b200/csrc/bigfft.cu
+++ b/ffsubsync_b200/csrc/bigfft.cu
@@ -7,8 +7,8 @@
 #include "bigfft.cuh"
 #include "corr_jobs.cuh"
 
-int bigfft_min_log2n() { return bigfft::kMinQ1 + 11; }
-int bigfft_max_log2n() { return bigfft::kMaxQ1 + 11; }
+static_assert(kBigMinLog2n == bigfft::kMinQ1 + 11 && kBigMaxLog2n == bigfft::kMaxQ1 + 11,
+              "padded lengths of the large-window path");
 
 namespace {
 
diff --git a/ffsubsync_b200/csrc/common.cuh b/ffsubsync_b200/csrc/common.cuh
--- a/ffsubsync_b200/csrc/common.cuh
+++ b/ffsubsync_b200/csrc/common.cuh
@@ -141,7 +141,8 @@
 bool b2i_vad_lane_eligible(const int64_t* pcm_off_host, int B, int fpw);
 int b2i_vad_launch(b2_ctx* h, const int16_t* d_pcm, const int64_t* pcm_off_host, int B, int fpw,
                    float non_speech_label, int64_t e_min_full, int z_lo, int z_hi,
-                   float* d_out, const int64_t* out_off_host, const int64_t* tail_emin_host = nullptr);
+                   float* d_out, const int64_t* out_off_host, const int64_t* tail_emin_host = nullptr,
+                   bool packed = false);
 struct B2TokenizerParams {
   double min_length, max_continuous_silence, non_speech_label;
   long long max_length;
@@ -173,6 +174,7 @@
   double start_seconds;
   float ref_label;
   bool ref_two_level;
+  bool ref_packed = false;
 };
 int b2i_raster_bits_launch(b2_ctx* h, const B2CueSource* src, int B, int K, const int64_t* sig_off,
                            const long long* bits_off, uint32_t* d_bits);
diff --git a/ffsubsync_b200/csrc/corr.cu b/ffsubsync_b200/csrc/corr.cu
--- a/ffsubsync_b200/csrc/corr.cu
+++ b/ffsubsync_b200/csrc/corr.cu
@@ -3,6 +3,7 @@
 #include <algorithm>
 #include <cmath>
 
+#include "align_path.h"
 #include "common.cuh"
 #include "corr.cuh"
 #include "corr_jobs.cuh"
@@ -11,6 +12,7 @@
 namespace {
 
 using namespace corr;
+static_assert(kP == kAlignBlock, "overlap-save block of the host planner");
 
 struct SpecItem {
   long long ref_off;
@@ -381,6 +383,7 @@
   if (tid < scount) work_list[swarp[0] + tid] = (j << 5) | tid;
 }
 
+template <bool PACKED_REF>
 __global__ void __launch_bounds__(256) rescore_kernel(const SelJob* __restrict__ jobs,
                                                        const float* __restrict__ ref,
                                                        const float* __restrict__ sub,
@@ -388,7 +391,7 @@
                                                        const int* __restrict__ work_list,
                                                        const int* __restrict__ work_count,
                                                        const uint32_t* __restrict__ sub_bits,
-                                                       double* __restrict__ cand_partial) {
+                                                       double* __restrict__ cand_partial, float ref_label) {
   __shared__ double sh[256];
   const int total = *work_count * kRescoreSeg;
   for (int w = blockIdx.x; w < total; w += gridDim.x) {
@@ -404,7 +407,29 @@
     const int a0 = j_lo + seg * per, a1 = min(j_hi, a0 + per);
     double acc = 0.0;
     int i = a0 + threadIdx.x;
-    if (job.bits_off >= 0) {
+    if (PACKED_REF) {
+      const uint32_t* bits = sub_bits + job.bits_off;
+      const uint32_t* rbits = reinterpret_cast<const uint32_t*>(ref) + job.ref_off;
+      const double hi = 2.0 * (double)job.sub_level - 1.0;
+      const int rsh = (i + o) & 31;
+      for (; i + 7 * 256 < a1; i += 8 * 256) {
+        uint32_t bw[8];
+        float rv[8];
+#pragma unroll
+        for (int u = 0; u < 8; ++u) {
+          bw[u] = __ldg(bits + ((i + u * 256) >> 5));
+          rv[u] = ((__ldg(rbits + ((i + u * 256 + o) >> 5)) >> rsh) & 1u) ? 1.0f : ref_label;
+        }
+#pragma unroll
+        for (int u = 0; u < 8; ++u)
+          acc = fma(((bw[u] >> (i & 31)) & 1u) ? hi : -1.0, 2.0 * (double)rv[u] - 1.0, acc);
+      }
+      for (; i < a1; i += 256) {
+        const double a = ((__ldg(bits + (i >> 5)) >> (i & 31)) & 1u) ? hi : -1.0;
+        const float rv = ((__ldg(rbits + ((i + o) >> 5)) >> rsh) & 1u) ? 1.0f : ref_label;
+        acc = fma(a, 2.0 * (double)rv - 1.0, acc);
+      }
+    } else if (job.bits_off >= 0) {
       const uint32_t* bits = sub_bits + job.bits_off;
       const double hi = 2.0 * (double)job.sub_level - 1.0;
       for (; i + 7 * 256 < a1; i += 8 * 256) {
@@ -570,76 +595,23 @@
     V = B;
   }
   const bool cue_mode = cue_src != nullptr;
-  std::vector<long long> bits_off(cue_mode ? J + 1 : 1, 0);
-  if (cue_mode)
-    for (size_t j = 0; j < J; ++j)
-      bits_off[j + 1] = bits_off[j] + ((sub_off[j + 1] - sub_off[j]) + kP) / 32 + 1;
-  std::vector<SelJob> sel(J);
-  std::vector<long long> idx_lo(J, 0), idx_hi(J, 0), n_pad(J, 0);
-  struct PairPlan { long long o_min, o_max; int n_tiles; bool any; };
-  std::vector<PairPlan> pp(V);
-  long long max_w = 1;
-  bool big_ok = true;
-  const long long mo_clamped =
-      std::max<long long>(-(1LL << 40), std::min<long long>(1LL << 40, max_offset_samples));
-  for (int v = 0; v < V; ++v) {
-    const long long R = ref_off[v + 1] - ref_off[v];
-    if (R < 0 || R > 0x3fffffff) B2_FAIL(h, B2_ERR_BAD_ARG, "align: bad reference length at %d", v);
-    PairPlan& p = pp[v];
-    p.any = false;
-    p.o_min = 0;
-    p.o_max = -1;
-    for (int b = trk_off[v]; b < trk_off[v + 1]; ++b) {
-      long long t_min = 0, t_max = -1;
-      bool t_any = false;
-      for (int k = 0; k < K; ++k) {
-        const size_t j = (size_t)b * K + k;
-        const long long S = sub_off[j + 1] - sub_off[j];
-        if (S < 0 || S > 0x3fffffff) B2_FAIL(h, B2_ERR_BAD_ARG, "align: bad subtitle length at %zu", j);
-        SelJob& s = sel[j];
-        memset(&s, 0, sizeof(s));
-        s.ref_off = ref_off[v];
-        s.sub_off = sub_off[j];
-        s.R = (int)R;
-        s.S = (int)S;
-        s.out_index = (int)j;
-        s.bits_off = cue_mode ? bits_off[j] : -1;
-        s.sub_level = cue_mode ? (float)std::min(1.0 / cue_src->ratios[k], 1.0) : 0.f;
-        const B2JobPlan jp = b2_plan_job(R, S, max_offset_samples, h->log2_quirk_mask);
-        if (jp.kind != 0) {
-          s.kind = jp.kind;
-          s.masked_offset = jp.masked_offset;
-          continue;
-        }
-        const long long N = jp.N, o_lo = jp.o_lo, o_hi = jp.o_hi;
-        idx_lo[j] = jp.lo;
-        idx_hi[j] = jp.hi;
-        n_pad[j] = N;
-        if (N < (1LL << (bigfft_min_log2n())) || N > (1LL << bigfft_max_log2n())) big_ok = false;
-        s.kind = 0;
-        s.m_lo = (int)o_lo;
-        s.m_hi = (int)o_hi;
-        t_min = t_any ? std::min(t_min, o_lo) : o_lo;
-        t_max = t_any ? std::max(t_max, o_hi) : o_hi;
-        t_any = true;
-      }
-      if (!t_any) continue;
-      p.o_min = p.any ? std::min(p.o_min, t_min) : t_min;
-      p.o_max = p.any ? std::max(p.o_max, t_max) : t_max;
-      p.any = true;
-      if (max_offset_samples != B2_MAX_OFFSET_NONE && std::max(llabs(t_min), llabs(t_max)) > mo_clamped)
-        for (int k = 0; k < K; ++k) sel[(size_t)b * K + k].no_prune = 1;
-    }
-    if (p.any) max_w = std::max(max_w, p.o_max - p.o_min + 1);
-  }
+  B2AlignJobs aj;
+  if (const int st = b2_plan_align_jobs(ref_off, V, trk_off, sub_off, B, K, max_offset_samples, h->log2_quirk_mask,
+                                        cue_mode ? cue_src->ratios : nullptr, &aj)) {
+    h->err = aj.err;
+    return st;
+  }
+  std::vector<SelJob>& sel = aj.sel;
+  const std::vector<long long>& bits_off = aj.bits_off;
+  std::vector<B2AlignPairPlan>& pp = aj.pp;
+  const long long max_w = aj.max_w;
   const bool capture = h->capture.scores != nullptr;
   if (capture)
     for (size_t j = 0; j < J; ++j)
       if (sel[j].kind == 0 && (long long)sel[j].m_hi - sel[j].m_lo + 1 > h->capture.stride)
         B2_FAIL(h, B2_ERR_BAD_ARG, "capture: job %lld has %lld surviving offsets, stride %lld",
                 capture_j0 + (long long)j, (long long)sel[j].m_hi - sel[j].m_lo + 1, h->capture.stride);
-  const int Wt = (int)(max_w <= kP / 2 + 1 ? 32 * ((max_w + 30) / 32) + 1 : (kP / 2 + 1));
-  const int L = kP - Wt + 1;
+  const int Wt = aj.Wt, L = aj.L;
   uint32_t* d_bits = nullptr;
   if (cue_mode) {
     void* db;
@@ -660,51 +632,30 @@
   cb.work_count = cb.work_list + J * kCandMax;
   if (J >= (1u << 26)) B2_FAIL(h, B2_ERR_UNSUPPORTED, "align: B*K too large for one call");
 
-  bool use_big = big_ok && max_w > (long long)kBigMinTiles * (kP / 2 + 1);
-  const char* path_env = getenv("B2_ALIGN_PATH");
-  const bool force_runs = path_env && !strcmp(path_env, "runs");
-  if (path_env) {
-    if (!strcmp(path_env, "tiled") || force_runs) use_big = false;
-    if (!strcmp(path_env, "big") && big_ok) use_big = true;
-  }
-  if (cue_mode && (!capture || force_runs) && !use_big && cue_src->ref_two_level && std::isfinite(cue_src->ref_label) &&
-      !(path_env && !strcmp(path_env, "tiled"))) {
-    bool fits = true, pays = true;
-    int max_runs = 1;
-    for (int v = 0; v < V && fits; ++v) {
-      const long long n_tiles_v = pp[v].any ? ceil_div64(pp[v].o_max - pp[v].o_min + 1, Wt) : 0;
-      for (int b = trk_off[v]; b < trk_off[v + 1]; ++b) {
-        const long long cues = cue_src->cue_off[b + 1] - cue_src->cue_off[b];
-        for (int k = 0; k < K; ++k) {
-          const SelJob& s = sel[(size_t)b * K + k];
-          if (s.kind != 0) continue;
-          const long long w = (long long)s.m_hi - s.m_lo + 1;
-          if (w > kRunMaxWindow || cues > kRunMaxCues || llabs((long long)s.m_lo) > (1LL << 30) ||
-              llabs((long long)s.m_hi) > (1LL << 30))
-            fits = false;
-          if ((double)cues * (double)w > kRunCostPerBlock * (double)(n_tiles_v * (ceil_div64(s.S, L) + 1)))
-            pays = false;
-          max_runs = std::max<int>(max_runs, (int)std::min<long long>(cues, kRunMaxCues));
-        }
-      }
-    }
-    if (fits && (pays || force_runs)) {
-      const SelJob* d_sel_runs = nullptr;
-      B2_TRY(b2i_align_runs(h, d_ref, ref_off, V, trk_off, K, sel, d_bits, max_runs, cue_src->ref_label, winner_only,
-                            cb, &d_sel_runs, capture_j0));
-      return b2i_rescore_pick(h, d_sel_runs, J, d_ref, d_sub, d_bits, cb, d_score, d_offset, d_status);
-    }
-  }
-  if (use_big) {
+  const B2AlignPathChoice path =
+      b2_align_path(aj, trk_off, V, K, cue_mode ? cue_src->cue_off : nullptr, cue_mode && cue_src->ref_two_level,
+                    cue_mode ? cue_src->ref_label : 0.0f, getenv("B2_ALIGN_PATH"), capture);
+  const bool ref_packed = cue_mode && cue_src->ref_packed;
+  if (ref_packed && path.path != B2_PATH_RUNS)
+    B2_FAIL(h, B2_ERR_UNSUPPORTED, "align: internal error: packed reference on a chain that takes the %s path",
+            path.path == B2_PATH_BIG ? "large-window" : "tiled");
+  if (path.path == B2_PATH_RUNS) {
+    const SelJob* d_sel_runs = nullptr;
+    B2_TRY(b2i_align_runs(h, d_ref, ref_off, V, trk_off, K, sel, d_bits, path.max_runs, cue_src->ref_label,
+                          winner_only, ref_packed, cb, &d_sel_runs, capture_j0));
+    return b2i_rescore_pick(h, d_sel_runs, J, d_ref, d_sub, d_bits, cb, d_score, d_offset, d_status, ref_packed,
+                            cue_src->ref_label);
+  }
+  if (path.path == B2_PATH_BIG) {
     const SelJob* d_sel_big = nullptr;
-    B2_TRY(b2i_align_big(h, d_ref, d_sub, d_bits, V, trk_off, K, sel, idx_lo, idx_hi, n_pad, winner_only, cb,
-                         &d_sel_big, capture_j0));
+    B2_TRY(b2i_align_big(h, d_ref, d_sub, d_bits, V, trk_off, K, sel, aj.idx_lo, aj.idx_hi, aj.n_pad, winner_only,
+                         cb, &d_sel_big, capture_j0));
     return b2i_rescore_pick(h, d_sel_big, J, d_ref, d_sub, d_bits, cb, d_score, d_offset, d_status);
   }
 
   long long n_jobs_total = 0, max_blocks = 1;
   for (int v = 0; v < V; ++v) {
-    PairPlan& p = pp[v];
+    B2AlignPairPlan& p = pp[v];
     p.n_tiles = p.any ? (int)ceil_div64(p.o_max - p.o_min + 1, Wt) : 0;
     for (size_t j = (size_t)trk_off[v] * K; j < (size_t)trk_off[v + 1] * K; ++j) {
       const SelJob& s = sel[j];
@@ -720,7 +671,7 @@
   if (const char* e = getenv("B2_ALIGN_SPLIT")) n_split = std::max(1, atoi(e));
   long long score_total = 0, energy_total = 0, max_score_len = 0;
   for (int v = 0; v < V; ++v) {
-    PairPlan& p = pp[v];
+    B2AlignPairPlan& p = pp[v];
     for (size_t j = (size_t)trk_off[v] * K; j < (size_t)trk_off[v + 1] * K; ++j) {
       SelJob& s = sel[j];
       if (s.kind != 0) continue;
@@ -787,7 +738,7 @@
   };
 
   for (int v = 0; v < V; ++v) {
-    const PairPlan& p = pp[v];
+    const B2AlignPairPlan& p = pp[v];
     if (!p.any) continue;
     const long long R = ref_off[v + 1] - ref_off[v];
     const size_t j_lo = (size_t)trk_off[v] * K, j_hi = (size_t)trk_off[v + 1] * K;
@@ -855,9 +806,10 @@
 
 int b2i_rescore_pick(b2_ctx* h, const SelJob* d_sel, size_t J, const float* d_ref, const float* d_sub,
                      const uint32_t* d_bits, const B2CandBuffers& cb, double* d_score, int32_t* d_offset,
-                     int32_t* d_status) {
-  rescore_kernel<<<(unsigned)(h->sm_count * 8), 256, 0, h->stream>>>(
-      d_sel, d_ref, d_sub, cb.cand_off, cb.work_list, cb.work_count, d_bits, cb.cand_partial);
+                     int32_t* d_status, bool ref_packed, float ref_label) {
+  auto rescore = ref_packed ? rescore_kernel<true> : rescore_kernel<false>;
+  rescore<<<(unsigned)(h->sm_count * 8), 256, 0, h->stream>>>(
+      d_sel, d_ref, d_sub, cb.cand_off, cb.work_list, cb.work_count, d_bits, cb.cand_partial, ref_label);
   B2_CHECK_LAUNCH(h, "rescore_kernel");
   pick_kernel<<<(unsigned)((J + 127) / 128), 128, 0, h->stream>>>(d_sel, (int)J, cb.cand_off, cb.cand_cnt,
                                                                    cb.cand_partial, cb.job_stat, d_score,
diff --git a/ffsubsync_b200/csrc/corr_jobs.cuh b/ffsubsync_b200/csrc/corr_jobs.cuh
--- a/ffsubsync_b200/csrc/corr_jobs.cuh
+++ b/ffsubsync_b200/csrc/corr_jobs.cuh
@@ -31,8 +31,7 @@
 
 
 constexpr int kBigMinTiles = 4;
-int bigfft_min_log2n();
-int bigfft_max_log2n();
+constexpr int kBigMinLog2n = 17, kBigMaxLog2n = 23;
 
 struct B2CandBuffers {
   double* cand_partial;
@@ -46,12 +45,12 @@
                       int n_chunks, int K, int winner_only, int* chunk_cnt, const B2CandBuffers& cb);
 int b2i_rescore_pick(b2_ctx* h, const SelJob* d_sel, size_t J, const float* d_ref, const float* d_sub,
                      const uint32_t* d_bits, const B2CandBuffers& cb, double* d_score, int32_t* d_offset,
-                     int32_t* d_status);
+                     int32_t* d_status, bool ref_packed = false, float ref_label = 0.0f);
 int b2i_capture_launch(b2_ctx* h, const SelJob* d_sel, const int* d_jlist, int n, const float* scores,
                        const B2CandBuffers& cb, long long j0, bool scores_written = false);
 int b2i_align_runs(b2_ctx* h, const float* d_ref, const int64_t* ref_off, int V, const int* trk_off, int K,
                    std::vector<SelJob>& sel, const uint32_t* d_bits, int max_runs, float ref_label, int winner_only,
-                   const B2CandBuffers& cb, const SelJob** d_sel_out, long long capture_j0);
+                   bool ref_packed, const B2CandBuffers& cb, const SelJob** d_sel_out, long long capture_j0);
 constexpr double kRunCostPerBlock = 5.6e5;
 constexpr int kRunMaxCues = 16384;
 constexpr int kRunMaxWindow = 32 * 1024;
diff --git a/ffsubsync_b200/csrc/runcorr.cu b/ffsubsync_b200/csrc/runcorr.cu
--- a/ffsubsync_b200/csrc/runcorr.cu
+++ b/ffsubsync_b200/csrc/runcorr.cu
@@ -85,6 +85,40 @@
     if (w < n_words) q[w + 1] = make_uint2(mine, (uint32_t)(carry + ex));
     carry += tot;
   }
+}
+
+__global__ void __launch_bounds__(1024) ref_words_scan_kernel(const uint32_t* __restrict__ ref_words,
+                                                              const RunRef* __restrict__ vids,
+                                                              uint2* __restrict__ q_all) {
+  __shared__ int sh[33];
+  const RunRef v = vids[blockIdx.x];
+  const uint32_t* r = ref_words + v.ref_off;
+  uint2* q = q_all + v.q_off;
+  const int n_in = (v.R + 31) >> 5;
+  const int n_words = (v.R >> 5) + 2;
+  if (threadIdx.x == 0) q[0] = make_uint2(0u, 0u);
+  int carry = 0;
+  for (int w0 = 0; w0 < n_words; w0 += blockDim.x) {
+    const int w = w0 + threadIdx.x;
+    const uint32_t mine = w < n_in ? __ldg(r + w) : 0u;
+    int tot;
+    const int ex = block_excl_scan(__popc(mine), sh, &tot);
+    if (w < n_words) q[w + 1] = make_uint2(mine, (uint32_t)(carry + ex));
+    carry += tot;
+  }
+}
+
+int launch_ref_table(b2_ctx* h, const float* d_ref, bool ref_packed, const RunRef* d_vids, size_t n_vids, uint2* q) {
+  if (n_vids == 0) return B2_OK;
+  if (ref_packed) {
+    ref_words_scan_kernel<<<(unsigned)n_vids, 1024, 0, h->stream>>>(reinterpret_cast<const uint32_t*>(d_ref), d_vids,
+                                                                    q);
+    B2_CHECK_LAUNCH(h, "ref_words_scan_kernel");
+  } else {
+    ref_bits_kernel<<<(unsigned)n_vids, 1024, 0, h->stream>>>(d_ref, d_vids, q);
+    B2_CHECK_LAUNCH(h, "ref_bits_kernel");
+  }
+  return B2_OK;
 }
 
 template <bool CAPTURE>
@@ -252,8 +286,8 @@
 
 int b2i_align_runs(b2_ctx* h, const float* d_ref, const int64_t* ref_off, int V, const int* trk_off, int K,
                    std::vector<SelJob>& sel, const uint32_t* d_bits, int max_runs, float ref_label, int winner_only,
-                   const B2CandBuffers& cb, const SelJob** d_sel_out, long long capture_j0) {
-  B2Range range("b2:align runs (ref_bits, run_corr, finalize)");
+                   bool ref_packed, const B2CandBuffers& cb, const SelJob** d_sel_out, long long capture_j0) {
+  B2Range range("b2:align runs (ref_bits or ref_words_scan, run_corr, finalize)");
   const size_t J = sel.size();
   std::vector<RunRef> vids;
   std::vector<long long> job_q(J, 0);
@@ -290,10 +324,7 @@
   const RunRef* d_vids = vids.empty() ? nullptr : (const RunRef*)b2i_meta_put(&a, vids.data(), vids.size() * sizeof(RunRef));
   B2_TRY(b2i_meta_commit(&a));
   *d_sel_out = d_sel;
-  if (!vids.empty()) {
-    ref_bits_kernel<<<(unsigned)vids.size(), 1024, 0, h->stream>>>(d_ref, d_vids, q);
-    B2_CHECK_LAUNCH(h, "ref_bits_kernel");
-  }
+  B2_TRY(launch_ref_table(h, d_ref, ref_packed, d_vids, vids.size(), q));
   max_runs = std::max(1, max_runs);
   const size_t smem = (size_t)3 * max_runs * sizeof(int);
   const bool capture = h->capture.scores != nullptr;
@@ -393,8 +424,7 @@
   const RunRef* d_vids = (const RunRef*)b2i_meta_put(&a, vids.data(), vids.size() * sizeof(RunRef));
   B2_TRY(b2i_meta_commit(&a));
 
-  ref_bits_kernel<<<(unsigned)vids.size(), 1024, 0, h->stream>>>(d_ref, d_vids, q);
-  B2_CHECK_LAUNCH(h, "ref_bits_kernel");
+  B2_TRY(launch_ref_table(h, d_ref, src.ref_packed, d_vids, vids.size(), q));
   const size_t smem = (size_t)3 * max_runs * sizeof(int);
   B2_CUDA(h, cudaFuncSetAttribute(run_corr_kernel<false>, cudaFuncAttributeMaxDynamicSharedMemorySize, (int)smem));
   for (int r = 0; r < kGssEvals; ++r) {
@@ -407,7 +437,8 @@
     B2_CUDA(h, cudaMemsetAsync(cb.work_count, 0, sizeof(int), h->stream));
     run_finalize_kernel<<<(unsigned)((T + 127) / 128), 128, 0, h->stream>>>(d_sel, T, 1, 0, stat, cb);
     B2_CHECK_LAUNCH(h, "run_finalize_kernel");
-    B2_TRY(b2i_rescore_pick(h, d_sel, (size_t)T, d_ref, nullptr, d_bits, cb, r_score, r_offset, r_status));
+    B2_TRY(b2i_rescore_pick(h, d_sel, (size_t)T, d_ref, nullptr, d_bits, cb, r_score, r_offset, r_status,
+                            src.ref_packed, src.ref_label));
   }
   return b2i_gss_combine_launch(h, T, K, d_trk, d_x, r_score, r_offset, max_offset_samples, out);
 }
diff --git a/ffsubsync_b200/csrc/sync_plan.h b/ffsubsync_b200/csrc/sync_plan.h
--- a/ffsubsync_b200/csrc/sync_plan.h
+++ b/ffsubsync_b200/csrc/sync_plan.h
@@ -8,6 +8,7 @@
 #include <string>
 #include <vector>
 
+#include "align_path.h"
 #include "common.cuh"
 #include "corr_jobs.cuh"
 #include "job_plan.cuh"
@@ -251,6 +252,11 @@
   const char* subbatches;
   const char* vad_sms;
   bool (*lane_eligible)(const int64_t* pcm_off, int n, int fpw);
+  uint64_t quirk_mask = 0;
+  bool capture = false;
+  const char* align_path = nullptr;
+  bool fused = true;
+  const char* ref_packed = nullptr;
 };
 
 struct SyncPlan {
@@ -270,6 +276,7 @@
   std::vector<double> max_end;
   int n_sub = 1, vad_sms = 0;
   std::vector<int> cut;
+  std::vector<uint8_t> ref_packed;
 };
 
 static void plan_cuts(const SyncRequest& r, const SyncPipeEnv& env, SyncPlan* p) {
@@ -294,6 +301,27 @@
   }
   p->cut.push_back(V);
   p->n_sub = (int)p->cut.size() - 1;
+}
+
+static void plan_ref_format(const SyncRequest& r, const SyncPipeEnv& env, SyncPlan* p) {
+  p->ref_packed.assign(p->n_sub, 0);
+  if (p->auditok || !env.fused || (env.ref_packed && atoi(env.ref_packed) == 0)) return;
+  for (int i = 0; i < p->n_sub; ++i) {
+    const int v0 = p->cut[i], v1 = p->cut[i + 1];
+    const auto& sv = p->sub_video;
+    if (std::lower_bound(sv.begin(), sv.end(), v0) != std::lower_bound(sv.begin(), sv.end(), v1)) continue;
+    if (!env.lane_eligible(r.pcm_off + v0, v1 - v0, p->fpw)) continue;
+    const int t0 = p->trk_off[v0], nt = p->trk_off[v1] - t0;
+    std::vector<int> chain_trk(v1 - v0 + 1);
+    for (int v = v0; v <= v1; ++v) chain_trk[v - v0] = p->trk_off[v] - t0;
+    B2AlignJobs aj;
+    if (b2_plan_align_jobs(p->ref_off.data() + v0, v1 - v0, chain_trk.data(), p->sub_off.data() + (size_t)t0 * r.K,
+                           nt, r.K, r.max_offset_samples, env.quirk_mask, r.ratios, &aj) != B2_OK)
+      continue;
+    const B2AlignPathChoice c = b2_align_path(aj, chain_trk.data(), v1 - v0, r.K, r.cue_off + t0, p->two_level,
+                                              p->ref_label, env.align_path, env.capture);
+    p->ref_packed[i] = c.path == B2_PATH_RUNS;
+  }
 }
 
 static int plan_refs_check(const SyncRequest& r, SyncPlan* p, bool* any_audio) {
@@ -442,5 +470,6 @@
         p->max_end[t] = c == r.cue_off[t] ? r.cue_end_s[c] : std::max(p->max_end[t], r.cue_end_s[c]);
   }
   plan_cuts(r, env, p);
+  plan_ref_format(r, env, p);
   return B2_OK;
 }
diff --git a/ffsubsync_b200/csrc/vad.cu b/ffsubsync_b200/csrc/vad.cu
--- a/ffsubsync_b200/csrc/vad.cu
+++ b/ffsubsync_b200/csrc/vad.cu
@@ -34,6 +34,7 @@
   long long pcm_total_bytes;
   long long e_min;
   const long long* tail_emin;
+  uint32_t* bits;
   int B, fpw, G, tw, z_lo, z_hi, fast, stage_bytes, cpl, stages, consumers, batch, evict_first;
   float label;
 };
@@ -296,7 +297,7 @@
   const long long w0 = (t - c.tile_lo) * p.tw;
   const long long s0 = c.sig0 + w0 * p.fpw;
   d.sig = c.b;
-  d.out_base = c.out0 + w0;
+  d.out_base = c.out0 + (p.bits ? w0 >> 5 : w0);
   d.n_left = c.sig1 - s0;
   d.seq = 0;
   if (t + 1 < c.tile_hi) {
@@ -453,7 +454,12 @@
         for (int i = 0; i < (int)avail; ++i) e += (long long)xs[i] * xs[i];
         speech = e >= p.tail_emin[d.sig];
       }
-      if (active) p.out[d.out_base + wl] = speech ? 1.0f : p.label;
+      if (p.bits) {
+        const uint32_t m = __ballot_sync(0xffffffffu, active && (speech || p.label == 1.0f));
+        if (lane == 0 && 32 * k < d.n_windows) p.bits[d.out_base + k] = m;
+      } else if (active) {
+        p.out[d.out_base + wl] = speech ? 1.0f : p.label;
+      }
     }
     __syncwarp();
     if (lane == 0) mbar_arrive(&empty_bar[stage]);
@@ -518,7 +524,7 @@
 
 int b2i_vad_launch(b2_ctx* h, const int16_t* d_pcm, const int64_t* pcm_off, int B, int fpw,
                    float non_speech_label, int64_t e_min_full, int z_lo, int z_hi,
-                   float* d_out, const int64_t* out_off, const int64_t* tail_emin) {
+                   float* d_out, const int64_t* out_off, const int64_t* tail_emin, bool packed) {
   B2Range range("b2:vad_energy_zcr");
   if (((uintptr_t)d_pcm & 15) != 0)
     B2_FAIL(h, B2_ERR_BAD_ARG, "vad: device PCM pointer must be 16-byte aligned");
@@ -595,6 +601,9 @@
       tile_off[b + 1] = tile_off[b] + ((n + fpw - 1) / fpw + p.tw - 1) / p.tw;
     }
   }
+  if (packed && !lane_layout)
+    B2_FAIL(h, B2_ERR_UNSUPPORTED, "vad: internal error: packed output asked of the lane-group kernel");
+  p.bits = packed ? reinterpret_cast<uint32_t*>(d_out) : nullptr;
   p.total_tiles = tile_off[B];
   if (p.total_tiles == 0) return B2_OK;
 
```

After: 13450, median of 6. 7.9% higher.
